# musikisomorphie/implicit-normalizing-flows

Measured on AMD Instinct MI355X. Metric: samples/sec (whole node) + bits/dim Δ vs ref, CIFAR10 density eval at 1/8 GPU, higher is better.
Workload: dtype f32; 1 GPU; cifar10 implicit flow density eval (run_cifar10.sh arch), batch 64 per GPU; global_batch=64, per_gpu_batch=64, parallelism=dp1, probes=device, mode=eval

## Files before the change

implicit-normalizing-flows_amd/csrc/engine.h:

```cpp
#pragma once
#include <math.h>
#include <stdio.h>
#include <stdlib.h>
#include <string.h>

#include <algorithm>
#include <functional>
#include <vector>

#include "glue.h"
#include "kernels.h"

constexpr unsigned INF_EV_SYNC = hipEventDisableTiming | hipEventDisableSystemFence;
constexpr unsigned INF_EV_TIMING = hipEventDisableSystemFence;

namespace inf {

constexpr int TAPS_MAX_CH = 64;
constexpr int SERIES_MAX = 128;

struct Operand {
  int load = BL_DIRECT;
  int taps = 0;
  int M = 0, Mpad = 0, K = 0, Kpad = 0;
  int pack = PK_ROWMAJOR;
  float* A = nullptr;
};

struct WLayer {
  int kind = 0, cin = 0, cout = 0, ks = 1;
  const float *W = nullptr, *b = nullptr, *u = nullptr, *v = nullptr;
  float coeff = 1.f;
  int act = ACT_NONE;
  const float* act_beta = nullptr;
  Operand f, g;
  float* factor = nullptr;
  float* zb = nullptr;
};

}

struct InfNet {
  int C = 0, H = 1, W = 1, P = 1, d = 0;
  bool fc = false;
  int pre_act = inf::ACT_NONE;
  const float* pre_beta = nullptr;
  std::vector<inf::WLayer> L;
  int hidden_max = 0;
  int rows_max = 0;
  float* dev = nullptr;
  double* scratch = nullptr;
  size_t scratch_doubles = 0;
  int device = 0;
  bool fused = false;
  int fhid = 0, K1pad = 0, M3 = 0, M3pad = 0;
  int ftiles = 0, fpix = 0;
  float *F1f = nullptr, *F1b = nullptr, *F2f = nullptr, *F2b = nullptr, *F3f = nullptr, *F3b = nullptr;
  uint16_t* Fs[6] = {nullptr, nullptr, nullptr, nullptr, nullptr, nullptr};
  uint16_t* Fh[6] = {nullptr, nullptr, nullptr, nullptr, nullptr, nullptr};
  int* Fexp = nullptr;
  uint16_t* Fhp[2] = {nullptr, nullptr};
  int mfma_mode = INF_MFMA_F32;
  float* f0 = nullptr;
  int f0_batch = -1;
  int k128 = 1;
  int eval_overlap = 1;
  int convergence = INF_CONV_GLOBAL;
  int line_search = 0;
  int exact_scale = 0;
  int presplit = 1;
  int fc_block = 1;
  int fc_series = 1;
  int fc_skinny = 1;
  bool fcfused = false;
  uint16_t* fch = nullptr;
  int* fchexp = nullptr;
  std::vector<size_t> fch_off;
  uint16_t* fcht = nullptr;
  int* fchtexp = nullptr;
};

namespace inf {

struct WS {
  char* base;
  size_t cap, off;
  bool ok = true;
  template <typename T>
  T* take(size_t n) {
    off = (off + 255) & ~(size_t)255;
    T* p = base ? reinterpret_cast<T*>(base + off) : nullptr;
    off += n * sizeof(T);
    if (off > cap) ok = false;
    return p;
  }
};

struct Bufs {
  float *h0, *h1, *Y;
  std::vector<float*> D;
  float *xin, *xemb, *fx, *xa, *xb, *ga, *gb, *upd, *dx, *dg, *lowest, *va, *vb, *eps_t, *zero, *tmp;
  float *fcur, *flow;
  float* fspec;
  float *U, *VT;
  float *ext0, *ext1;
  double *part, *bpart, *sumsq;
  double* ps_state;
  int *ps_active, *ps_improved;
  float *ps_lowx, *ps_lowf;
  unsigned int* counter;
  int nchunk;
  float* Y2;
  int snchunk;
  unsigned* bk_sync;
  size_t bk_sync_bytes;
  char* bk_out;
  size_t bk_out_bytes;
  hipEvent_t stop_ev = nullptr;
  bool stop_bound = false;
  float* kslab = nullptr;
  size_t kslab_bytes = 0;
  bool sample_sums = false;
};

struct GradBufs {
  std::vector<float*> H, Hd, Ad;
  std::vector<float*> A;
  float *gA, *gB, *hA, *hB, *gad, *ga, *Y, *slab, *dWe, *dWe2, *dsig, *xin, *tmp_in, *act;
  float *x_t, *w_t, *e_t, *gx_t;
  double *bpart, *dot;
  int max_split;
  float* kslab;
  size_t kslab_bytes;
};

size_t carve(const InfNet* n, int B, int T, void* ws, size_t cap, Bufs& b);
size_t ws_need(const InfNet* n, int B, int T);
inline int carve_ws(const InfNet* n, int B, int T, void* ws, size_t ws_bytes, Bufs& b) {
  return (!ws || carve(n, B, T, ws, ws_bytes, b) > ws_bytes) ? INF_ERR_WORKSPACE : INF_OK;
}

inline bool same_shape(const InfNet* a, const InfNet* b) {
  return a->C == b->C && a->H == b->H && a->W == b->W && a->fc == b->fc && a->d == b->d;
}
inline bool fused_pair(const InfNet* a, const InfNet* b) {
  return a->fused && b->fused && a->fhid == b->fhid && (a->L[0].act == ACT_SWISH) == (b->L[0].act == ACT_SWISH);
}

GemmArgs gemm_base(const InfNet* n, const Operand& op, const float* X, int in_ch, int B);
void set_out(const InfNet* n, GemmArgs& g, float* out, int out_rows);
int layer_gemm(const InfNet* n, const GemmArgs& g, int load, int epi, float* kslab, size_t kslab_bytes, hipStream_t s);
Net313Args net313_args(const InfNet* n, const float* in, int B, Bufs& bf, bool vjp);
FcArgs fc_args(const InfNet* n, const float* x, int B);
int out_stage(const InfNet* n, const Operand& op, int mode, OutArgs a, float* Y, int B, hipStream_t s);
inline Operand fused_taps(const InfNet* n) {
  Operand op;
  op.taps = 1;
  op.M = n->M3;
  return op;
}
int run_forward(InfNet* n, const float* x, int B, Bufs& bf, int mode, const OutArgs* oa, hipStream_t s);
int run_vjp(InfNet* n, const float* v, float* vout, const float* xin, const float* eps, double* partial, int B,
            Bufs& bf, hipStream_t s);
int to_internal(InfNet* n, const float* x, float* buf, int B, hipStream_t s, const float** xi);
int to_boundary(InfNet* n, const float* xi, float* out, int B, hipStream_t s);
template <typename Produce>
int write_boundary(InfNet* n, Bufs& bf, float* out, int B, hipStream_t s, Produce&& produce) {
  INF_TRY(produce(n->fc ? bf.tmp : out));
  return n->fc ? to_boundary(n, bf.tmp, out, B, s) : INF_OK;
}

int host_wait(hipEvent_t ev);
InfBroydenStats stats_for(const InfBroydenStats* caller);
struct SpecTail {
  std::function<int(const float* x, const float* f)> fn;
  const float* x = nullptr;
  const float* f = nullptr;
};
int broyden_solve(InfNet* f, const float* y, int B, int T, double eps_in, InfBroydenStats* st, float* diff_detail,
                  Bufs& bf, hipStream_t s, SpecTail* tail = nullptr);
int fc_block_eval(InfNet* nx, InfNet* nz, const float* x, float* z, float* logdet_x, float* logdet_z, int B, int T,
                  double eps_in, InfBroydenStats* stats, Bufs& bf, hipStream_t s);
void solve_release_thread();

int fc_jacobian(InfNet* n, const float* x, int B, Bufs& bf, const float** tang, hipStream_t s);
void logdet_release_thread();

}
```

implicit-normalizing-flows_amd/csrc/engine_chain.hip:

```cpp
#include "engine.h"

using namespace inf;

GemmArgs inf::gemm_base(const InfNet* n, const Operand& op, const float* X, int in_ch, int B) {
  GemmArgs g;
  memset(&g, 0, sizeof(g));
  g.x6 = n->mfma_mode != INF_MFMA_F32;
  g.A = op.A;
  g.M = op.M;
  g.Kpad = op.Kpad;
  g.Ktot = op.K;
  g.X = X;
  if (n->fc) {
    g.P = B;
    g.N = B;
    g.x_sample = 0;
    g.H = 1;
    g.W = B;
  } else {
    g.P = n->P;
    g.N = B * n->P;
    g.x_sample = (long)in_ch * n->P;
    g.H = n->H;
    g.W = n->W;
// ... 108 lines not shown
  }
  const float* cur = x;
  int cur_ch = n->C;
  for (int l = 0; l < L - 1; ++l) {
    const WLayer& w = n->L[l];
    float* out = (l % 2 == 0) ? bf.h0 : bf.h1;
    GemmArgs g = gemm_base(n, w.f, cur, cur_ch, B);
    g.pre_beta = (l == 0) ? n->pre_beta : nullptr;
    g.pre_act = (l == 0) ? n->pre_act : ACT_NONE;
    set_out(n, g, out, w.cout);
    g.bias = w.b;
    g.act = w.act;
    g.act_beta = w.act_beta;
    g.deriv_out = (mode < 0) ? bf.D[l] : nullptr;
    g.write_out = (mode < 0 && l == L - 2) ? 0 : 1;
    INF_TRY(layer_gemm(n, g, w.f.load, EP_BIAS_ACT, bf.kslab, bf.kslab_bytes, s));
    cur = out;
    cur_ch = w.cout;
  }
  if (mode < 0) return INF_OK;
  const WLayer& w = n->L[L - 1];
  GemmArgs g = gemm_base(n, w.f, cur, cur_ch, B);
  g.pre_beta = (L == 1) ? n->pre_beta : nullptr;
  g.pre_act = (L == 1) ? n->pre_act : ACT_NONE;
  set_out(n, g, bf.Y, w.f.M);
  INF_TRY(layer_gemm(n, g, w.f.load, EP_STORE, bf.kslab, bf.kslab_bytes, s));
  OutArgs a = *oa;
  a.bias = w.b;
  a.pre_beta = nullptr;
  return out_stage(n, w.f, mode, a, bf.Y, B, s);
}

int inf::run_vjp(InfNet* n, const float* v, float* vout, const float* xin, const float* eps, double* partial, int B,
                 Bufs& bf, hipStream_t s) {
  const int L = (int)n->L.size();
  OutArgs a;
  memset(&a, 0, sizeof(a));
  a.in0 = eps;
  a.in1 = xin;
  a.out0 = vout;
  a.pre_beta = n->pre_beta;
  a.pre_act = n->pre_act;
  a.partial = partial;
  a.nchunk = n->fc ? fc_nchunk(n->d) : out_nchunk(n->d);
  if (n->fused) {
    Net313Args f = net313_args(n, v, B, bf, true);
    INF_TRY(launch_net313(f, n->fhid, MODE_VJP, s));
    return out_stage(n, fused_taps(n), OM_VJP, a, bf.Y, B, s);
  }
  const float* cur = v;
  int cur_ch = n->C;
  for (int l = L - 1; l >= 1; --l) {
    const WLayer& w = n->L[l];
    float* out = ((L - 1 - l) % 2 == 0) ? bf.h0 : bf.h1;
    GemmArgs g = gemm_base(n, w.g, cur, cur_ch, B);
    set_out(n, g, out, w.cin);
    g.deriv_in = bf.D[l - 1];
    INF_TRY(layer_gemm(n, g, w.g.load, EP_MUL_DERIV, bf.kslab, bf.kslab_bytes, s));
    cur = out;
    cur_ch = w.cin;
  }
  const WLayer& w = n->L[0];
  GemmArgs g = gemm_base(n, w.g, cur, cur_ch, B);
  set_out(n, g, bf.Y, w.g.M);
  INF_TRY(layer_gemm(n, g, w.g.load, EP_STORE, bf.kslab, bf.kslab_bytes, s));
  return out_stage(n, w.g, OM_VJP, a, bf.Y, B, s);
}

int inf::to_internal(InfNet* n, const float* x, float* buf, int B, hipStream_t s, const float** xi) {
  *xi = n->fc ? buf : x;
  return n->fc ? launch_transpose(x, buf, B, n->d, s) : INF_OK;
}
int inf::to_boundary(InfNet* n, const float* xi, float* out, int B, hipStream_t s) {
  if (!n->fc) {
    if (xi != out) INF_HIP(hipMemcpyAsync(out, xi, sizeof(float) * (size_t)B * n->d, hipMemcpyDeviceToDevice, s));
    return INF_OK;
  }
  return launch_transpose(xi, out, n->d, B, s);
}

extern "C" {

int inf_net_forward(InfNet* n, const float* x, float* y, int B, void* ws, size_t ws_bytes, void* stream) {
  if (!n || !x || !y || B <= 0) return INF_ERR_INVALID;
  hipStream_t s = (hipStream_t)stream;
  Bufs bf;
  INF_TRY(carve_ws(n, B, 1, ws, ws_bytes, bf));
  const float* xi;
  INF_TRY(to_internal(n, x, bf.xin, B, s, &xi));
  OutArgs a;
  memset(&a, 0, sizeof(a));
  return write_boundary(n, bf, y, B, s, [&](float* o) {
    a.out0 = o;
    return run_forward(n, xi, B, bf, OM_PLAIN, &a, s);
  });
}

int inf_net_vjp(InfNet* n, const float* x, const float* v, float* out, int B, void* ws, size_t ws_bytes,
                void* stream) {
  if (!n || !x || !v || !out || B <= 0) return INF_ERR_INVALID;
  hipStream_t s = (hipStream_t)stream;
  Bufs bf;
  INF_TRY(carve_ws(n, B, 1, ws, ws_bytes, bf));
  const float *xi, *vi;
  INF_TRY(to_internal(n, x, bf.xin, B, s, &xi));
  INF_TRY(to_internal(n, v, bf.eps_t, B, s, &vi));
  INF_TRY(run_forward(n, xi, B, bf, -1, nullptr, s));
  return write_boundary(n, bf, out, B, s,
                        [&](float* o) { return run_vjp(n, vi, o, xi, nullptr, nullptr, B, bf, s); });
}

}
```

implicit-normalizing-flows_amd/csrc/engine_grad.hip:

```cpp
#include "engine.h"

using namespace inf;

namespace {

constexpr int GRAD_SPLIT = 32;
constexpr int GRAD_BLOCKS = 512;

size_t carve_grad(const InfNet* n, int B, void* ws, size_t cap, GradBufs& g) {
  WS w{reinterpret_cast<char*>(ws), cap, 0};
  const size_t hid = (size_t)B * n->hidden_max * n->P, in = (size_t)B * n->d;
  const int L = (int)n->L.size();
  size_t mn = 1;
  for (const auto& l : n->L) mn = std::max(mn, (size_t)l.cout * l.cin * l.ks * l.ks);
  g.H.resize(L > 0 ? L - 1 : 0);
  g.Hd.resize(L > 0 ? L - 1 : 0);
  g.Ad.resize(L > 0 ? L : 0);
  for (auto& p : g.H) p = w.take<float>(hid);
  for (auto& p : g.Hd) p = w.take<float>(hid);
  for (int l = 0; l < L; ++l) g.Ad[l] = w.take<float>(l == 0 ? in : hid);
  g.A.resize(L > 0 ? L : 0);
  for (int l = 0; l < L; ++l) g.A[l] = w.take<float>(l == 0 ? in : hid);
  for (float** p : {&g.gA, &g.gB, &g.hA, &g.hB, &g.gad, &g.ga}) *p = w.take<float>(std::max(hid, in));
  g.Y = w.take<float>((size_t)B * n->rows_max * n->P);
// ... 233 lines not shown
                                nin, GRAD_BLOCKS, s));
        if (n->pre_beta && gr->dpre_beta) INF_TRY(launch_beta_reduce(gb.bpart, GRAD_BLOCKS, gr->dpre_beta, 0, s));
      } else if (gx) {
        if (G_pri) INF_HIP(hipMemcpyAsync(gx, gb.ga, sizeof(float) * nin, hipMemcpyDeviceToDevice, s));
        else INF_HIP(hipMemsetAsync(gx, 0, sizeof(float) * nin, s));
      }
    }
  }
  return INF_OK;
}

constexpr int FC_JAC_MAX = 16;

size_t logdet_grad_layout(InfNet* n, int B, int mode, int n_terms, char* ws, size_t cap, Bufs* bf, GradBufs* gb,
                          float** A, float** bv, float** xr, float** gxs, float** eps_t, float** a_scr, float** b_scr) {
  const int T = mode == LOGDET_SERIES ? n_terms : n->d;
  const long N = (long)T * B;
  Bufs bf0;
  GradBufs gb0;
  const size_t s1 = (carve(n, B, 1, ws, ws ? cap : 0, bf ? *bf : bf0) + 255) & ~(size_t)255;
  char* w2 = ws ? ws + s1 : nullptr;
  const size_t s2 = (carve_grad(n, (int)N, w2, ws ? (cap > s1 ? cap - s1 : 0) : 0, gb ? *gb : gb0) + 255) & ~(size_t)255;
  WS w{ws ? ws + s1 + s2 : nullptr, ws ? (cap > s1 + s2 ? cap - s1 - s2 : 0) : 0, 0};
  float* p[6];
  const size_t cnt[6] = {(size_t)n->d * N, (size_t)n->d * N, (size_t)n->d * N, (size_t)n->d * N,
                         n->d > FC_JAC_MAX ? 0 : (size_t)n->d * B, mode == LOGDET_SERIES ? (size_t)n_terms * n->d * B : 1};
  for (int i = 0; i < 6; ++i) p[i] = w.take<float>(cnt[i]);
  float* pb = n->d > FC_JAC_MAX ? w.take<float>(((size_t)n_terms + 1) * n->d * B) : nullptr;
  if (A) {
    *A = p[0];
    *bv = p[1];
    *xr = p[2];
    *gxs = p[3];
    *eps_t = p[4];
    *a_scr = p[5];
    *b_scr = pb;
  }
  return s1 + s2 + w.off + 256;
}

int run_jvp(InfNet* n, const float* v, float* out, int B, Bufs& bf, hipStream_t s) {
  const int L = (int)n->L.size();
  const float* cur = v;
  for (int l = 0; l < L; ++l) {
    const WLayer& w = n->L[l];
    const bool last = l == L - 1;
    float* o = last ? out : ((l % 2 == 0) ? bf.h0 : bf.h1);
    GemmArgs g = gemm_base(n, w.f, cur, w.cin, B);
    set_out(n, g, o, w.cout);
    g.deriv_in = last ? nullptr : bf.D[l];
    INF_TRY(layer_gemm(n, g, w.f.load, last ? EP_STORE : EP_MUL_DERIV, bf.kslab, bf.kslab_bytes, s));
    cur = o;
  }
  return INF_OK;
}

int series_pairs_chains(InfNet* n, const float* x, const float* eps, const float* coeff, int n_terms, const float* gout,
                        float* value, int B, Bufs& bf, float* A, float* bv, float* xr, float* a_scr, float* b_scr,
                        hipStream_t s) {
  const size_t dB = (size_t)n->d * B;
  const float* xi;
  INF_TRY(to_internal(n, x, bf.xin, B, s, &xi));
  INF_TRY(launch_transpose(eps, a_scr, B, n->d, s));
  INF_HIP(hipMemcpyAsync(b_scr, a_scr, sizeof(float) * dB, hipMemcpyDeviceToDevice, s));
  INF_TRY(run_forward(n, xi, B, bf, -1, nullptr, s));
  for (int j = 0; j + 1 < n_terms; ++j)
    INF_TRY(run_vjp(n, a_scr + j * dB, a_scr + (j + 1) * dB, xi, nullptr, nullptr, B, bf, s));
  for (int m = 0; m < n_terms; ++m) INF_TRY(run_jvp(n, b_scr + m * dB, b_scr + (m + 1) * dB, B, bf, s));
  return launch_series_pairs_wide(a_scr, b_scr, xi, gout, coeff, n_terms, n->d, B, A, bv, xr, value, s);
}

}

extern "C" {

size_t inf_grad_workspace_bytes(InfNet* n, int B) {
  if (!n || B <= 0) return 0;
  GradBufs gb;
  return carve_grad(n, B, nullptr, 0, gb);
}

int inf_net_param_grad(InfNet* n, const float* x, const float* gout, float* gx, const InfNetGrads* gr, int B,
                       void* ws, size_t ws_bytes, void* stream) {
  if (!n || !x || !gout || !gr || B <= 0) return INF_ERR_INVALID;
  if (!grad_supported(n)) return INF_ERR_UNSUPPORTED;
  hipStream_t s = (hipStream_t)stream;
  GradBufs gb;
  if (!ws || carve_grad(n, B, ws, ws_bytes, gb) > ws_bytes) return INF_ERR_WORKSPACE;
  if (!n->fc) return param_grad_core(n, x, gout, gx, gr, B, gb, s);
  INF_TRY(launch_transpose(x, gb.x_t, B, n->d, s));
  INF_TRY(launch_transpose(gout, gb.w_t, B, n->d, s));
  INF_TRY(param_grad_core(n, gb.x_t, gb.w_t, gx ? gb.gx_t : nullptr, gr, B, gb, s));
  if (gx) INF_TRY(launch_transpose(gb.gx_t, gx, n->d, B, s));
  return INF_OK;
}

int inf_net_surrogate_grad(InfNet* n, const float* x, const float* w, const float* eps, float* value, float* gx,
                           const InfNetGrads* gr, int B, void* ws, size_t ws_bytes, void* stream) {
  if (!n || !x || !w || !eps || !gr || B <= 0) return INF_ERR_INVALID;
  if (!grad_supported(n) || (n->fc && value)) return INF_ERR_UNSUPPORTED;
  hipStream_t s = (hipStream_t)stream;
  GradBufs gb;
  if (!ws || carve_grad(n, B, ws, ws_bytes, gb) > ws_bytes) return INF_ERR_WORKSPACE;
  if (!n->fc) return surrogate_core(n, x, w, eps, value, gx, gr, B, gb, s);
  INF_TRY(launch_transpose(x, gb.x_t, B, n->d, s));
  INF_TRY(launch_transpose(w, gb.w_t, B, n->d, s));
  INF_TRY(launch_transpose(eps, gb.e_t, B, n->d, s));
  INF_TRY(surrogate_core(n, gb.x_t, gb.w_t, gb.e_t, nullptr, gx ? gb.gx_t : nullptr, gr, B, gb, s));
  if (gx) INF_TRY(launch_transpose(gb.gx_t, gx, n->d, B, s));
  return INF_OK;
}

size_t inf_logdet_grad_workspace_bytes(InfNet* n, int B, int mode, int n_terms) {
  if (!n || B <= 0 || mode < LOGDET_SERIES || mode > LOGDET_TRACE || (mode != LOGDET_EXACT && n_terms < 1)) return 0;
  return logdet_grad_layout(n, B, mode, n_terms, nullptr, 0, nullptr, nullptr, nullptr, nullptr, nullptr, nullptr,
                            nullptr, nullptr, nullptr);
}

int inf_logdet_grad(InfNet* n, const float* x, int mode, const float* eps, const float* coeff, int n_terms,
                    const float* gout, float* value, float* gx, const InfNetGrads* gr, int B, void* ws, size_t ws_bytes,
                    void* stream) {
  if (!n || !x || !gr || B <= 0 || mode < LOGDET_SERIES || mode > LOGDET_TRACE) return INF_ERR_INVALID;
  if (mode == LOGDET_SERIES && (!eps || !coeff || n_terms < 1 || n_terms > 128)) return INF_ERR_INVALID;
  if (mode == LOGDET_TRACE && (!coeff || n_terms < 1 || n_terms > 128)) return INF_ERR_INVALID;
  const bool wide = n->fc && n->d > FC_JAC_MAX;
  if (!n->fc || (wide && mode != LOGDET_SERIES) || !grad_supported(n)) return INF_ERR_UNSUPPORTED;
  if (wide && (long)n_terms * B > 0x7fffffffL) return INF_ERR_INVALID;
  hipStream_t s = (hipStream_t)stream;
  Bufs bf;
  GradBufs gb;
  float *A, *bv, *xr, *gxs, *eps_t, *a_scr, *b_scr;
  const int nt = mode == LOGDET_EXACT ? 1 : n_terms;
  if (!ws || logdet_grad_layout(n, B, mode, nt, reinterpret_cast<char*>(ws), ws_bytes, &bf, &gb, &A, &bv, &xr, &gxs,
                                &eps_t, &a_scr, &b_scr) > ws_bytes)
    return INF_ERR_WORKSPACE;
  const int T = mode == LOGDET_SERIES ? n_terms : n->d;
  if (wide) {
    INF_TRY(series_pairs_chains(n, x, eps, coeff, n_terms, gout, value, B, bf, A, bv, xr, a_scr, b_scr, s));
  } else {
    const float* tang = nullptr;
    INF_TRY(fc_jacobian(n, x, B, bf, &tang, s));
    if (mode == LOGDET_SERIES) INF_TRY(launch_transpose(eps, eps_t, B, n->d, s));
    const float one = 1.f;
    INF_TRY(launch_logdet_pairs(mode, tang, eps_t, bf.xin, gout, mode == LOGDET_EXACT ? &one : coeff, nt, n->d, B, A,
                                bv, xr, value, a_scr, s));
  }
  INF_TRY(surrogate_core(n, xr, A, bv, nullptr, gx ? gxs : nullptr, gr, T * B, gb, s));
  if (gx) INF_TRY(launch_sum_pairs(gxs, T, n->d, B, gx, s));
  return INF_OK;
}

}
```

implicit-normalizing-flows_amd/csrc/engine_logdet.hip:

```cpp
#include "engine.h"

using namespace inf;

namespace {

int series_fused(InfNet* const* nets, const float* const* xs, const float* const* es, int nn, const float* coeff,
                 int n_terms, float* const* outs, int B, Bufs* bfs, hipStream_t s, unsigned save_mask = 3u,
                 float* const* wouts = nullptr, const float* ncoeff = nullptr) {
  Net313Args args[2];
  for (int i = 0; i < nn; ++i) {
    args[i] = net313_args(nets[i], xs[i], B, bfs[i], false);
    if (!wouts) INF_HIP(hipMemsetAsync(bfs[i].part, 0, sizeof(double) * n_terms * B * bfs[i].snchunk, s));
    else INF_HIP(hipMemcpyAsync(wouts[i], es[i], sizeof(float) * (size_t)B * nets[i]->d, hipMemcpyDeviceToDevice, s));
  }
  const unsigned all = (1u << nn) - 1u;
  if ((save_mask & all) == all) {
    INF_TRY(launch_net313_multi(args, nn, nets[0]->fhid, MODE_SAVE, s));
  } else {
    for (int i = 0; i < nn; ++i)
      if (save_mask & (1u << i)) INF_TRY(launch_net313_multi(&args[i], 1, nets[0]->fhid, MODE_SAVE, s, nn));
  }
  for (int k = 0; k < n_terms; ++k) {
    for (int i = 0; i < nn; ++i) {
      InfNet* n = nets[i];
      Bufs& bf = bfs[i];
      Net313Args& v = args[i];
      v = net313_args(n, es[i], B, bf, true);
      v.Y = (k % 2 == 0) ? bf.Y : bf.Y2;
      v.tile_order = k & 1;
      if (k > 0) {
        v.in = nullptr;
        v.in_taps = (k % 2 == 1) ? bf.Y : bf.Y2;
        v.vmul_x = n->pre_act != ACT_NONE ? xs[i] : nullptr;
        v.vmul_beta = n->pre_beta;
        v.vmul_act = n->pre_act == ACT_SWISH ? 0 : n->pre_act;
        if (wouts) {
          v.acc_w = wouts[i];
          v.acc_coef = ncoeff[k];
        } else {
          v.dot_eps = es[i];
          v.dot_part = bf.part + (size_t)(k - 1) * B * bf.snchunk;
          v.dot_nchunk = bf.snchunk;
        }
      }
    }
    INF_TRY(launch_net313_multi(args, nn, nets[0]->fhid, MODE_VJP, s));
  }
  for (int i = 0; i < nn; ++i) {
    InfNet* n = nets[i];
    Bufs& bf = bfs[i];
    OutArgs a;
    memset(&a, 0, sizeof(a));
    a.in0 = wouts ? nullptr : es[i];
    a.in1 = xs[i];
    a.out0 = bf.va;
    a.pre_beta = n->pre_beta;
    a.pre_act = n->pre_act;
    a.partial = wouts ? nullptr : bf.part + (size_t)(n_terms - 1) * B * bf.snchunk;
    a.nchunk = bf.snchunk;
    INF_TRY(out_stage(n, fused_taps(n), OM_VJP, a, ((n_terms - 1) % 2 == 0) ? bf.Y : bf.Y2, B, s));
    if (wouts) INF_TRY(glue_axpy_scaled(wouts[i], bf.va, ncoeff[n_terms], (long)B * n->d, s));
  }
  if (wouts) return INF_OK;
  for (int i = 0; i < nn; ++i)
    INF_TRY(launch_series_combine(bfs[i].part, coeff, n_terms, B, bfs[i].snchunk, outs[i], s));
  return INF_OK;
}

struct SideStream {
  hipStream_t s = nullptr;
  hipEvent_t fork = nullptr, join = nullptr;
};
thread_local SideStream g_side[16];
SideStream* side_stream() {
  int dev = 0;
  if (hipGetDevice(&dev) != hipSuccess || dev < 0 || dev >= 16) return nullptr;
  SideStream& ss = g_side[dev];
  if (!ss.s) {
    if (hipStreamCreateWithFlags(&ss.s, hipStreamNonBlocking) != hipSuccess) return nullptr;
    if (hipEventCreateWithFlags(&ss.fork, INF_EV_SYNC) != hipSuccess ||
        hipEventCreateWithFlags(&ss.join, INF_EV_SYNC) != hipSuccess)
      return nullptr;
  }
  return &ss;
}

struct SideJoin {
  SideStream* side = nullptr;
  hipStream_t s = nullptr;
  ~SideJoin() {
    if (!side) return;
    (void)hipEventRecord(side->join, side->s);
    (void)hipStreamWaitEvent(s, side->join, 0);
  }
};

struct FcNextX {
  InfNet* nx = nullptr;
  Bufs* bf = nullptr;
  float* logdet = nullptr;
  bool done = false;
};
struct FcLogpStep {
  const float* lin = nullptr;
  float* lout = nullptr;
  bool done = false;
};
bool fc_block_first(const InfNet* nz) {
  return nz->fc_block == 2 || (nz->fc_block == 1 && nz->convergence == INF_CONV_PER_SAMPLE);
}
bool fc_pair_ok(const InfNet* a, const InfNet* b) {
  return a->fcfused && b->fcfused && a->mfma_mode == INF_MFMA_F16X3 && b->mfma_mode == INF_MFMA_F16X3 &&
         same_shape(a, b) && !a->L.empty() && !b->L.empty() && a->L[0].act == b->L[0].act;
}

int eval_exact_fc(InfNet* nx, InfNet* nz, const float* x, float* z, float* logdet_x, float* logdet_z, int B, int T,
                  double eps, InfBroydenStats* stats, Bufs& bf, hipStream_t s, bool x_done, FcNextX* next,
                  FcLogpStep* lp = nullptr) {
  if (next) next->done = false;
  if (lp) lp->done = false;
  const float* xi = bf.xin;
  if (fc_block_first(nz)) {
    const int st = fc_block_eval(nx, nz, x, z, logdet_x, logdet_z, B, T, eps, stats, bf, s);
    if (st != INF_ERR_UNSUPPORTED) return st;
  }
  if (!x_done) {
    FcArgs fjx = fc_args(nx, nullptr, B);
    fjx.x_bnd = x;
    fjx.x_int = bf.xin;
    fjx.logdet = logdet_x;
    fjx.o.in0 = xi;
    fjx.o.out0 = bf.fx;
    fjx.o.out1 = bf.xemb;
    INF_TRY(launch_fcnet(fjx, true, s));
  }
  auto jac_z = [&](const float* flow) {
    FcArgs fjz = fc_args(nz, nullptr, B);
    fjz.logdet = logdet_z;
    fjz.rc_fx = bf.fx;
    fjz.rc_fz = flow;
    fjz.rc_x = xi;
    fjz.rc_out = z;
    if (lp) {
      fjz.lp_in = lp->lin;
      fjz.lp_ldx = logdet_x;
      fjz.lp_out = lp->lout;
      lp->done = true;
    }
    if (next) {
      FcArgs fjn = fc_args(next->nx, nullptr, B);
      fjn.rc_fx = bf.fx;
      fjn.rc_fz = flow;
      fjn.rc_x = xi;
      fjn.x_int = next->bf->xin;
      fjn.logdet = next->logdet;
      fjn.o.out0 = next->bf->fx;
      fjn.o.out1 = next->bf->xemb;
      const int st = launch_fcnet_jac_pair(fjz, fjn, s);
      next->done = st == INF_OK;
      if (st != INF_ERR_UNSUPPORTED) return st;
    }
    return launch_fcnet(fjz, true, s);
  };
  SpecTail tail;
  tail.fn = [&](const float*, const float* f) { return jac_z(f); };
  InfBroydenStats sst = stats_for(stats);
  INF_TRY(broyden_solve(nz, xi, B, T, eps, &sst, nullptr, bf, s, nz->convergence == INF_CONV_GLOBAL ? &tail : nullptr));
  if (stats) *stats = sst;
  if (!sst.prot_break) {
    if (tail.x && tail.x == bf.lowest && tail.f == bf.flow) return INF_OK;
    return jac_z(bf.flow);
  }
  if (next) next->done = false;
  if (lp) lp->done = false;
  OutArgs a;
  memset(&a, 0, sizeof(a));
// ... 67 lines not shown
  }
  const float *xi, *ei;
  INF_TRY(to_internal(n, x, bf.xin, B, s, &xi));
  INF_TRY(to_internal(n, vareps, bf.eps_t, B, s, &ei));
  if (n->fused) return series_fused(&n, &xi, &ei, 1, coeff, n_terms, &out, B, &bf, s);
  INF_TRY(run_forward(n, xi, B, bf, -1, nullptr, s));
  const float* v = ei;
  for (int k = 0; k < n_terms; ++k) {
    float* vo = (k % 2 == 0) ? bf.va : bf.vb;
    INF_TRY(run_vjp(n, v, vo, xi, ei, bf.part + (size_t)k * B * bf.nchunk, B, bf, s));
    v = vo;
  }
  return launch_series_combine(bf.part, coeff, n_terms, B, bf.nchunk, out, s);
}

int neumann_w(InfNet* n, const float* xi, const float* ei, const float* ncoeff, int n_terms, int B, Bufs& bf,
              hipStream_t s) {
  const size_t E = (size_t)B * n->d;
  INF_TRY(run_forward(n, xi, B, bf, -1, nullptr, s));
  INF_HIP(hipMemcpyAsync(bf.tmp, ei, sizeof(float) * E, hipMemcpyDeviceToDevice, s));
  const float* v = ei;
  for (int k = 1; k <= n_terms; ++k) {
    float* vo = (k % 2 == 1) ? bf.va : bf.vb;
    INF_TRY(run_vjp(n, v, vo, xi, nullptr, nullptr, B, bf, s));
    INF_TRY(glue_axpy_scaled(bf.tmp, vo, ncoeff[k], (long)E, s));
    v = vo;
  }
  return INF_OK;
}

}

int inf::fc_jacobian(InfNet* n, const float* x, int B, Bufs& bf, const float** tang, hipStream_t s) {
  const int d = n->d;
  const float* xi;
  INF_TRY(to_internal(n, x, bf.xin, B, s, &xi));
  if (n->fcfused) {
    FcArgs f = fc_args(n, xi, B);
    f.tang = bf.ext1;
    if (fcnet_supported(f, true)) {
      INF_TRY(launch_fcnet(f, true, s));
      *tang = bf.ext1;
      return INF_OK;
    }
  }
  INF_TRY(glue_init_tangents(xi, bf.ext0, d, B, s));
  const int cols = (d + 1) * B;
  const float* cur = bf.ext0;
  for (size_t l = 0; l < n->L.size(); ++l) {
    const WLayer& w = n->L[l];
    float* o = (l % 2 == 0) ? bf.ext1 : bf.ext0;
    GemmArgs g;
    memset(&g, 0, sizeof(g));
    g.A = w.f.A;
    g.M = w.f.M;
    g.Kpad = w.f.Kpad;
    g.Ktot = w.f.K;
    g.X = cur;
    g.x_sample = 0;
    g.P = cols;
    g.N = cols;
    g.H = 1;
    g.W = cols;
    g.out = o;
    g.o_sample = 0;
    g.bias = w.b;
    g.n_primal = B;
    INF_TRY(launch_gemm(g, BL_DIRECT, EP_BIAS_PRIMAL, s));
    if (w.act != ACT_NONE) INF_TRY(launch_fwdmode_act(o, nullptr, w.cout, B, d, w.act, w.act_beta, s));
    cur = o;
  }
  *tang = cur;
  return INF_OK;
}

void inf::logdet_release_thread() {
  int cur = 0;
  (void)hipGetDevice(&cur);
  for (int dev = 0; dev < 16; ++dev) {
    SideStream& ss = g_side[dev];
    if (!ss.s) continue;
    (void)hipSetDevice(dev);
    (void)hipStreamSynchronize(ss.s);
    if (ss.fork) (void)hipEventDestroy(ss.fork);
    if (ss.join) (void)hipEventDestroy(ss.join);
    (void)hipStreamDestroy(ss.s);
    ss = SideStream{};
  }
  (void)hipSetDevice(cur);
}

extern "C" {

int inf_imblock_eval(InfNet* nx, InfNet* nz, const float* x, float* z, const float* eps_x, const float* eps_z,
                     const float* coeff, int n_terms, float* logdet_x, float* logdet_z, int B, int T, double eps,
                     InfBroydenStats* stats, void* ws, size_t ws_bytes, void* stream) {
  if (!nx || !nz || !x || !z || !eps_x || !eps_z || !coeff || !logdet_x || !logdet_z || B <= 0 || T <= 0 || T > 64 ||
      n_terms < 1 || n_terms > SERIES_MAX || !same_shape(nx, nz))
    return INF_ERR_INVALID;
  if (!fused_pair(nx, nz)) return INF_ERR_UNSUPPORTED;
  hipStream_t s = (hipStream_t)stream;
  const size_t half = ws_need(nx, B, T), zneed = ws_need(nz, B, 1), xneed = ws_need(nx, B, 1);
  if (!ws || ws_bytes < half + zneed) return INF_ERR_WORKSPACE;
  char* w0 = reinterpret_cast<char*>(ws);
  Bufs bfa, bfb, bfc;
  carve(nx, B, T, w0, half, bfa);
  carve(nz, B, 1, w0 + half, zneed, bfb);
  const bool overlap = nx->eval_overlap && ws_bytes >= half + zneed + xneed;
  if (overlap) {
    carve(nx, B, 1, w0 + half + zneed, xneed, bfc);
    bfc.D = bfa.D;
  }
  const int layout = overlap ? 1 : 2;
  {
    Net313Args f = net313_args(nx, x, B, bfa, false);
    INF_TRY(launch_net313_multi(&f, 1, nx->fhid, MODE_EVALSAVE, s, layout));
    OutArgs a;
    memset(&a, 0, sizeof(a));
    a.bias = nx->L[2].b;
    a.in0 = x;
    a.out0 = bfa.fx;
    a.out1 = bfa.xemb;
    INF_TRY(out_stage(nx, fused_taps(nx), OM_EMBED, a, bfa.Y, B, s));
  }
  SideJoin join;
  if (overlap) {
    SideStream* side = side_stream();
    if (!side) return INF_ERR_HIP;
    INF_HIP(hipEventRecord(side->fork, s));
    INF_HIP(hipStreamWaitEvent(side->s, side->fork, 0));
    join.side = side;
    join.s = s;
    INF_TRY(series_fused(&nx, &x, &eps_x, 1, coeff, n_terms, &logdet_x, B, &bfc, side->s, 0u));
  }
  InfBroydenStats st = stats_for(stats);
  INF_TRY(broyden_solve(nz, x, B, T, eps, &st, nullptr, bfa, s));
  if (stats) *stats = st;
  if (!st.prot_break) {
    INF_TRY(glue_recomp(bfa.fx, bfa.flow, x, z, (long)B * nx->d, s));
  } else {
    OutArgs a;
    memset(&a, 0, sizeof(a));
    a.in0 = bfa.fx;
    a.in1 = x;
    a.out0 = z;
    INF_TRY(run_forward(nz, bfa.lowest, B, bfa, OM_RECOMP, &a, s));
  }
  if (overlap) {
    const float* zin = z;
    return series_fused(&nz, &zin, &eps_z, 1, coeff, n_terms, &logdet_z, B, &bfb, s, 1u);
  }
  InfNet* nets[2] = {nx, nz};
  const float* xs[2] = {x, z};
  const float* es[2] = {eps_x, eps_z};
  float* outs[2] = {logdet_x, logdet_z};
  Bufs bfs[2] = {bfa, bfb};
  return series_fused(nets, xs, es, 2, coeff, n_terms, outs, B, bfs, s, 2u);
}

int inf_imblock_eval_exact(InfNet* nx, InfNet* nz, const float* x, float* z, float* logdet_x, float* logdet_z, int B,
                           int T, double eps, InfBroydenStats* stats, void* ws, size_t ws_bytes, void* stream) {
  if (!nx || !nz || !x || !z || !logdet_x || !logdet_z || B <= 0 || T <= 0 || T > 64 || !same_shape(nx, nz))
    return INF_ERR_INVALID;
  INF_TRY(eval_exact_check(nx, nz, x, B));
  Bufs bf;
  INF_TRY(carve_ws(nz, B, T, ws, ws_bytes, bf));
  return eval_exact_fc(nx, nz, x, z, logdet_x, logdet_z, B, T, eps, stats, bf, (hipStream_t)stream, false, nullptr);
}

size_t inf_flow_chain_workspace_bytes(InfNet* const* net_z, int n_blocks, int batch, const int* thresholds) {
  if (!net_z || n_blocks <= 0 || batch <= 0 || !thresholds) return 0;
  size_t blk = 0;
  for (int i = 0; i < n_blocks; ++i)
    if (net_z[i]) blk = std::max(blk, inf_workspace_bytes(net_z[i], batch, thresholds[i]));
  const size_t d = net_z[0] ? (size_t)net_z[0]->d : 0;
  return 2 * ((blk + 255) & ~(size_t)255) + 256 * 8 + sizeof(float) * ((size_t)2 * batch * d + (size_t)6 * batch);
}

int inf_flow_eval_exact_chain(InfNet* const* net_x, InfNet* const* net_z, int n_blocks, const float* x, float* z,
                              const float* logp_in, float* logp_out, int B, const int* thresholds, const double* eps,
                              InfBroydenStats* stats, void* ws, size_t ws_bytes, void* stream) {
  if (!net_x || !net_z || n_blocks <= 0 || !x || !z || !logp_out || B <= 0 || !thresholds || !eps || x == z ||
      logp_in == logp_out)
    return INF_ERR_INVALID;
  for (int i = 0; i < n_blocks; ++i) {
    InfNet *nx = net_x[i], *nz = net_z[i];
    if (!nx || !nz || !same_shape(nx, nz) || !same_shape(nz, net_z[0]) || thresholds[i] <= 0 || thresholds[i] > 64)
      return INF_ERR_INVALID;
    INF_TRY(eval_exact_check(nx, nz, x, B));
  }
  if (!ws || ws_bytes < inf_flow_chain_workspace_bytes(net_z, n_blocks, B, thresholds)) return INF_ERR_WORKSPACE;
  hipStream_t s = (hipStream_t)stream;
  const size_t E = (size_t)B * net_z[0]->d;
  size_t blk = 0;
  for (int i = 0; i < n_blocks; ++i) blk = std::max(blk, inf_workspace_bytes(net_z[i], B, thresholds[i]));
  blk = (blk + 255) & ~(size_t)255;
  char* base = reinterpret_cast<char*>(ws);
  size_t off = 2 * blk;
  auto take = [&](size_t bytes) {
    off = (off + 255) & ~(size_t)255;
    char* p = base + off;
    off += bytes;
    return reinterpret_cast<float*>(p);
  };
  float* zb[2] = {take(sizeof(float) * E), take(sizeof(float) * E)};
  float* ldx[2] = {take(sizeof(float) * B), take(sizeof(float) * B)};
  float* ldz[2] = {take(sizeof(float) * B), take(sizeof(float) * B)};
  float* lp[2] = {take(sizeof(float) * B), take(sizeof(float) * B)};
  Bufs bfs[2];
  auto carve_block = [&](int i) {
    return carve_ws(net_z[i], B, thresholds[i], base + (size_t)(i & 1) * blk, blk, bfs[i & 1]);
  };
  INF_TRY(carve_block(0));
  const float* in = x;
  const float* lin = logp_in;
  bool x_done = false;
  for (int i = 0; i < n_blocks; ++i) {
    const bool last = i == n_blocks - 1;
    float* out = last ? z : zb[i & 1];
    float* lout = last ? logp_out : lp[i & 1];
    FcNextX nxt;
    FcNextX* np = nullptr;
    if (!last) {
      INF_TRY(carve_block(i + 1));
      if (!fc_block_first(net_z[i]) && !fc_block_first(net_z[i + 1]) && fc_pair_ok(net_z[i], net_x[i + 1])) {
        nxt.nx = net_x[i + 1];
        nxt.bf = &bfs[(i + 1) & 1];
        nxt.logdet = ldx[(i + 1) & 1];
        np = &nxt;
      }
    }
    FcLogpStep lps;
    lps.lin = lin;
    lps.lout = lout;
    INF_TRY(eval_exact_fc(net_x[i], net_z[i], in, out, ldx[i & 1], ldz[i & 1], B, thresholds[i], eps[i],
                          stats ? &stats[i] : nullptr, bfs[i & 1], s, x_done, np, &lps));
    if (!lps.done) INF_TRY(glue_logp_step(lin, ldx[i & 1], ldz[i & 1], lout, B, s));
    x_done = np && nxt.done;
    in = out;
    lin = lout;
  }
  return INF_OK;
}

int inf_logdet_series(InfNet* n, const float* x, const float* vareps, const float* coeff, int n_terms, float* out,
                      int B, void* ws, size_t ws_bytes, void* stream) {
  if (!n || !x || !vareps || !coeff || !out || B <= 0 || n_terms < 0 || n_terms > SERIES_MAX) return INF_ERR_INVALID;
  return series_single(n, x, vareps, coeff, n_terms, out, B, ws, ws_bytes, (hipStream_t)stream, true);
}

int inf_logdet_series_pair(InfNet* na, const float* xa, const float* ea, InfNet* nb, const float* xb, const float* eb,
                           const float* coeff, int n_terms, float* out_a, float* out_b, int B, void* ws,
                           size_t ws_bytes, void* stream) {
  if (!na || !nb || !xa || !xb || !ea || !eb || !coeff || !out_a || !out_b || B <= 0 || n_terms < 0 ||
      n_terms > SERIES_MAX || !same_shape(na, nb))
    return INF_ERR_INVALID;
  const size_t half = ws_need(na, B, 1);
  if (!ws || ws_bytes < 2 * half) return INF_ERR_WORKSPACE;
  char* w0 = reinterpret_cast<char*>(ws);
  hipStream_t s = (hipStream_t)stream;
  InfNet* nets[2] = {na, nb};
  const float* xs[2] = {xa, xb};
  const float* es[2] = {ea, eb};
  float* outs[2] = {out_a, out_b};
  if (n_terms > 0) {
    const int st = fc_series(nets, xs, es, coeff, n_terms, outs, 2, B, s);
    if (st != INF_ERR_UNSUPPORTED) return st;
  }
  if (!fused_pair(na, nb)) {
    INF_TRY(series_single(na, xa, ea, coeff, n_terms, out_a, B, w0, half, s, false));
    return series_single(nb, xb, eb, coeff, n_terms, out_b, B, w0 + half, half, s, false);
  }
  Bufs bfs[2];
  carve(na, B, 1, w0, half, bfs[0]);
  carve(nb, B, 1, w0 + half, half, bfs[1]);
  if (n_terms == 0) {
    INF_HIP(hipMemsetAsync(out_a, 0, sizeof(float) * B, s));
    INF_HIP(hipMemsetAsync(out_b, 0, sizeof(float) * B, s));
    return INF_OK;
  }
  return series_fused(nets, xs, es, 2, coeff, n_terms, outs, B, bfs, s);
}

int inf_neumann_vector(InfNet* n, const float* x, const float* vareps, const float* ncoeff, int n_terms, float* w,
                       int B, void* ws, size_t ws_bytes, void* stream) {
  if (!n || !x || !vareps || !ncoeff || !w || B <= 0 || n_terms < 0) return INF_ERR_INVALID;
  hipStream_t s = (hipStream_t)stream;
  Bufs bf;
  INF_TRY(carve_ws(n, B, 1, ws, ws_bytes, bf));
  const float *xi, *ei;
  INF_TRY(to_internal(n, x, bf.xin, B, s, &xi));
  INF_TRY(to_internal(n, vareps, bf.eps_t, B, s, &ei));
  INF_TRY(neumann_w(n, xi, ei, ncoeff, n_terms, B, bf, s));
  return to_boundary(n, bf.tmp, w, B, s);
}

int inf_neumann_vector_pair(InfNet* na, const float* xa, const float* ea, InfNet* nb, const float* xb,
                            const float* eb, const float* ncoeff, int n_terms, float* wa, float* wb, int B, void* ws,
                            size_t ws_bytes, void* stream) {
  if (!na || !nb || !xa || !xb || !ea || !eb || !ncoeff || !wa || !wb || B <= 0 || n_terms < 0 || !same_shape(na, nb))
    return INF_ERR_INVALID;
  const size_t half = ws_bytes / 2;
  char* w1 = reinterpret_cast<char*>(ws) + half;
  if (!fused_pair(na, nb) || n_terms == 0) {
    INF_TRY(inf_neumann_vector(na, xa, ea, ncoeff, n_terms, wa, B, ws, half, stream));
    return inf_neumann_vector(nb, xb, eb, ncoeff, n_terms, wb, B, w1, half, stream);
  }
  hipStream_t s = (hipStream_t)stream;
  Bufs bfs[2];
  INF_TRY(carve_ws(na, B, 1, ws, half, bfs[0]));
  INF_TRY(carve_ws(nb, B, 1, w1, half, bfs[1]));
  InfNet* nets[2] = {na, nb};
  const float* xs[2] = {xa, xb};
  const float* es[2] = {ea, eb};
  float* wouts[2] = {wa, wb};
  float* outs[2] = {nullptr, nullptr};
  return series_fused(nets, xs, es, 2, nullptr, n_terms, outs, B, bfs, s, 3u, wouts, ncoeff);
}

int inf_logdet_neumann(InfNet* n, const float* x, const float* vareps, const float* ncoeff, int n_terms, float* out,
                       int B, void* ws, size_t ws_bytes, void* stream) {
  if (!n || !x || !vareps || !ncoeff || !out || B <= 0 || n_terms < 0) return INF_ERR_INVALID;
  hipStream_t s = (hipStream_t)stream;
  Bufs bf;
  INF_TRY(carve_ws(n, B, 1, ws, ws_bytes, bf));
  const float *xi, *ei;
  INF_TRY(to_internal(n, x, bf.xin, B, s, &xi));
  INF_TRY(to_internal(n, vareps, bf.eps_t, B, s, &ei));
  INF_TRY(neumann_w(n, xi, ei, ncoeff, n_terms, B, bf, s));
  INF_TRY(run_vjp(n, bf.tmp, bf.va, xi, ei, bf.part, B, bf, s));
  const float one = 1.f;
  return launch_series_combine(bf.part, &one, 1, B, bf.nchunk, out, s);
}

int inf_logdet_exact(InfNet* n, const float* x, float* out, int B, void* ws, size_t ws_bytes, void* stream) {
  if (!n || !x || !out || B <= 0) return INF_ERR_INVALID;
  if (!n->fc || n->d > 16 || n->pre_act != ACT_NONE) return INF_ERR_UNSUPPORTED;
  hipStream_t s = (hipStream_t)stream;
  Bufs bf;
  INF_TRY(carve_ws(n, B, 1, ws, ws_bytes, bf));
  if (n->fcfused) {
    const float* xi;
    INF_TRY(to_internal(n, x, bf.xin, B, s, &xi));
    FcArgs f = fc_args(n, xi, B);
    f.logdet = out;
    if (fcnet_supported(f, true)) return launch_fcnet(f, true, s);
  }
  const float* tang = nullptr;
  INF_TRY(fc_jacobian(n, x, B, bf, &tang, s));
  return launch_logdet_small(tang, out, n->d, B, B, s);
}

int inf_logdet_exact_trace(InfNet* n, const float* x, const float* coeff, int n_terms, float* out, int B, void* ws,
                           size_t ws_bytes, void* stream) {
  if (!n || !x || !coeff || !out || B <= 0 || n_terms < 1 || n_terms > SERIES_MAX) return INF_ERR_INVALID;
  if (!n->fc || n->d > 16 || n->pre_act != ACT_NONE) return INF_ERR_UNSUPPORTED;
  hipStream_t s = (hipStream_t)stream;
  Bufs bf;
  INF_TRY(carve_ws(n, B, 1, ws, ws_bytes, bf));
  const float* tang = nullptr;
  INF_TRY(fc_jacobian(n, x, B, bf, &tang, s));
  return launch_trace_series(tang, coeff, n_terms, out, n->d, B, B, s);
}

}
```

implicit-normalizing-flows_amd/csrc/engine_plan.hip:

```cpp
#include <memory>
#include <new>

#include "engine.h"

using namespace inf;

namespace {

int round_up(int x, int m) { return (x + m - 1) / m * m; }

bool fused_act_kind(int act) {
  return act == ACT_SWISH || act == ACT_SIN || act == ACT_ELU || act == ACT_SOFTPLUS || act == ACT_RELU;
}

int act_of_kind(int kind) {
  switch (kind) {
    case INF_ACT_SWISH: return ACT_SWISH;
    case INF_ACT_SIN: return ACT_SIN;
    case INF_ACT_ELU: return ACT_ELU;
    case INF_ACT_SOFTPLUS: return ACT_SOFTPLUS;
    case INF_ACT_RELU: return ACT_RELU;
    case INF_ACT_LCUBE: return ACT_LCUBE;
    case INF_ACT_IDENTITY: return ACT_IDENTITY;
    case INF_ACT_ZERO: return ACT_ZERO;
    default: return -1;
  }
}

struct FusedSizes {
  size_t n[6];
  explicit FusedSizes(const InfNet* net) {
    n[0] = n[1] = (size_t)net->fhid * net->K1pad;
    n[2] = n[3] = (size_t)net->fhid * net->fhid;
    n[4] = n[5] = (size_t)net->M3pad * net->fhid;
  }
  size_t sum() const { return n[0] + n[1] + n[2] + n[3] + n[4] + n[5]; }
};

int parse_mfma(const char* mm, bool has_bf16x6, int* mode) {
  if (!mm || !*mm) return INF_OK;
  if (!strcmp(mm, "f32") || !strcmp(mm, "fp32")) *mode = INF_MFMA_F32;
  else if (!strcmp(mm, "bf16x6")) *mode = has_bf16x6 ? INF_MFMA_BF16X6 : INF_MFMA_F32;
  else if (strcmp(mm, "f16x3") != 0) {
    fprintf(stderr, "libinflow: INFLOW_MFMA=%s is not one of f32, fp32, bf16x6, f16x3\n", mm);
    return INF_ERR_INVALID;
  }
  return INF_OK;
}

struct NetOption {
  int id;
  int InfNet::*slot;
  int hi;
  const char* env;
  const char* names[4];
  bool resets_f0;
};
const NetOption OPTIONS[] = {
    {INF_OPT_FUSED_K128, &InfNet::k128, 3, "INFLOW_FUSED_K128", {"0", "1", "2", "3"}, true},
    {INF_OPT_EVAL_OVERLAP, &InfNet::eval_overlap, 1, "INFLOW_EVAL_OVERLAP", {"0", "1"}, false},
    {INF_OPT_CONVERGENCE, &InfNet::convergence, 1, "INFLOW_CONVERGENCE", {"global", "per_sample"}, false},
    {INF_OPT_LINE_SEARCH, &InfNet::line_search, 1, nullptr, {}, false},
    {INF_OPT_K128_EXACT_SCALE, &InfNet::exact_scale, 1, nullptr, {}, true},
    {INF_OPT_FC_BLOCK, &InfNet::fc_block, 2, "INFLOW_FC_BLOCK", {"0", "1", "2"}, false},
    {INF_OPT_FC_SERIES, &InfNet::fc_series, 1, "INFLOW_FC_SERIES", {"0", "1"}, false},
    {INF_OPT_FC_SKINNY, &InfNet::fc_skinny, 1, nullptr, {}, false},
    {INF_OPT_FUSED_PRESPLIT, &InfNet::presplit, 1, "INFLOW_FUSED_PRESPLIT", {"0", "1"}, false},
};
const NetOption* find_option(int id) {
  for (const NetOption& o : OPTIONS)
    if (o.id == id) return &o;
  return nullptr;
}

void free_net(InfNet* n) {
  if (!n) return;
  if (n->dev) (void)hipFree(n->dev);
  if (n->scratch) (void)hipFree(n->scratch);
  if (n->f0) (void)hipFree(n->f0);
  if (n->fch) (void)hipFree(n->fch);
  if (n->fchexp) (void)hipFree(n->fchexp);
  delete n;
}
struct NetDeleter {
  void operator()(InfNet* n) const { free_net(n); }
};

size_t per_sample_hidden(const InfNet* n) {
  return (size_t)n->hidden_max * (n->fc ? 1 : (n->fused ? std::max(n->P, n->fpix) : n->P));
}

}

size_t inf::carve(const InfNet* n, int B, int T, void* ws, size_t cap, Bufs& b) {
  WS w{reinterpret_cast<char*>(ws), cap, 0};
  const size_t E = (size_t)B * n->d;
  const size_t Hs = (size_t)B * per_sample_hidden(n);
  const size_t Ys = (size_t)B * n->rows_max * (n->fc ? 1 : n->P);
  const int nchunk = n->fc ? fc_nchunk(n->d) : out_nchunk(n->d);
  b.nchunk = nchunk;
  b.snchunk = n->fused ? std::max(nchunk, std::max(n->P / 32, n->ftiles)) : nchunk;
  b.h0 = w.take<float>(Hs);
  b.h1 = w.take<float>(Hs);
  b.Y = w.take<float>(Ys);
  b.Y2 = n->fused ? w.take<float>(Ys) : nullptr;
  b.D.resize(n->L.size() > 0 ? n->L.size() - 1 : 0);
  for (auto& p : b.D) p = w.take<float>(Hs);
  float** vecs[] = {&b.xin, &b.xemb, &b.fx, &b.xa, &b.xb, &b.ga, &b.gb, &b.upd,
                    &b.dx, &b.dg, &b.lowest, &b.va, &b.vb, &b.eps_t, &b.zero, &b.tmp, &b.fcur, &b.flow,
                    &b.fspec, &b.ps_lowx, &b.ps_lowf};
  for (float** v : vecs) *v = w.take<float>(E);
  b.U = w.take<float>((size_t)T * E);
  b.VT = w.take<float>((size_t)T * E);
  if (n->fc && n->d <= 16) {
    const size_t ext = (size_t)(n->d + 1) * B * std::max(n->hidden_max, n->d);
    b.ext0 = w.take<float>(ext);
    b.ext1 = w.take<float>(ext);
  } else {
    b.ext0 = b.ext1 = nullptr;
  }
  b.part = w.take<double>((size_t)B * std::max(nchunk, b.snchunk) * SERIES_MAX);
  const int bch = (n->d + 1023) / 1024;
  b.bpart = w.take<double>((size_t)B * bch * (3 * (size_t)T + 2) + 64);
  b.sumsq = w.take<double>((size_t)B + 1);
  b.counter = w.take<unsigned int>(64);
  b.ps_state = w.take<double>((size_t)B * (PS_HEAD + T));
  b.ps_active = w.take<int>((size_t)B);
  b.ps_improved = w.take<int>((size_t)B);
  if (n->fc) {
    b.bk_sync_bytes = 16 + sizeof(unsigned long long) * 8 * (size_t)fcblock_grid(B);
    b.bk_sync = reinterpret_cast<unsigned*>(w.take<char>(b.bk_sync_bytes));
    b.bk_out_bytes = sizeof(FcBlockStats) + (sizeof(int) * 3 + sizeof(double)) * (size_t)B + 64;
    b.bk_out = w.take<char>(b.bk_out_bytes);
  } else {
    b.bk_sync = nullptr;
    b.bk_out = nullptr;
    b.bk_sync_bytes = b.bk_out_bytes = 0;
  }
  b.kslab_bytes = (n->fc && n->d > FC_NARROW_MAX) ? SKINNY_SLAB_BYTES : 0;
  b.kslab = b.kslab_bytes ? w.take<float>(b.kslab_bytes / sizeof(float)) : nullptr;
  return w.off + 256;
}

// ... 203 lines not shown
    if (v < 0) {
      fprintf(stderr, "libinflow: %s=%s is not one of", o.env, e);
      for (int k = 0; k <= o.hi; ++k) fprintf(stderr, " %s", o.names[k]);
      fprintf(stderr, "\n");
      return INF_ERR_INVALID;
    }
    n->*o.slot = v;
  }
  size_t sc = SIGMA_MAX_PARTS + 64;
  for (auto& w : n->L) sc = std::max(sc, (size_t)w.cout * (n->fc ? 1 : n->P) / 256 + 64);
  n->scratch_doubles = sc;
  if (hipGetDevice(&n->device) != hipSuccess) n->device = 0;
  if (hipMalloc(&n->dev, floats * sizeof(float)) != hipSuccess ||
      hipMalloc(&n->scratch, sc * sizeof(double)) != hipSuccess)
    return INF_ERR_HIP;
  float* p = n->dev;
  for (auto& w : n->L) {
    for (Operand* op : {&w.f, &w.g}) {
      op->A = p;
      p += (size_t)op->Mpad * op->Kpad + 64;
    }
    w.factor = p;
    p += 64;
    if (!w.b) {
      w.zb = p;
      w.b = p;
      p += round_up(w.cout, 64);
    }
  }
  if (n->fused) {
    float** bufs[] = {&n->F1f, &n->F1b, &n->F2f, &n->F2b, &n->F3f, &n->F3b};
    const FusedSizes sz(n);
    for (int k = 0; k < 6; ++k) {
      *bufs[k] = p;
      p += sz.n[k] + 64;
    }
    for (int k = 0; k < 6; ++k) {
      n->Fs[k] = reinterpret_cast<uint16_t*>(p);
      p += (3 * sz.n[k] + 1) / 2 + 64;
    }
    for (int k = 0; k < 6; ++k) {
      n->Fh[k] = reinterpret_cast<uint16_t*>(p);
      p += sz.n[k] + 64;
    }
    n->Fexp = reinterpret_cast<int*>(p);
    p += 64;
    for (int k = 0; k < 2; ++k) {
      n->Fhp[k] = reinterpret_cast<uint16_t*>(p);
      p += sz.n[4 + k] + 64;
    }
  }
  *out = net.release();
  return INF_OK;
}

int inf_net_destroy(InfNet* n) {
  free_net(n);
  return INF_OK;
}

int inf_net_set_mfma(InfNet* n, int mode) {
  if (!n || (mode != INF_MFMA_F32 && mode != INF_MFMA_BF16X6 && mode != INF_MFMA_F16X3)) return INF_ERR_INVALID;
  if (n->mfma_mode != mode) n->f0_batch = -1;
  n->mfma_mode = mode;
  return INF_OK;
}
int inf_net_get_mfma(const InfNet* n) { return n ? n->mfma_mode : -1; }

int inf_net_set_option(InfNet* n, int option, int value) {
  const NetOption* o = n ? find_option(option) : nullptr;
  if (!o || value < 0 || value > o->hi) return -INF_ERR_INVALID;
  const int prev = n->*o->slot;
  n->*o->slot = value;
  if (prev != value && o->resets_f0) n->f0_batch = -1;
  return prev;
}

int inf_net_get_option(const InfNet* n, int option) {
  const NetOption* o = n ? find_option(option) : nullptr;
  return o ? n->*o->slot : -INF_ERR_INVALID;
}

int inf_net_refresh(InfNet* n, void* stream) {
  if (!n) return INF_ERR_INVALID;
  hipStream_t s = (hipStream_t)stream;
  n->f0_batch = -1;
  for (auto& w : n->L) {
    if (w.zb) INF_HIP(hipMemsetAsync(w.zb, 0, sizeof(float) * w.cout, s));
    const int H = n->fc ? 1 : (w.ks == 1 ? 1 : n->H), Wd = n->fc ? 1 : (w.ks == 1 ? 1 : n->W);
    INF_TRY(launch_sigma(w.W, w.u, w.v, w.cout, w.cin, w.ks, H, Wd, w.coeff, w.factor,
                         reinterpret_cast<float*>(n->scratch), s));
    INF_TRY(launch_pack(w.W, w.factor, w.f.A, w.cout, w.cin, w.ks, w.f.Mpad, w.f.Kpad, w.f.pack, s));
    INF_TRY(launch_pack(w.W, w.factor, w.g.A, w.cout, w.cin, w.ks, w.g.Mpad, w.g.Kpad, w.g.pack, s));
  }
  if (n->fch) {
    const int L = (int)n->L.size();
    for (int l = 0; l < L; ++l) {
      const WLayer& w = n->L[l];
      const int nrt = l == L - 1 ? 1 : 8, nks = l == 0 ? 1 : 4;
      INF_TRY(launch_fc_split_h3(w.f.A, w.cout, w.f.Kpad, nrt, nks, n->fch + n->fch_off[l], n->fchexp + l, s));
      const int j = L - 1 - l, trt = j == L - 1 ? 1 : 8, tks = j == 0 ? 1 : 4;
      INF_TRY(launch_fc_split_h3(w.g.A, w.cin, w.g.Kpad, trt, tks, n->fcht + n->fch_off[j], n->fchtexp + j, s));
    }
  }
  if (n->fused) {
    const WLayer &l0 = n->L[0], &l1 = n->L[1], &l2 = n->L[2];
    const int H = n->fhid;
    INF_TRY(launch_pack(l0.W, l0.factor, n->F1f, l0.cout, l0.cin, 3, H, n->K1pad, PK_IM2COL_FWD, s, 1));
    INF_TRY(launch_pack(l2.W, l2.factor, n->F1b, l2.cout, l2.cin, 3, H, n->K1pad, PK_IM2COL_BWD, s, 1));
    INF_TRY(launch_pack(l1.W, l1.factor, n->F2f, H, H, 1, H, H, PK_ROWMAJOR, s, 1));
    INF_TRY(launch_pack(l1.W, l1.factor, n->F2b, H, H, 1, H, H, PK_TRANSPOSE, s, 1));
    INF_TRY(launch_pack(l2.W, l2.factor, n->F3f, l2.cout, l2.cin, 3, n->M3pad, H, PK_TAPS_FWD, s, 1));
    INF_TRY(launch_pack(l0.W, l0.factor, n->F3b, l0.cout, l0.cin, 3, n->M3pad, H, PK_TAPS_BWD, s, 1));
    const float* src[6] = {n->F1f, n->F1b, n->F2f, n->F2b, n->F3f, n->F3b};
    const FusedSizes cnt(n);
    for (int i = 0; i < 6; ++i) INF_TRY(launch_split3(src[i], n->Fs[i], (long)cnt.n[i], s));
    for (int i = 0; i < 6; ++i)
      INF_TRY(launch_split2h(src[i], n->Fh[i], (long)cnt.n[i], n->Fexp + 3 * (i & 1) + i / 2, s));
    for (int i = 0; i < 2; ++i) INF_TRY(launch_permute_k23(n->Fh[4 + i], n->Fhp[i], (long)cnt.n[4 + i] / 512, s));
  }
  return INF_OK;
}

}
```

implicit-normalizing-flows_amd/csrc/engine_solve.hip:

```cpp
#include <chrono>
#include <thread>

#include "engine.h"

using namespace inf;

namespace {

struct SumsSlot {
  double* host = nullptr;
  hipEvent_t ev = nullptr;
  int cap = 0;
};
thread_local SumsSlot g_sums_slots[2];
int sums_slot(int i, int B, SumsSlot** out) {
  SumsSlot& sl = g_sums_slots[i & 1];
  if (sl.cap < B + 1) {
    if (sl.host) (void)hipHostFree(sl.host);
    sl.host = nullptr;
    const int cap = std::max(B + 1, 1024);
    if (hipHostMalloc(reinterpret_cast<void**>(&sl.host), sizeof(double) * cap, hipHostMallocCoherent) != hipSuccess)
      return INF_ERR_HIP;
    sl.cap = cap;
  }
// ... 744 lines not shown
  INF_HIP(hipMemcpyAsync(g_bk_host, bf.bk_sync, 16, hipMemcpyDeviceToHost, s));
  INF_HIP(hipMemcpyAsync(g_bk_host + 16, bf.bk_out, nbytes, hipMemcpyDeviceToHost, s));
  if (!g_bk_ev && hipEventCreateWithFlags(&g_bk_ev, INF_EV_SYNC) != hipSuccess) return INF_ERR_HIP;
  hipEvent_t ev = g_bk_ev;
  INF_HIP(hipEventRecord(ev, s));
  INF_TRY(host_wait(ev));
  if (*reinterpret_cast<unsigned*>(g_bk_host) != 0) {
    set_hip_error(hipErrorLaunchTimeOut);
    return INF_ERR_HIP;
  }
  const FcBlockStats* hs = reinterpret_cast<const FcBlockStats*>(g_bk_host + 16);
  InfBroydenStats st = stats_for(stats);
  st.convergence = nz->convergence;
  if (!a.per_sample) {
    st.nstep = hs->nstep;
    st.lowest_step = hs->lowest_step;
    st.prot_break = hs->prot_break;
    st.n_trace = std::min(hs->n_trace, 64);
    for (int k = 0; k < st.n_trace; ++k) st.trace[k] = hs->trace[k];
    st.diff = hs->lowest;
    st.eps = a.eps;
  } else {
    const char* base = g_bk_host + 16;
    const int* sn = reinterpret_cast<const int*>(base + sizeof(FcBlockStats));
    const int* sl = sn + B;
    const int* sp = sl + B;
    const double* slo = reinterpret_cast<const double*>(
        base + ((sizeof(FcBlockStats) + sizeof(int) * 3 * (size_t)B + 7) & ~(size_t)7));
    double d2 = 0.0;
    for (int b = 0; b < B; ++b) {
      st.nstep = std::max(st.nstep, sn[b]);
      st.lowest_step = std::max(st.lowest_step, sl[b]);
      st.prot_break |= sp[b];
      d2 += slo[b] * slo[b];
      if (st.sample_nstep) st.sample_nstep[b] = sn[b];
      if (st.sample_lowest_step) st.sample_lowest_step[b] = sl[b];
      if (st.sample_prot_break) st.sample_prot_break[b] = sp[b];
    }
    st.diff = sqrt(d2);
    st.eps = a.eps_ps;
  }
  st.tnstep = st.nstep;
  if (st.prot_break) {
    std::vector<int> todo;
    if (a.per_sample) {
      const int* sp = reinterpret_cast<const int*>(g_bk_host + 16 + sizeof(FcBlockStats)) + 2 * B;
      todo.assign(sp, sp + B);
    }
    int it = 0;
    INF_TRY(banach_solve(nz, bf.xin, B, eps_in, 1000, todo.empty() ? nullptr : todo.data(), bf, s, &it));
    st.fixed_point_iters = it;
    OutArgs o;
    memset(&o, 0, sizeof(o));
    o.in0 = bf.fx;
    o.in1 = bf.xin;
    o.out0 = bf.tmp;
    INF_TRY(run_forward(nz, bf.lowest, B, bf, OM_RECOMP, &o, s));
    FcArgs fjz = fc_args(nz, bf.tmp, B);
    fjz.logdet = logdet_z;
    INF_TRY(launch_fcnet(fjz, true, s));
    INF_TRY(to_boundary(nx, bf.tmp, z, B, s));
  }
  if (stats) *stats = st;
  return INF_OK;
}

void inf::solve_release_thread() {
  for (SumsSlot& sl : g_sums_slots) {
    if (sl.host) (void)hipHostFree(sl.host);
    if (sl.ev) (void)hipEventDestroy(sl.ev);
    sl = SumsSlot{};
  }
  if (g_bk_host) (void)hipHostFree(g_bk_host);
  g_bk_host = nullptr;
  g_bk_host_cap = 0;
  if (g_bk_ev) (void)hipEventDestroy(g_bk_ev);
  g_bk_ev = nullptr;
}

extern "C" {

int inf_root_find(InfNet* f, InfNet* e, const float* y, float* out, int B, int T, double eps, InfBroydenStats* stats,
                  float* diff_detail, void* ws, size_t ws_bytes, void* stream) {
  if (!f || !e || !y || !out || B <= 0 || T <= 0 || T > 64 || !same_shape(f, e)) return INF_ERR_INVALID;
  hipStream_t s = (hipStream_t)stream;
  Bufs bf;
  INF_TRY(carve_ws(f, B, T, ws, ws_bytes, bf));
  const float* yi;
  INF_TRY(embed(f, e, y, B, bf, &yi, s));
  INF_TRY(broyden_solve(f, yi, B, T, eps, stats, diff_detail, bf, s));
  return to_boundary(f, bf.lowest, out, B, s);
}

int inf_imblock_forward(InfNet* nx, InfNet* nz, const float* x, float* z, int B, int T, double eps,
                        InfBroydenStats* stats, void* ws, size_t ws_bytes, void* stream) {
  if (!nx || !nz || !x || !z || B <= 0 || T <= 0 || T > 64 || !same_shape(nx, nz)) return INF_ERR_INVALID;
  hipStream_t s = (hipStream_t)stream;
  Bufs bf;
  INF_TRY(carve_ws(nx, B, T, ws, ws_bytes, bf));
  const float* xi;
  InfBroydenStats st = stats_for(stats);
  INF_TRY(embed(nz, nx, x, B, bf, &xi, s));
  INF_TRY(broyden_solve(nz, xi, B, T, eps, &st, nullptr, bf, s));
  if (stats) *stats = st;
  return write_boundary(nx, bf, z, B, s, [&](float* o) {
    if (!st.prot_break) return glue_recomp(bf.fx, bf.flow, xi, o, (long)B * nx->d, s);
    OutArgs a;
    memset(&a, 0, sizeof(a));
    a.in0 = bf.fx;
    a.in1 = xi;
    a.out0 = o;
    return run_forward(nz, bf.lowest, B, bf, OM_RECOMP, &a, s);
  });
}

int inf_imblock_backward(InfNet* nx, InfNet* nz, const float* z, const float* x, const float* grad, float* dl_dh,
                         float* dl_dx, int B, int T, double eps, InfBroydenStats* stats, void* ws, size_t ws_bytes,
                         void* stream) {
  if (!nx || !nz || !z || !x || !grad || !dl_dh || !dl_dx || B <= 0 || T <= 0 || T > 64 || !same_shape(nx, nz))
    return INF_ERR_INVALID;
  hipStream_t s = (hipStream_t)stream;
  {
    Bufs bf;
    INF_TRY(carve_ws(nz, B, T, ws, ws_bytes, bf));
    const float *zi, *gi;
    INF_TRY(to_internal(nz, z, bf.xin, B, s, &zi));
    INF_TRY(to_internal(nz, grad, bf.xemb, B, s, &gi));
    INF_TRY(run_forward(nz, zi, B, bf, -1, nullptr, s));
    InfBroydenStats bs = stats_for(stats);
    std::vector<double> lowest_ss;
    const ResidFn resid = [&](const float* y, float* gout, float* dg, const float* gprev) {
      return vjp_resid_part(nz, y, zi, gi, gout, dg, gprev, B, bf, s);
    };
    INF_TRY(broyden_core(nz, resid, B, T, eps, bs, lowest_ss, bf, s));
    if (stats) *stats = bs;
    INF_TRY(to_boundary(nz, bf.lowest, dl_dh, B, s));
  }
  Bufs bf;
  INF_TRY(carve_ws(nx, B, 1, ws, ws_bytes, bf));
  const float *xi, *hi;
  INF_TRY(to_internal(nx, x, bf.xin, B, s, &xi));
  INF_TRY(to_internal(nx, dl_dh, bf.eps_t, B, s, &hi));
  INF_TRY(run_forward(nx, xi, B, bf, -1, nullptr, s));
  INF_TRY(run_vjp(nx, hi, bf.va, xi, nullptr, nullptr, B, bf, s));
  return write_boundary(nx, bf, dl_dx, B, s,
                        [&](float* o) { return glue_add(bf.va, hi, o, (long)B * nx->d, s); });
}

int inf_banach_find_root(InfNet* f, InfNet* e, const float* y, float* out, int B, int threshold, double eps,
                         int* iters, void* ws, size_t ws_bytes, void* stream) {
  if (!f || !e || !y || !out || B <= 0 || threshold < 0 || !same_shape(f, e)) return INF_ERR_INVALID;
  hipStream_t s = (hipStream_t)stream;
  Bufs bf;
  INF_TRY(carve_ws(f, B, 1, ws, ws_bytes, bf));
  const float* yi;
  INF_TRY(embed(f, e, y, B, bf, &yi, s));
  std::vector<int> todo;
  if (f->convergence == INF_CONV_PER_SAMPLE) todo.assign(B, 1);
  int it = 0;
  INF_TRY(banach_solve(f, yi, B, eps, threshold, todo.empty() ? nullptr : todo.data(), bf, s, &it));
  if (iters) *iters = it;
  return to_boundary(f, bf.lowest, out, B, s);
}

size_t inf_broyden_workspace_bytes(int batch, int d, int threshold) {
  const size_t nchunk = (size_t)(d + 1023) / 1024;
  return sizeof(double) * ((size_t)batch * nchunk * (3 * (size_t)threshold + 2) + 64);
}

int inf_broyden_update(float* U, float* VT, const float* dx, const float* dg, const float* gx, const float* x,
                       float* update, float* x_next, float* dx_next, int B, int d, int T, int nstep, void* ws,
                       size_t ws_bytes, void* stream) {
  if (!U || !VT || !dx || !dg || !gx || !x || !update || !x_next || !dx_next || B <= 0 || d <= 0 || T <= 0 ||
      T > 64 || nstep < 1 || nstep > T)
    return INF_ERR_INVALID;
  if (!ws || ws_bytes < inf_broyden_workspace_bytes(B, d, T)) return INF_ERR_WORKSPACE;
  BroydenArgs ba;
  memset(&ba, 0, sizeof(ba));
  ba.batch = B;
  ba.d = d;
  ba.T = T;
  ba.sb = d;
  ba.si = 1;
  ba.cs = (long)B * d;
  ba.U = U;
  ba.VT = VT;
  ba.dx = dx;
  ba.dg = dg;
  ba.gx = gx;
  ba.x = x;
  ba.xnew = x_next;
  ba.dxnew = dx_next;
  ba.upd = update;
  ba.part = reinterpret_cast<double*>(ws);
  ba.m = (nstep - 1) % T;
  ba.ncols = std::min(nstep, T);
  return launch_broyden_update(ba, (hipStream_t)stream);
}

int inf_broyden_line_step(const float* x0, const float* update, float step, float* x_est, float* dx, size_t n,
                          void* stream) {
  if (!x0 || !update || !x_est || !dx || n == 0) return INF_ERR_INVALID;
  return launch_line_step(x0, update, step, x_est, dx, (long)n, (hipStream_t)stream);
}

}
```

implicit-normalizing-flows_amd/csrc/glue.h:

```cpp
#pragma once
#include "common.h"

namespace inf {
int glue_logit(const float* x, float* y, const float* lin, float* lout, int B, int per, float alpha, hipStream_t s);
int glue_actnorm(const float* x, float* y, const float* w, const float* b, const float* lin, float* lout, int B, int C,
                 int hw, hipStream_t s);
int glue_squeeze2(const float* x, float* y, int B, int C, int H, int W, hipStream_t s);
int glue_normal_logprob(const float* z, float* out, int B, int per, hipStream_t s);
int glue_rademacher(float* out, size_t n, uint64_t seed, uint64_t offset, hipStream_t s);
int glue_poison_lds(hipStream_t s);
int glue_add(const float* a, const float* b, float* out, long n, hipStream_t s);
size_t glue_batched_dot_scratch(int B, long per);
int glue_batched_dot(const float* a, const float* c, float* out, int B, long per, double* scratch, hipStream_t s);
int glue_logp_step(const float* lin, const float* ldx, const float* ldz, float* lout, int B, hipStream_t s);
int glue_recomp(const float* fx, const float* fz, const float* x, float* out, long n, hipStream_t s);
int glue_fixed_point_check(const float* x, const float* xp, const float* y, long n, float eps, unsigned int* count,
                           hipStream_t s);
int glue_axpy_scaled(float* y, const float* x, float c, long n, hipStream_t s);
int glue_init_tangents(const float* xT, float* ext, int d, int B, hipStream_t s);
}
```

implicit-normalizing-flows_amd/csrc/glue.hip:

```cpp
#include "kernels.h"
#include "glue.h"

namespace inf {

__global__ __launch_bounds__(256) void logit_kernel(const float* x, float* y, const float* lin, float* lout, int per,
                                                    float alpha) {
  __shared__ double red[16];
  const int b = blockIdx.x;
  const float* xb = x + (long)b * per;
  float* yb = y + (long)b * per;
  const float c1 = 1.f - 2.f * alpha;
  const float lc = logf(c1);
  double acc = 0.0;
  for (int i = threadIdx.x; i < per; i += blockDim.x) {
    const float s = alpha + c1 * xb[i];
    yb[i] = logf(s) - logf(1.f - s);
    acc += (double)(-logf(s - s * s) + lc);
  }
  acc = block_sum(acc, red);
  if (threadIdx.x == 0) lout[b] = (lin ? lin[b] : 0.f) - (float)acc;
}

__global__ __launch_bounds__(256) void actnorm_kernel(const float* x, float* y, const float* w, const float* bias,
                                                      const float* lin, float* lout, int C, int hw, int vec) {
  __shared__ double red[16];
  const int b = blockIdx.y;
  const long per = (long)C * hw;
  const float* xb = x + b * per;
  float* yb = y + b * per;
  const long i0 = ((long)blockIdx.x * blockDim.x + threadIdx.x) * 4;
  if (vec) {
    if (i0 < per) {
      const int c = (int)(i0 / hw);
      const float bc = bias[c], ec = expf(w[c]);
      const float4 v = *reinterpret_cast<const float4*>(xb + i0);
      *reinterpret_cast<float4*>(yb + i0) = make_float4((v.x + bc) * ec, (v.y + bc) * ec, (v.z + bc) * ec, (v.w + bc) * ec);
    }
  } else {
    for (long i = i0; i < i0 + 4 && i < per; ++i) {
      const int c = (int)(i / hw);
      yb[i] = (xb[i] + bias[c]) * expf(w[c]);
    }
  }
  if (blockIdx.x != 0) return;
  double acc = 0.0;
  for (int c = threadIdx.x; c < C; c += blockDim.x) acc += (double)w[c] * hw;
  acc = block_sum(acc, red);
  if (threadIdx.x == 0 && lout) lout[b] = (lin ? lin[b] : 0.f) - (float)acc;
}

__global__ void squeeze2_kernel(const float* x, float* y, int C, int H, int W, long n) {
  const long i = (long)blockIdx.x * blockDim.x + threadIdx.x;
  if (i >= n) return;
  const int Ho = H / 2, Wo = W / 2;
  long t = i;
  const int xo = t % Wo; t /= Wo;
  const int yo = t % Ho; t /= Ho;
  const int co = t % (4 * C); t /= (4 * C);
  const long b = t;
  const int c = co >> 2, ry = (co >> 1) & 1, rx = co & 1;
  y[i] = x[((b * C + c) * H + 2 * yo + ry) * W + 2 * xo + rx];
}

__global__ __launch_bounds__(256) void normal_logprob_kernel(const float* z, float* out, int per) {
  __shared__ double red[16];
  const int b = blockIdx.x;
  const float* zb = z + (long)b * per;
  const float logZ = -0.5f * logf(2.f * 3.14159265358979323846f);
  double acc = 0.0;
  for (int i = threadIdx.x; i < per; i += blockDim.x) {
    const float v = zb[i];
    acc += (double)(logZ - v * v / 2.f);
  }
  acc = block_sum(acc, red);
  if (threadIdx.x == 0) out[b] = (float)acc;
}

__device__ __forceinline__ uint64_t splitmix64(uint64_t z) {
  z += 0x9e3779b97f4a7c15ULL;
  z = (z ^ (z >> 30)) * 0xbf58476d1ce4e5b9ULL;
  z = (z ^ (z >> 27)) * 0x94d049bb133111ebULL;
  return z ^ (z >> 31);
}
__global__ void rademacher_kernel(float* out, size_t n, uint64_t seed, uint64_t offset) {
  const size_t i = (size_t)blockIdx.x * blockDim.x + threadIdx.x;
  if (i >= n) return;
  const uint64_t h = splitmix64(seed * 0x2545F4914F6CDD1DULL + offset + i);
  out[i] = (h >> 63) ? 1.f : -1.f;
}

__global__ void fixed_point_check_kernel(const float* x, const float* xp, const float* y, long n, float eps,
                                         unsigned int* count) {
  const long i = (long)blockIdx.x * blockDim.x + threadIdx.x;
  bool bad = false;
  if (i < n) {
    const float d = x[i] - xp[i];
    const float tol = eps + eps * fabsf(y[i]);
    bad = !((d * d) / tol < 1.f);
  }
  const unsigned long long m = __ballot(bad);
  if ((threadIdx.x & 63) == 0 && m) atomicAdd(count, (unsigned int)__popcll(m));
}

__global__ void axpy_scaled_kernel(float* y, const float* x, float c, long n) {
  const long i = (long)blockIdx.x * blockDim.x + threadIdx.x;
  if (i < n) y[i] = y[i] + c * x[i];
}

__global__ void init_tangents_kernel(const float* xT, float* ext, int d, int B) {
  const long i = (long)blockIdx.x * blockDim.x + threadIdx.x;
  const long ld = (long)(d + 1) * B;
  if (i >= (long)d * ld) return;
  const int f = i / ld;
  const long col = i - (long)f * ld;
  const int j = col / B, b = col - (long)j * B;
  ext[i] = j == 0 ? xT[(long)f * B + b] : (f == j - 1 ? 1.f : 0.f);
}

#define GRID1(n) dim3((unsigned)(((n) + 255) / 256)), dim3(256)

int glue_logit(const float* x, float* y, const float* lin, float* lout, int B, int per, float alpha, hipStream_t s) {
  hipLaunchKernelGGL(logit_kernel, dim3(B), dim3(256), 0, s, x, y, lin, lout, per, alpha);
  INF_CHECK_LAUNCH();
  return INF_OK;
}
int glue_actnorm(const float* x, float* y, const float* w, const float* b, const float* lin, float* lout, int B, int C,
                 int hw, hipStream_t s) {
  const long per = (long)C * hw;
  const int vec = (hw % 4 == 0) && (((uintptr_t)x | (uintptr_t)y) & 15) == 0;
  hipLaunchKernelGGL(actnorm_kernel, dim3((unsigned)((per + 1023) / 1024), B), dim3(256), 0, s, x, y, w, b, lin, lout, C, hw,
                     vec);
  INF_CHECK_LAUNCH();
  return INF_OK;
}
int glue_squeeze2(const float* x, float* y, int B, int C, int H, int W, hipStream_t s) {
  const long n = (long)B * C * H * W;
  hipLaunchKernelGGL(squeeze2_kernel, GRID1(n), 0, s, x, y, C, H, W, n);
  INF_CHECK_LAUNCH();
  return INF_OK;
}
int glue_normal_logprob(const float* z, float* out, int B, int per, hipStream_t s) {
  hipLaunchKernelGGL(normal_logprob_kernel, dim3(B), dim3(256), 0, s, z, out, per);
  INF_CHECK_LAUNCH();
  return INF_OK;
}
int glue_rademacher(float* out, size_t n, uint64_t seed, uint64_t offset, hipStream_t s) {
  if (n == 0) return INF_OK;
  INF_PROF_LAUNCH(s, 721, 4.0 * n, rademacher_kernel, GRID1(n), 0, s, out, n, seed, offset);
  return INF_OK;
}
int glue_fixed_point_check(const float* x, const float* xp, const float* y, long n, float eps, unsigned int* count,
                           hipStream_t s) {
  hipLaunchKernelGGL(fixed_point_check_kernel, GRID1(n), 0, s, x, xp, y, n, eps, count);
  INF_CHECK_LAUNCH();
  return INF_OK;
}
int glue_axpy_scaled(float* y, const float* x, float c, long n, hipStream_t s) {
  hipLaunchKernelGGL(axpy_scaled_kernel, GRID1(n), 0, s, y, x, c, n);
  INF_CHECK_LAUNCH();
  return INF_OK;
}
int glue_init_tangents(const float* xT, float* ext, int d, int B, hipStream_t s) {
  const long n = (long)d * (d + 1) * B;
  hipLaunchKernelGGL(init_tangents_kernel, GRID1(n), 0, s, xT, ext, d, B);
  INF_CHECK_LAUNCH();
  return INF_OK;
}

__global__ void add_kernel(const float* a, const float* b, float* out, long n) {
  const long i = (long)blockIdx.x * blockDim.x + threadIdx.x;
  if (i < n) out[i] = b[i] + a[i];
}
int glue_add(const float* a, const float* b, float* out, long n, hipStream_t s) {
  hipLaunchKernelGGL(add_kernel, GRID1(n), 0, s, a, b, out, n);
  INF_CHECK_LAUNCH();
  return INF_OK;
}

__global__ void logp_step_kernel(const float* lin, const float* ldx, const float* ldz, float* lout, int B) {
  const int b = blockIdx.x * blockDim.x + threadIdx.x;
  if (b < B) lout[b] = (lin ? lin[b] : 0.f) - (ldx[b] - ldz[b]);
}
int glue_logp_step(const float* lin, const float* ldx, const float* ldz, float* lout, int B, hipStream_t s) {
  hipLaunchKernelGGL(logp_step_kernel, dim3((B + 255) / 256), dim3(256), 0, s, lin, ldx, ldz, lout, B);
  INF_CHECK_LAUNCH();
  return INF_OK;
}

__global__ void recomp_kernel(const float* fx, const float* fz, const float* x, float* out, long n) {
  const long i = (long)blockIdx.x * blockDim.x + threadIdx.x;
  if (i < n) out[i] = (fx[i] - fz[i]) + x[i];
}
int glue_recomp(const float* fx, const float* fz, const float* x, float* out, long n, hipStream_t s) {
  INF_PROF_LAUNCH(s, 706, 16.0 * n, recomp_kernel, GRID1(n), 0, s, fx, fz, x, out, n);
  return INF_OK;
}

constexpr int DOT_CHUNK = 16384;
__global__ __launch_bounds__(256) void batched_dot_partial_kernel(const float* a, const float* c, double* part,
                                                                  long per, int nchunk) {
  __shared__ double red[16];
  const int ch = blockIdx.x, b = blockIdx.y;
  const long base = (long)b * per, lo = (long)ch * DOT_CHUNK, hi = min(per, lo + DOT_CHUNK);
  double acc = 0.0;
  for (long i = lo + threadIdx.x; i < hi; i += blockDim.x) acc += (double)a[base + i] * (double)c[base + i];
  const double t = block_sum(acc, red);
  if (threadIdx.x == 0) part[(long)b * nchunk + ch] = t;
}
__global__ void batched_dot_final_kernel(const double* part, int nchunk, int B, float* out) {
  const int b = blockIdx.x * blockDim.x + threadIdx.x;
  if (b >= B) return;
  double s = 0.0;
  for (int k = 0; k < nchunk; ++k) s += part[(long)b * nchunk + k];
  out[b] = (float)s;
}
size_t glue_batched_dot_scratch(int B, long per) { return (size_t)B * ((per + DOT_CHUNK - 1) / DOT_CHUNK); }
int glue_batched_dot(const float* a, const float* c, float* out, int B, long per, double* scratch, hipStream_t s) {
// ... 22 lines not shown
```

implicit-normalizing-flows_amd/csrc/power.hip:

```cpp
#include <algorithm>
#include <cstring>
#include <vector>

#include "kernels.h"

namespace inf {

struct PIState {
  int done, iters, use_tol, pad;
  float atol, rtol;
  double err_u, max_u;
  double sigma;
};

struct PIOp {
  const float* W;
  int cin, cout, ks, H, Wd;
};

__global__ void pi_apply_w(PIOp op, const float* __restrict__ x, float* __restrict__ y, const PIState* st) {
  if (st && st->done) return;
  const int P = op.H * op.Wd;
  const long n = (long)op.cout * P;
  const long i = (long)blockIdx.x * blockDim.x + threadIdx.x;
// ... 441 lines not shown
  op.H = spatial ? d->height : 1;
  op.Wd = spatial ? d->width : 1;
  return op;
}

static long pi_nu(const PIOp& op) { return (long)op.cout * op.H * op.Wd; }
static long pi_nv(const PIOp& op) { return (long)op.cin * op.H * op.Wd; }

static int pi_valid(const InfPowerIterDesc* d) {
  if (!d || !d->weight || !d->u || !d->v || d->cin <= 0 || d->cout <= 0) return 0;
  if (d->kind == INF_LAYER_CONV) {
    if (d->ksize < 1 || !(d->ksize & 1)) return 0;
    if (d->ksize > 1 && (d->height <= 0 || d->width <= 0)) return 0;
  } else if (d->kind != INF_LAYER_LINEAR) {
    return 0;
  }
  for (const float p : {d->domain, d->codomain})
    if (!(p == 0.f || p >= 1.f)) return 0;
  return 1;
}

static bool pi_stale_u(const InfPowerIterDesc* d) {
  return d->kind == INF_LAYER_CONV && d->ksize == 1 && std::isinf(d->codomain);
}
static bool pi_stale_v(const InfPowerIterDesc* d) {
  return d->kind == INF_LAYER_CONV && d->ksize == 1 && d->domain == 1.f;
}
static size_t pi_align(size_t b) { return (b + 255) / 256 * 256; }
static size_t pi_layer_bytes(const InfPowerIterDesc* d) {
  const PIOp op = pi_op(d);
  const size_t nu = (size_t)pi_nu(op), nv = (size_t)pi_nv(op);
  return pi_align((nu + nv) * sizeof(float)) + pi_align(PI_SCR * sizeof(double)) +
         (pi_stale_u(d) ? pi_align(nu * sizeof(float)) : 0) + (pi_stale_v(d) ? pi_align(nv * sizeof(float)) : 0);
}

struct PILayer {
  PIOp op;
  long nu, nv;
  PINorm nmu, nmv;
  float *us, *vs;
  float *u, *v;
  double* scr;
};
static int pi_layer_setup(const InfPowerIterDesc* d, char* cur, PILayer* l, hipStream_t s) {
  l->op = pi_op(d);
  l->nu = pi_nu(l->op);
  l->nv = pi_nv(l->op);
  l->nmu = pi_norm_of(d->codomain, true);
  l->nmv = pi_norm_of(d->domain, false);
  l->us = reinterpret_cast<float*>(cur);
  l->vs = l->us + l->nu;
  cur += pi_align((size_t)(l->nu + l->nv) * sizeof(float));
  l->scr = reinterpret_cast<double*>(cur);
  cur += pi_align(PI_SCR * sizeof(double));
  l->u = d->u;
  l->v = d->v;
  if (pi_stale_u(d)) {
    l->u = reinterpret_cast<float*>(cur);
    cur += pi_align((size_t)l->nu * sizeof(float));
    INF_HIP(hipMemcpyAsync(l->u, d->u, (size_t)l->nu * sizeof(float), hipMemcpyDeviceToDevice, s));
  }
  if (pi_stale_v(d)) {
    l->v = reinterpret_cast<float*>(cur);
    INF_HIP(hipMemcpyAsync(l->v, d->v, (size_t)l->nv * sizeof(float), hipMemcpyDeviceToDevice, s));
  }
  return INF_OK;
}
static void pi_launch_iteration(const PILayer& l, PIState* st, hipStream_t s) {
  pi_launch_w(l.op, l.v, l.us, st, s);
  pi_launch_normalize(l.us, l.u, l.nu, st, 0, l.nmu, l.scr, s);
  pi_launch_wt(l.op, l.u, l.vs, st, s);
  pi_launch_normalize(l.vs, l.v, l.nv, st, 1, l.nmv, l.scr, s);
}
static void pi_launch_sigma(const PILayer& l, PIState* st, float* scale, hipStream_t s) {
  pi_launch_w(l.op, l.v, l.us, nullptr, s);
  if (l.nu < PI_MULTI_MIN) {
    hipLaunchKernelGGL(pi_sigma, dim3(1), dim3(1024), 0, s, l.u, l.us, l.nu, st, scale);
  } else {
    hipLaunchKernelGGL(pi_dot_part, dim3(PI_NB), dim3(256), 0, s, l.u, l.us, l.nu, nullptr, l.scr);
    hipLaunchKernelGGL(pi_sigma_final, dim3(1), dim3(256), 0, s, l.scr, PI_NB, st, scale);
  }
}

}

using namespace inf;

extern "C" {

size_t inf_power_iteration_workspace_bytes(const InfPowerIterDesc* d) {
  if (!pi_valid(d)) return 0;
  return 256 + pi_layer_bytes(d);
}

int inf_power_iteration(const InfPowerIterDesc* d, int max_iters, int use_tol, float atol, float rtol,
                        int* iters_used, void* ws, size_t ws_bytes, void* stream) {
  if (!pi_valid(d) || max_iters < 0) return INF_ERR_INVALID;
  if (!ws || ws_bytes < inf_power_iteration_workspace_bytes(d)) return INF_ERR_WORKSPACE;
  hipStream_t s = (hipStream_t)stream;
  char* base = reinterpret_cast<char*>(ws);
  PIState* st = reinterpret_cast<PIState*>(base);
  PILayer l;
  INF_TRY(pi_layer_setup(d, base + 256, &l, s));
  PIState h;
  memset(&h, 0, sizeof(h));
  hipLaunchKernelGGL(pi_init, dim3(1), dim3(1), 0, s, st, use_tol ? 1 : 0, atol, rtol);
  int done_iters = 0, chunk = use_tol ? 2 : max_iters;
  while (done_iters < max_iters) {
    const int n = std::min(chunk, max_iters - done_iters);
    for (int k = 0; k < n; ++k) pi_launch_iteration(l, st, s);
    INF_CHECK_LAUNCH();
    done_iters += n;
    chunk = std::min(2 * chunk, 8);
    if (!use_tol) continue;
    INF_HIP(hipMemcpyAsync(&h, st, sizeof(h), hipMemcpyDeviceToHost, s));
    INF_HIP(hipStreamSynchronize(s));
    if (h.done) break;
  }
  pi_launch_sigma(l, st, d->scale, s);
  INF_CHECK_LAUNCH();
  if (iters_used) *iters_used = use_tol ? h.iters : max_iters;
  return INF_OK;
}

size_t inf_power_iteration_batch_workspace_bytes(const InfPowerIterDesc* descs, int n) {
  if (!descs || n <= 0) return 0;
  size_t b = ((sizeof(PIState) * (size_t)n + 255) / 256) * 256;
  for (int i = 0; i < n; ++i) {
    if (!pi_valid(&descs[i])) return 0;
    b += pi_layer_bytes(&descs[i]);
  }
  return b;
}

int inf_power_iteration_batch(const InfPowerIterDesc* descs, int n, int max_iters, int use_tol, float atol,
                              float rtol, int* iters_used, void* ws, size_t ws_bytes, void* stream) {
  if (!descs || n <= 0 || max_iters < 0) return INF_ERR_INVALID;
  for (int i = 0; i < n; ++i)
    if (!pi_valid(&descs[i])) return INF_ERR_INVALID;
  if (!ws || ws_bytes < inf_power_iteration_batch_workspace_bytes(descs, n)) return INF_ERR_WORKSPACE;
  hipStream_t s = (hipStream_t)stream;
  char* base = reinterpret_cast<char*>(ws);
  PIState* states = reinterpret_cast<PIState*>(base);
  char* cur = base + ((sizeof(PIState) * (size_t)n + 255) / 256) * 256;
  std::vector<PILayer> L(n);
  for (int i = 0; i < n; ++i) {
    INF_TRY(pi_layer_setup(&descs[i], cur, &L[i], s));
    cur += pi_layer_bytes(&descs[i]);
    hipLaunchKernelGGL(pi_init, dim3(1), dim3(1), 0, s, states + i, use_tol ? 1 : 0, atol, rtol);
  }
  std::vector<PIState> h(n);
  memset(h.data(), 0, sizeof(PIState) * n);
  std::vector<char> live(n, 1);
  int done_iters = 0, chunk = use_tol ? 2 : max_iters;
  while (done_iters < max_iters) {
    const int c = std::min(chunk, max_iters - done_iters);
    for (int i = 0; i < n; ++i) {
      if (!live[i]) continue;
      for (int k = 0; k < c; ++k) pi_launch_iteration(L[i], states + i, s);
    }
    INF_CHECK_LAUNCH();
    done_iters += c;
    chunk = std::min(2 * chunk, 8);
    if (!use_tol) continue;
    INF_HIP(hipMemcpyAsync(h.data(), states, sizeof(PIState) * n, hipMemcpyDeviceToHost, s));
    INF_HIP(hipStreamSynchronize(s));
    bool any = false;
    for (int i = 0; i < n; ++i) {
      if (h[i].done) live[i] = 0;
      any = any || live[i];
    }
    if (!any) break;
  }
  for (int i = 0; i < n; ++i) pi_launch_sigma(L[i], states + i, descs[i].scale, s);
  INF_CHECK_LAUNCH();
  if (iters_used)
    for (int i = 0; i < n; ++i) iters_used[i] = use_tol ? h[i].iters : max_iters;
  return INF_OK;
}

}
```

implicit-normalizing-flows_amd/lib/_hip/__init__.py:

```python
import atexit
import ctypes
import os
import threading
import weakref

import torch

_HERE = os.path.dirname(os.path.abspath(__file__))
LIB_PATH = os.path.join(_HERE, 'libinflow.so')
LIB_PATH = os.environ.get('INFLOW_LIB') or LIB_PATH

INF_LAYER_CONV, INF_LAYER_LINEAR, INF_ACT_SWISH, INF_ACT_SIN = 1, 2, 3, 4
INF_ACT_ELU, INF_ACT_SOFTPLUS, INF_ACT_RELU, INF_ACT_LCUBE, INF_ACT_IDENTITY, INF_ACT_ZERO = 5, 6, 7, 8, 9, 10
INF_ERR_UNSUPPORTED = 4
INF_OPT_FUSED_K128, INF_OPT_EVAL_OVERLAP, INF_OPT_CONVERGENCE, INF_OPT_K128_EXACT_SCALE = 1, 2, 3, 4
INF_OPT_FC_BLOCK, INF_OPT_FC_SERIES, INF_OPT_LINE_SEARCH, INF_OPT_FUSED_PRESPLIT = 5, 6, 7, 8
INF_OPT_FC_SKINNY = 9
INF_CONV_GLOBAL, INF_CONV_PER_SAMPLE = 0, 1
CONVERGENCE = {'global': INF_CONV_GLOBAL, 'per_sample': INF_CONV_PER_SAMPLE}


class PowerIterDesc(ctypes.Structure):
    _fields_ = [('kind', ctypes.c_int), ('cin', ctypes.c_int), ('cout', ctypes.c_int), ('ksize', ctypes.c_int),
                ('height', ctypes.c_int), ('width', ctypes.c_int), ('weight', ctypes.c_void_p),
                ('u', ctypes.c_void_p), ('v', ctypes.c_void_p), ('scale', ctypes.c_void_p),
                ('domain', ctypes.c_float), ('codomain', ctypes.c_float)]


class NetGrads(ctypes.Structure):
    _fields_ = [('dW', ctypes.POINTER(ctypes.c_void_p)), ('db', ctypes.POINTER(ctypes.c_void_p)),
                ('dbeta', ctypes.POINTER(ctypes.c_void_p)), ('dpre_beta', ctypes.c_void_p)]


class LayerDesc(ctypes.Structure):
    _fields_ = [('kind', ctypes.c_int), ('cin', ctypes.c_int), ('cout', ctypes.c_int), ('ksize', ctypes.c_int),
                ('weight', ctypes.c_void_p), ('bias', ctypes.c_void_p), ('u', ctypes.c_void_p),
                ('v', ctypes.c_void_p), ('coeff', ctypes.c_float), ('beta', ctypes.c_void_p)]


class NetDesc(ctypes.Structure):
    _fields_ = [('n_layers', ctypes.c_int), ('layers', ctypes.POINTER(LayerDesc)), ('channels', ctypes.c_int),
                ('height', ctypes.c_int), ('width', ctypes.c_int)]


class BroydenStats(ctypes.Structure):
    _fields_ = [('nstep', ctypes.c_int), ('lowest_step', ctypes.c_int), ('prot_break', ctypes.c_int),
                ('n_trace', ctypes.c_int), ('trace', ctypes.c_double * 64), ('diff', ctypes.c_double),
                ('eps', ctypes.c_double), ('fixed_point_iters', ctypes.c_int), ('convergence', ctypes.c_int),
                ('sample_nstep', ctypes.POINTER(ctypes.c_int)), ('sample_lowest_step', ctypes.POINTER(ctypes.c_int)),
                ('sample_prot_break', ctypes.POINTER(ctypes.c_int)), ('tnstep', ctypes.c_int)]

    def want_samples(self, batch):
        self._samples = [(ctypes.c_int * batch)() for _ in range(3)]
        self.sample_nstep, self.sample_lowest_step, self.sample_prot_break = [
            ctypes.cast(a, ctypes.POINTER(ctypes.c_int)) for a in self._samples]
        return self

    def as_dict(self, threshold):
        d = {'nstep': self.nstep, 'tnstep': self.tnstep, 'lowest_step': self.lowest_step,
             'diff': self.diff, 'prot_break': bool(self.prot_break),
             'trace': [self.trace[i] for i in range(self.n_trace)], 'eps': self.eps,
             'threshold': threshold, 'fixed_point_iters': self.fixed_point_iters,
             'convergence': 'per_sample' if self.convergence == INF_CONV_PER_SAMPLE else 'global'}
        if self.convergence == INF_CONV_PER_SAMPLE and getattr(self, '_samples', None):
            d['sample_nstep'], d['sample_lowest_step'], d['sample_prot_break'] = [list(a) for a in self._samples]
        return d


class KernelStat(ctypes.Structure):
    _fields_ = [('tag', ctypes.c_int), ('launches', ctypes.c_int), ('total_ms', ctypes.c_double),
                ('flops', ctypes.c_double), ('bytes', ctypes.c_double), ('peak_ms', ctypes.c_double)]


class HipError(RuntimeError):
    pass


_lib = None
_lock = threading.Lock()

_P = ctypes.c_void_p
_SIGS = {
    'inf_version': (ctypes.c_int, []),
    'inf_shutdown': (ctypes.c_int, []),
    'inf_status_string': (ctypes.c_char_p, [ctypes.c_int]),
    'inf_last_hip_error': (ctypes.c_int, []),
    'inf_net_create': (ctypes.c_int, [ctypes.POINTER(NetDesc), ctypes.POINTER(_P)]),
    'inf_net_destroy': (ctypes.c_int, [_P]),
    'inf_net_refresh': (ctypes.c_int, [_P, _P]),
    'inf_net_set_tensors': (ctypes.c_int, [_P, ctypes.POINTER(NetDesc)]),
    'inf_net_set_mfma': (ctypes.c_int, [_P, ctypes.c_int]),
    'inf_net_get_mfma': (ctypes.c_int, [_P]),
    'inf_workspace_bytes': (ctypes.c_size_t, [_P, ctypes.c_int, ctypes.c_int]),
    'inf_net_forward': (ctypes.c_int, [_P, _P, _P, ctypes.c_int, _P, ctypes.c_size_t, _P]),
    'inf_net_vjp': (ctypes.c_int, [_P, _P, _P, _P, ctypes.c_int, _P, ctypes.c_size_t, _P]),
    'inf_root_find': (ctypes.c_int, [_P, _P, _P, _P, ctypes.c_int, ctypes.c_int, ctypes.c_double,
                                     ctypes.POINTER(BroydenStats), _P, _P, ctypes.c_size_t, _P]),
    'inf_imblock_eval': (ctypes.c_int, [_P, _P, _P, _P, _P, _P, ctypes.POINTER(ctypes.c_float), ctypes.c_int, _P, _P,
                                        ctypes.c_int, ctypes.c_int, ctypes.c_double, ctypes.POINTER(BroydenStats), _P,
                                        ctypes.c_size_t, _P]),
    'inf_imblock_eval_exact': (ctypes.c_int, [_P, _P, _P, _P, _P, _P, ctypes.c_int, ctypes.c_int, ctypes.c_double,
                                              ctypes.POINTER(BroydenStats), _P, ctypes.c_size_t, _P]),
    'inf_flow_chain_workspace_bytes': (ctypes.c_size_t, [ctypes.POINTER(_P), ctypes.c_int, ctypes.c_int,
                                                         ctypes.POINTER(ctypes.c_int)]),
    'inf_flow_eval_exact_chain': (ctypes.c_int, [ctypes.POINTER(_P), ctypes.POINTER(_P), ctypes.c_int, _P, _P, _P, _P,
                                                 ctypes.c_int, ctypes.POINTER(ctypes.c_int),
                                                 ctypes.POINTER(ctypes.c_double), ctypes.POINTER(BroydenStats), _P,
                                                 ctypes.c_size_t, _P]),
    'inf_imblock_backward': (ctypes.c_int, [_P, _P, _P, _P, _P, _P, _P, ctypes.c_int, ctypes.c_int, ctypes.c_double,
                                            ctypes.POINTER(BroydenStats), _P, ctypes.c_size_t, _P]),
    'inf_imblock_forward': (ctypes.c_int, [_P, _P, _P, _P, ctypes.c_int, ctypes.c_int, ctypes.c_double,
                                           ctypes.POINTER(BroydenStats), _P, ctypes.c_size_t, _P]),
    'inf_broyden_workspace_bytes': (ctypes.c_size_t, [ctypes.c_int, ctypes.c_int, ctypes.c_int]),
    'inf_broyden_update': (ctypes.c_int, [_P, _P, _P, _P, _P, _P, _P, _P, _P, ctypes.c_int, ctypes.c_int,
                                          ctypes.c_int, ctypes.c_int, _P, ctypes.c_size_t, _P]),
    'inf_broyden_line_step': (ctypes.c_int, [_P, _P, ctypes.c_float, _P, _P, ctypes.c_size_t, _P]),
    'inf_logdet_series': (ctypes.c_int, [_P, _P, _P, ctypes.POINTER(ctypes.c_float), ctypes.c_int, _P,
                                         ctypes.c_int, _P, ctypes.c_size_t, _P]),
    'inf_logdet_series_pair': (ctypes.c_int, [_P, _P, _P, _P, _P, _P, ctypes.POINTER(ctypes.c_float), ctypes.c_int,
                                              _P, _P, ctypes.c_int, _P, ctypes.c_size_t, _P]),
    'inf_logdet_neumann': (ctypes.c_int, [_P, _P, _P, ctypes.POINTER(ctypes.c_float), ctypes.c_int, _P,
                                          ctypes.c_int, _P, ctypes.c_size_t, _P]),
    'inf_neumann_vector': (ctypes.c_int, [_P, _P, _P, ctypes.POINTER(ctypes.c_float), ctypes.c_int, _P,
                                          ctypes.c_int, _P, ctypes.c_size_t, _P]),
    'inf_neumann_vector_pair': (ctypes.c_int, [_P, _P, _P, _P, _P, _P, ctypes.POINTER(ctypes.c_float), ctypes.c_int,
                                               _P, _P, ctypes.c_int, _P, ctypes.c_size_t, _P]),
    'inf_logdet_exact': (ctypes.c_int, [_P, _P, _P, ctypes.c_int, _P, ctypes.c_size_t, _P]),
    'inf_logdet_exact_trace': (ctypes.c_int, [_P, _P, ctypes.POINTER(ctypes.c_float), ctypes.c_int, _P, ctypes.c_int,
                                              _P, ctypes.c_size_t, _P]),
    'inf_logit_forward': (ctypes.c_int, [_P, _P, _P, _P, ctypes.c_int, ctypes.c_int, ctypes.c_float, _P]),
    'inf_actnorm_forward': (ctypes.c_int, [_P, _P, _P, _P, _P, _P, ctypes.c_int, ctypes.c_int, ctypes.c_int, _P]),
    'inf_squeeze2': (ctypes.c_int, [_P, _P, ctypes.c_int, ctypes.c_int, ctypes.c_int, ctypes.c_int, _P]),
    'inf_normal_logprob': (ctypes.c_int, [_P, _P, ctypes.c_int, ctypes.c_int, _P]),
    'inf_profile_begin': (ctypes.c_int, [ctypes.c_int]),
    'inf_profile_end': (ctypes.c_int, [ctypes.POINTER(KernelStat), ctypes.c_int, ctypes.POINTER(ctypes.c_int)]),
    'inf_rademacher': (ctypes.c_int, [_P, ctypes.c_size_t, ctypes.c_uint64, ctypes.c_uint64, _P]),
    'inf_debug_poison_lds': (ctypes.c_int, [_P]),
    'inf_debug_readback_check': (ctypes.c_int, [ctypes.c_int, ctypes.c_int, _P]),
    'inf_net_set_option': (ctypes.c_int, [_P, ctypes.c_int, ctypes.c_int]),
    'inf_net_get_option': (ctypes.c_int, [_P, ctypes.c_int]),
    'inf_banach_find_root': (ctypes.c_int, [_P, _P, _P, _P, ctypes.c_int, ctypes.c_int, ctypes.c_double,
                                            ctypes.POINTER(ctypes.c_int), _P, ctypes.c_size_t, _P]),
    'inf_grad_workspace_bytes': (ctypes.c_size_t, [_P, ctypes.c_int]),
    'inf_logdet_grad_workspace_bytes': (ctypes.c_size_t, [_P, ctypes.c_int, ctypes.c_int, ctypes.c_int]),
    'inf_logdet_grad': (ctypes.c_int, [_P, _P, ctypes.c_int, _P, ctypes.POINTER(ctypes.c_float), ctypes.c_int, _P, _P,
                                       _P, ctypes.POINTER(NetGrads), ctypes.c_int, _P, ctypes.c_size_t, _P]),
    'inf_net_param_grad': (ctypes.c_int, [_P, _P, _P, _P, ctypes.POINTER(NetGrads), ctypes.c_int, _P, ctypes.c_size_t,
                                          _P]),
    'inf_net_surrogate_grad': (ctypes.c_int, [_P, _P, _P, _P, _P, _P, ctypes.POINTER(NetGrads), ctypes.c_int, _P,
                                              ctypes.c_size_t, _P]),
    'inf_power_iteration_workspace_bytes': (ctypes.c_size_t, [ctypes.POINTER(PowerIterDesc)]),
    'inf_power_iteration': (ctypes.c_int, [ctypes.POINTER(PowerIterDesc), ctypes.c_int, ctypes.c_int, ctypes.c_float,
                                           ctypes.c_float, ctypes.POINTER(ctypes.c_int), _P, ctypes.c_size_t, _P]),
    'inf_power_iteration_batch_workspace_bytes': (ctypes.c_size_t, [ctypes.POINTER(PowerIterDesc), ctypes.c_int]),
    'inf_power_iteration_batch': (ctypes.c_int, [ctypes.POINTER(PowerIterDesc), ctypes.c_int, ctypes.c_int,
                                                 ctypes.c_int, ctypes.c_float, ctypes.c_float,
                                                 ctypes.POINTER(ctypes.c_int), _P, ctypes.c_size_t, _P]),
}
EXPORTS = tuple(_SIGS)


def load(path=LIB_PATH):
    global _lib
    with _lock:
        if _lib is None:
            if not os.path.exists(path):
                raise HipError('libinflow.so is not built (%s); run __graft_entry__.build()' % path)
            lib = ctypes.CDLL(path)
            for name, (res, args) in _SIGS.items():
                fn = getattr(lib, name)
                fn.restype = res
                fn.argtypes = args
            _lib = lib
            atexit.register(_shutdown)
        return _lib


def _shutdown():
    if _lib is not None and torch.cuda.is_initialized():
        _lib.inf_shutdown()


def check(status, what):
    if status != 0:
        lib = load()
        msg = lib.inf_status_string(status).decode()
        raise HipError('%s failed: %s (status %d, hip error %d)' % (what, msg, status, lib.inf_last_hip_error()))


def ptr(t):
    return ctypes.c_void_p(t.data_ptr()) if t is not None else ctypes.c_void_p(0)


def stream_of(t):
    idx = t.device.index
    return ctypes.c_void_p(_raw_stream(idx if idx is not None else torch.cuda.current_device()))


def _raw_stream_slow(idx):
    return torch.cuda.current_stream(idx).cuda_stream


_raw_stream = getattr(torch._C, '_cuda_getCurrentRawStream', _raw_stream_slow)


def require_device(t, who):
    if not (isinstance(t, torch.Tensor) and t.is_cuda):
        raise HipError('%s runs on the MI355X engine (libinflow.so) and needs a HIP device tensor; got %s'
                       % (who, 'a CPU tensor' if isinstance(t, torch.Tensor) else type(t).__name__))
    if t.dtype != torch.float32:
        raise HipError('%s: fp32 tensors only (got %s)' % (who, t.dtype))


_ws = {}


def workspace(device, nbytes):
    idx = torch.device(device).index if torch.device(device).index is not None else torch.cuda.current_device()
    key = (idx, torch.cuda.current_stream(idx).cuda_stream)
    buf = _ws.get(key)
    if buf is None or buf.numel() < nbytes:
        buf = torch.empty(int(nbytes * 1.1) + 4096, dtype=torch.uint8, device=device)
        _ws[key] = buf
    return buf


class NativeNet:

    created = 0
    refreshed = 0

    def __init__(self, entries, shape, device):
        self.lib = load()
        self.device = device
        self.shape = tuple(shape)
        nd, self._tensors, keep = self._desc(entries)
        h = ctypes.c_void_p()
        with torch.cuda.device(device):
            check(self.lib.inf_net_create(ctypes.byref(nd), ctypes.byref(h)), 'inf_net_create')
        NativeNet.created += 1
        self.handle = h
        self._stamp = None
        self._lock = threading.Lock()
        self.value_source = None
        self.holder = None
        self.ptrs = self.current_ptrs()

    def _desc(self, entries):
        tensors, descs = [], []
        for kind, m in entries:
            d = LayerDesc()
            d.kind = kind
            if kind in (INF_LAYER_CONV, INF_LAYER_LINEAR):
                w = m.weight
                d.cin, d.cout = int(w.shape[1]), int(w.shape[0])
                d.ksize = int(w.shape[2]) if kind == INF_LAYER_CONV else 1
                d.weight, d.bias, d.u, d.v = ptr(w), ptr(m.bias), ptr(m.u), ptr(m.v)
                d.coeff = float(m.coeff)
                tensors += [t for t in (w, m.bias, m.u, m.v) if t is not None]
            elif kind == INF_ACT_SWISH:
                d.beta = ptr(m.beta)
                tensors.append(m.beta)
            descs.append(d)
        arr = (LayerDesc * len(descs))(*descs)
        nd = NetDesc()
        nd.n_layers = len(descs)
        nd.layers = arr
        if len(self.shape) == 3:
            nd.channels, nd.height, nd.width = self.shape
        else:
            nd.channels, nd.height, nd.width = self.shape[0], 1, 1
        return nd, tensors, arr

    def retarget(self, entries):
        nd, tensors, keep = self._desc(entries)
        check(self.lib.inf_net_set_tensors(self.handle, ctypes.byref(nd)), 'inf_net_set_tensors')
        self._tensors = tensors
        self.ptrs = self.current_ptrs()

    def current_ptrs(self):
        return tuple(t.data_ptr() for t in self._tensors)

    @staticmethod
    def _tensors_of(entries):
        out = []
        for kind, m in entries:
            if kind in (INF_LAYER_CONV, INF_LAYER_LINEAR):
                out += [t for t in (m.weight, m.bias, m.u, m.v) if t is not None]
            elif kind == INF_ACT_SWISH:
                out.append(m.beta)
        return out

    def stamp(self):
        return tuple((t.data_ptr(), t._version) for t in self._tensors)

    def refresh_if_needed(self, stream):
        with self._lock:
            st = self.value_source() if self.value_source is not None else self.stamp()
            if st != self._stamp:
                check(self.lib.inf_net_refresh(self.handle, stream), 'inf_net_refresh')
                NativeNet.refreshed += 1
                self._stamp = st

    def set_option(self, option, value):
        prev = self.lib.inf_net_set_option(self.handle, int(option), int(value))
        if prev < 0:
            raise HipError('inf_net_set_option(%d, %d): invalid option or value' % (option, value))
# ... 189 lines not shown
```

implicit-normalizing-flows_amd/lib/implicit_flow.py:

```python
import numpy as np
import torch
import torch.nn as nn

from . import layers
from .layers import base as base_layers

ACT_FNS = {
    'softplus': lambda b: nn.Softplus(),
    'elu': lambda b: nn.ELU(inplace=b),
    'swish': lambda b: base_layers.Swish(),
    'lcube': lambda b: base_layers.LipschitzCube(),
    'identity': lambda b: base_layers.Identity(),
    'relu': lambda b: nn.ReLU(inplace=b),
    'sin': lambda b: base_layers.Sin(),
    'zero': lambda b: base_layers.Zero(),
}


def _parse_vnorms(vnorms):
    ps = [float('inf') if p == 'f' else float(p) for p in vnorms]
    return ps[:-1], ps[1:]


class FCNet(nn.Module):

    def __init__(self, input_shape, idim, lipschitz_layer, nhidden, coeff, domains, codomains, n_iterations,
                 activation_fn, preact, dropout, sn_atol, sn_rtol, learn_p, div_in=1):
        super().__init__()
        if dropout or learn_p:
            raise NotImplementedError('dropout / learn_p are not provided')
        self.input_shape = input_shape
        dim = int(np.prod(input_shape))
        mods = [ACT_FNS[activation_fn](False)] if preact else []
        last = dim // div_in
        for i in range(nhidden):
            mods.append(lipschitz_layer(last, idim, coeff=coeff, n_iterations=n_iterations, domain=domains[i],
                                        codomain=codomains[i], atol=sn_atol, rtol=sn_rtol))
            mods.append(ACT_FNS[activation_fn](True))
            last = idim
        mods.append(lipschitz_layer(last, dim, coeff=coeff, n_iterations=n_iterations, domain=domains[-1],
                                    codomain=codomains[-1], atol=sn_atol, rtol=sn_rtol))
        self.nnet = nn.Sequential(*mods)

    def forward(self, x, restore=False):
        y = self.nnet(x.view(x.shape[0], -1))
        return y.view(y.shape[0], *self.input_shape)


class FCWrapper(nn.Module):

    def __init__(self, fc_module):
        super().__init__()
        self.fc_module = fc_module

    def forward(self, x, logpx=None, restore=False):
        shape = x.shape
        out = self.fc_module(x.reshape(shape[0], -1), logpx) if logpx is not None else self.fc_module(
            x.reshape(shape[0], -1))
        if logpx is None:
            return out.view(*shape)
        return out[0].view(*shape), out[1]

    def inverse(self, y, logpy=None):
        shape = y.shape
        if logpy is None:
            return self.fc_module.inverse(y.reshape(shape[0], -1)).view(*shape)
        x, logpx = self.fc_module.inverse(y.reshape(shape[0], -1), logpy)
        return x.view(*shape), logpx


class StackedImplicitBlocks(layers.SequentialFlow):

    def __init__(self, initial_size, idim, squeeze=True, init_layer=None, n_blocks=1, quadratic=False, actnorm=False,
                 fc_actnorm=False, batchnorm=False, dropout=0, fc=False, coeff=0.9, vnorms='122f',
                 n_lipschitz_iters=None, sn_atol=None, sn_rtol=None, n_power_series=5, n_dist='geometric',
                 n_samples=1, kernels='3-1-3', activation_fn='elu', fc_end=True, fc_nblocks=2, fc_idim=128,
                 n_exact_terms=0, preact=False, neumann_grad=True, grad_in_forward=False, first_resblock=True,
                 learn_p=False):
        if quadratic or batchnorm or dropout or learn_p:
            raise NotImplementedError('quadratic / batchnorm / dropout / learn_p are not provided')
        domains, codomains = _parse_vnorms(vnorms)
        ks = list(map(int, kernels.split('-')))
        assert len(domains) == len(ks)
        block_kw = dict(n_power_series=n_power_series, n_dist=n_dist, n_samples=n_samples,
                        n_exact_terms=n_exact_terms, neumann_grad=neumann_grad, grad_in_forward=grad_in_forward)

        def actnorm_layer(as_fc):
# ... 18 lines not shown

        def block(as_fc, first, width=idim):
            if as_fc:
                return layers.imBlock(fc_net(width), fc_net(width), **block_kw)
            return layers.imBlock(conv_net(first), conv_net(first), **block_kw)

        chain = []
        if init_layer is not None:
            chain.append(init_layer)
        if first_resblock and actnorm:
            chain.append(actnorm_layer(fc))
        if first_resblock and fc_actnorm:
            chain.append(actnorm_layer(True))
        for i in range(n_blocks):
            chain.append(block(fc, first_resblock and i == 0))
            if actnorm:
                chain.append(actnorm_layer(fc))
            if fc_actnorm:
                chain.append(actnorm_layer(True))
        if squeeze:
            chain.append(layers.SqueezeLayer(2))
        elif fc_end:
            for _ in range(fc_nblocks):
                chain.append(block(True, False, fc_idim))
                if actnorm or fc_actnorm:
                    chain.append(actnorm_layer(True))
        super().__init__(chain)


class ImplicitFlow(nn.Module):

    def __init__(self, input_size, n_blocks=[16, 16], intermediate_dim=64, factor_out=True, quadratic=False,
                 init_layer=None, actnorm=False, fc_actnorm=False, batchnorm=False, dropout=0, fc=False, coeff=0.9,
                 vnorms='122f', n_lipschitz_iters=None, sn_atol=None, sn_rtol=None, n_power_series=5,
                 n_dist='geometric', n_samples=1, kernels='3-1-3', activation_fn='elu', fc_end=True, fc_idim=128,
                 n_exact_terms=0, preact=False, neumann_grad=True, grad_in_forward=False, first_resblock=True,
                 learn_p=False, classification=False, classification_hdim=64, n_classes=10):
        super().__init__()
        if classification:
            raise NotImplementedError('classification heads are outside the density-evaluation path')
        _, c, h, w = input_size
        n_scale, hh, ww = 0, h, w
        while hh >= 4 and ww >= 4:
            n_scale, hh, ww = n_scale + 1, hh // 2, ww // 2
        self.n_scale = min(len(n_blocks), n_scale)
        if not self.n_scale > 0:
            raise ValueError('Could not compute number of scales for input of size (%d,%d,%d,%d)' % input_size)
        self.n_blocks = n_blocks
        self.factor_out = factor_out
        self.init_layer = init_layer
        common = dict(idim=intermediate_dim, quadratic=quadratic, actnorm=actnorm, fc_actnorm=fc_actnorm,
                      batchnorm=batchnorm, dropout=dropout, fc=fc, coeff=coeff, vnorms=vnorms,
                      n_lipschitz_iters=n_lipschitz_iters, sn_atol=sn_atol, sn_rtol=sn_rtol,
                      n_power_series=n_power_series, n_dist=n_dist, n_samples=n_samples, kernels=kernels,
                      activation_fn=activation_fn, fc_end=fc_end, fc_idim=fc_idim, n_exact_terms=n_exact_terms,
                      preact=preact, neumann_grad=neumann_grad, grad_in_forward=grad_in_forward, learn_p=learn_p)
        scales = []
        for i in range(self.n_scale):
            scales.append(StackedImplicitBlocks(initial_size=(c, h, w), squeeze=(i < self.n_scale - 1),
                                                init_layer=init_layer if i == 0 else None, n_blocks=n_blocks[i],
                                                first_resblock=first_resblock and i == 0, **common))
            c, h, w = (c * 2 if factor_out else c * 4), h // 2, w // 2
        self.transforms = nn.ModuleList(scales)
        self.dims = [o[1:] for o in self.calc_output_size(input_size)]

    def calc_output_size(self, input_size):
        n, c, h, w = input_size
        if not self.factor_out:
            k = self.n_scale - 1
            return [[n, c * 4 ** k, h // 2 ** k, w // 2 ** k]]
        sizes = []
        for i in range(self.n_scale):
            if i < self.n_scale - 1:
                c, h, w = c * 2, h // 2, w // 2
            sizes.append((n, c, h, w))
        return tuple(sizes)

    def forward(self, x, logpx=None, inverse=False, classify=False, restore=False):
        if inverse:
            return self.inverse(x, logpx)
        if classify:
            raise NotImplementedError('classification heads are outside the density-evaluation path')
        factored = []
        for idx, stage in enumerate(self.transforms):
            if logpx is not None:
                x, logpx = stage(x, logpx, restore=restore)
            else:
                x = stage(x, restore=restore)
            if self.factor_out and idx < len(self.transforms) - 1:
                half = x.size(1) // 2
                x, f = x[:, :half], x[:, half:]
                factored.append(f)
        factored.append(x)
        out = torch.cat([o.reshape(o.size(0), -1) for o in factored], 1)
        return out if logpx is None else (out, logpx)

    def inverse(self, z, logpz=None):
        if self.factor_out:
            z = z.view(z.shape[0], -1)
            parts, i = [], 0
            for dims in self.dims:
                s = int(np.prod(dims))
                parts.append(z[:, i:i + s].view(z.shape[0], *dims))
                i += s
            z_prev = parts[-1]
            for idx in range(len(self.transforms) - 1, -1, -1):
                if idx < len(self.transforms) - 1:
                    z_prev = torch.cat((z_prev, parts[idx]), dim=1)
                if logpz is None:
                    z_prev = self.transforms[idx].inverse(z_prev)
                else:
                    z_prev, logpz = self.transforms[idx].inverse(z_prev, logpz)
            return z_prev if logpz is None else (z_prev, logpz)
        z = z.view(z.shape[0], *self.dims[-1])
        for idx in range(len(self.transforms) - 1, -1, -1):
            if logpz is None:
                z = self.transforms[idx].inverse(z)
            else:
                z, logpz = self.transforms[idx].inverse(z, logpz)
        return z if logpz is None else (z, logpz)
```

implicit-normalizing-flows_amd/lib/layers/flows.py:

```python
import math

import torch
import torch.nn as nn

from .. import _hip

__all__ = ['SequentialFlow', 'Inverse', 'SqueezeLayer', 'ActNorm1d', 'ActNorm2d', 'LogitTransform',
           'ZeroMeanTransform', 'Normalize']


def _logp_tensor(logpx, B, device):
    if logpx is None:
        return None
    if torch.is_tensor(logpx):
        return logpx.reshape(B).contiguous().to(device=device, dtype=torch.float32)
    return torch.full((B,), float(logpx), device=device)


class SequentialFlow(nn.Module):

    def __init__(self, layersList):
        super().__init__()
        self.chain = nn.ModuleList(layersList)

    def forward(self, x, logpx=None, restore=False):
        if logpx is not None and not restore and not self.training and x.is_cuda:
            from .imblock import eval_exact_chain
            out = eval_exact_chain(list(self.chain), x, logpx, owner=self)
            if out is not None:
                return out
        if logpx is None:
            for layer in self.chain:
                x = layer(x, restore=restore)
            return x
        for layer in self.chain:
            x, logpx = layer(x, logpx, restore=restore)
        return x, logpx

    def inverse(self, y, logpy=None):
        for layer in reversed(self.chain):
            if logpy is None:
                y = layer.inverse(y)
            else:
                y, logpy = layer.inverse(y, logpy)
        return y if logpy is None else (y, logpy)


class Inverse(nn.Module):

    def __init__(self, flow):
        super().__init__()
        self.flow = flow

    def forward(self, x, logpx=None):
        return self.flow.inverse(x, logpx)

    def inverse(self, y, logpy=None):
        return self.flow.forward(y, logpy)


def _graph(*ts):
    return torch.is_grad_enabled() and any(t is not None and t.requires_grad for t in ts)


def squeeze(x, downscale_factor=2):
    if downscale_factor == 2 and x.is_cuda and x.dtype == torch.float32 and not _graph(x):
        B, C, H, W = x.shape
        x = x.contiguous()
        y = torch.empty(B, 4 * C, H // 2, W // 2, device=x.device)
        _hip.check(_hip.load().inf_squeeze2(_hip.ptr(x), _hip.ptr(y), B, C, H, W, _hip.stream_of(x)), 'inf_squeeze2')
        return y
    B, C, H, W = x.shape
    r = downscale_factor
    return x.reshape(B, C, H // r, r, W // r, r).permute(0, 1, 3, 5, 2, 4).reshape(B, C * r * r, H // r, W // r)


def unsqueeze(x, upscale_factor=2):
    return torch.pixel_shuffle(x, upscale_factor)


class SqueezeLayer(nn.Module):

    def __init__(self, downscale_factor):
        super().__init__()
        self.downscale_factor = downscale_factor

    def forward(self, x, logpx=None, restore=False):
        y = squeeze(x, self.downscale_factor)
        return y if logpx is None else (y, logpx)

    def inverse(self, y, logpy=None):
        x = unsqueeze(y, self.downscale_factor)
        return x if logpy is None else (x, logpy)


class _ActNorm(nn.Module):
    view_shape = None

    def __init__(self, num_features, eps=1e-12):
        super().__init__()
        self.num_features = num_features
        self.eps = eps
        self.weight = nn.Parameter(torch.Tensor(num_features))
        self.bias = nn.Parameter(torch.Tensor(num_features))
        self.register_buffer('initialized', torch.tensor(0))

    def _load_from_state_dict(self, *args, **kwargs):
        self.__dict__['_init_seen'] = False
        super()._load_from_state_dict(*args, **kwargs)

    def _data_init(self, x):
        with torch.no_grad():
            c = x.size(1)
            xt = x.transpose(0, 1).contiguous().view(c, -1)
            var = torch.max(torch.var(xt, dim=1), torch.tensor(0.2).to(xt))
            self.bias.data.copy_(-torch.mean(xt, dim=1))
            self.weight.data.copy_(-0.5 * torch.log(var))
            self.initialized.fill_(1)

    def forward(self, x, logpx=None, restore=None):
        if not self.__dict__.get('_init_seen', False):
            if not self.initialized:
                self._data_init(x)
            self.__dict__['_init_seen'] = True
        B, C = x.shape[0], x.shape[1]
        hw = x[0, 0].numel()
        lgraph = logpx if torch.is_tensor(logpx) else None
        if x.is_cuda and x.dtype == torch.float32 and not _graph(x, self.weight, self.bias, lgraph):
            x = x.contiguous()
            y = torch.empty_like(x)
            lin = _logp_tensor(logpx, B, x.device)
            lout = torch.empty(B, device=x.device) if logpx is not None else None
            _hip.check(_hip.load().inf_actnorm_forward(
                _hip.ptr(x), _hip.ptr(y), _hip.ptr(self.weight), _hip.ptr(self.bias), _hip.ptr(lin),
                _hip.ptr(lout), B, C, hw, _hip.stream_of(x)), 'inf_actnorm_forward')
            return y if logpx is None else (y, lout.view(B, 1))
        shape = [1, -1] + [1] * (x.dim() - 2)
        y = (x + self.bias.view(*shape)) * torch.exp(self.weight.view(*shape))
        return y if logpx is None else (y, logpx - self._logdetgrad(x))

    def inverse(self, y, logpy=None):
        shape = [1, -1] + [1] * (y.dim() - 2)
        x = y * torch.exp(-self.weight.view(*shape)) - self.bias.view(*shape)
        return x if logpy is None else (x, logpy + self._logdetgrad(x))

    def _logdetgrad(self, x):
        return (self.weight.sum() * x[0, 0].numel()).expand(x.shape[0], 1)

    def __repr__(self):
        return '%s(%d)' % (type(self).__name__, self.num_features)


class ActNorm1d(_ActNorm):
    pass


class ActNorm2d(_ActNorm):
    pass


class LogitTransform(nn.Module):

    def __init__(self, alpha=1e-6):
        super().__init__()
        self.alpha = alpha

    def forward(self, x, logpx=None, restore=False):
        B = x.shape[0]
        lgraph = logpx if torch.is_tensor(logpx) else None
        if x.is_cuda and x.dtype == torch.float32 and not _graph(x, lgraph):
            x = x.contiguous()
            y = torch.empty_like(x)
            lin = _logp_tensor(logpx, B, x.device)
            lout = torch.empty(B, device=x.device)
            _hip.check(_hip.load().inf_logit_forward(_hip.ptr(x), _hip.ptr(y), _hip.ptr(lin), _hip.ptr(lout), B,
                                                     x[0].numel(), float(self.alpha), _hip.stream_of(x)),
                       'inf_logit_forward')
            return y if logpx is None else (y, lout.view(B, 1))
        s = self.alpha + (1 - 2 * self.alpha) * x
        y = torch.log(s) - torch.log(1 - s)
        return y if logpx is None else (y, logpx - self._logdetgrad(x).view(B, -1).sum(1, keepdim=True))

    def inverse(self, y, logpy=None):
        x = (torch.sigmoid(y) - self.alpha) / (1 - 2 * self.alpha)
        if logpy is None:
            return x
        return x, logpy + self._logdetgrad(x).view(x.size(0), -1).sum(1, keepdim=True)

    def _logdetgrad(self, x):
        s = self.alpha + (1 - 2 * self.alpha) * x
        return -torch.log(s - s * s) + math.log(1 - 2 * self.alpha)

    def __repr__(self):
        return 'LogitTransform(%s)' % self.alpha


class ZeroMeanTransform(nn.Module):

    def forward(self, x, logpx=None, restore=False):
        return x - .5 if logpx is None else (x - .5, logpx)

    def inverse(self, y, logpy=None):
        return y + .5 if logpy is None else (y + .5, logpy)


class Normalize(nn.Module):

    def __init__(self, mean, std):
        super().__init__()
        self.register_buffer('mean', torch.as_tensor(mean, dtype=torch.float32))
        self.register_buffer('std', torch.as_tensor(std, dtype=torch.float32))

    def _per_channel(self, t):
        return t.view(1, -1, 1, 1)

    def _logdetgrad(self, x):
        hw = x[0, 0].numel()
        return (-hw * self.std.abs().log().sum()).expand(x.shape[0], 1)

    def forward(self, x, logpx=None, restore=False):
        c = self.mean.numel()
        y = x.clone()
        y[:, :c] = (x[:, :c] - self._per_channel(self.mean)) / self._per_channel(self.std)
        return y if logpx is None else (y, logpx - self._logdetgrad(x))

    def inverse(self, y, logpy=None):
        c = self.mean.numel()
        x = y.clone()
        x[:, :c] = y[:, :c] * self._per_channel(self.std) + self._per_channel(self.mean)
        return x if logpy is None else (x, logpy + self._logdetgrad(x))
```

implicit-normalizing-flows_amd/lib/layers/imblock.py:

```python
import copy
import ctypes
import math

import numpy as np
import torch
import torch.nn as nn

from .. import _hip
from . import netgrad, solvers

__all__ = ['imBlock', 'set_probe_mode', 'set_probe_shard', 'set_convergence', 'RootFind']

_PROBES = {'mode': 'reference', 'seed': 0, 'offset': 0, 'shard': None}
_SOLVE = {'convergence': 'global'}
_MFMA_F16X3 = 2
_JAC_MAX = 16
WIDE_FC_GRADS = True


def set_probe_mode(mode, seed=0):
    if mode not in ('reference', 'device'):
        raise ValueError(mode)
    _PROBES.update(mode=mode, seed=int(seed), offset=0)

# ... 486 lines not shown
        if key not in self.__dict__:
            allowed = (('InducedNormConv2d', 'Swish', 'Sin') if t.dim() == 4
                       else ('InducedNormLinear', 'Swish', 'Sin'))
            ok = True
            for net in (self.nnet_x, self.nnet_z):
                for m in net.modules():
                    if isinstance(m, nn.Sequential):
                        continue
                    if type(m).__name__ not in allowed:
                        ok = False
            self.__dict__[key] = ok
        return self.__dict__[key]

    def _net_forward(self, native, t):
        B = t.shape[0]
        ws = _hip.workspace(t.device, native.ws_bytes(B))
        y = torch.empty_like(t)
        _hip.check(_hip.load().inf_net_forward(native.handle, _hip.ptr(t.contiguous()), _hip.ptr(y), B, _hip.ptr(ws),
                                               ws.numel(), _hip.stream_of(t)), 'inf_net_forward')
        return y

    @staticmethod
    def _neumann_coeffs(n_ps, coeff_fn):
        nco = np.zeros(n_ps + 1, dtype=np.float32)
        nco[0] = 1.
        for k in range(1, n_ps + 1):
            nco[k] = (-1) ** k * coeff_fn(k)
        return nco

    def _neumann_pair(self, na, ta, ea, nb, tb, eb, n_ps, coeff_fn, stream):
        B = ta.shape[0]
        nco = self._neumann_coeffs(n_ps, coeff_fn)
        wa, wb = torch.empty_like(ta), torch.empty_like(tb)
        ws = _hip.workspace(ta.device, 2 * max(na.ws_bytes(B), nb.ws_bytes(B)))
        half = ws.numel() // 2
        _hip.check(_hip.load().inf_neumann_vector_pair(
            na.handle, _hip.ptr(ta.contiguous()), _hip.ptr(ea), nb.handle, _hip.ptr(tb.contiguous()), _hip.ptr(eb),
            nco.ctypes.data_as(ctypes.POINTER(ctypes.c_float)), n_ps, _hip.ptr(wa), _hip.ptr(wb), B, _hip.ptr(ws),
            2 * half, stream), 'inf_neumann_vector_pair')
        return wa, wb

    def _neumann_vector(self, native, t, eps, n_ps, coeff_fn, stream):
        B = t.shape[0]
        nco = np.zeros(n_ps + 1, dtype=np.float32)
        nco[0] = 1.
        for k in range(1, n_ps + 1):
            nco[k] = (-1) ** k * coeff_fn(k)
        w = torch.empty_like(t)
        ws = _hip.workspace(t.device, native.ws_bytes(B))
        _hip.check(_hip.load().inf_neumann_vector(native.handle, _hip.ptr(t.contiguous()), _hip.ptr(eps),
                                                  nco.ctypes.data_as(ctypes.POINTER(ctypes.c_float)), n_ps,
                                                  _hip.ptr(w), B, _hip.ptr(ws), ws.numel(), stream),
                   'inf_neumann_vector')
        return w

    def _root(self, net_f, net_e, y, eps, stream, forward):
        lib = _hip.load()
        y = y.contiguous()
        B = y.shape[0]
        T = int(self.threshold)
        ws = _hip.workspace(y.device, max(net_f.ws_bytes(B, T), net_e.ws_bytes(B, T)))
        out = torch.empty_like(y)
        st = _stats(B, (net_f,))
        if forward:
            rc = lib.inf_imblock_forward(net_e.handle, net_f.handle, _hip.ptr(y), _hip.ptr(out), B, T, float(eps),
                                         ctypes.byref(st), _hip.ptr(ws), ws.numel(), stream)
            _hip.check(rc, 'inf_imblock_forward')
        else:
            rc = lib.inf_root_find(net_f.handle, net_e.handle, _hip.ptr(y), _hip.ptr(out), B, T, float(eps),
                                   ctypes.byref(st), None, _hip.ptr(ws), ws.numel(), stream)
            _hip.check(rc, 'inf_root_find')
        self.last_broyden = st.as_dict(T)
        return out

    def forward(self, x, logpx=None, restore=False):
        if _needs_graph(self, x):
            return self._forward_graph(x, logpx, restore)
        if restore:
            with torch.no_grad():
                self.nnet_x_copy(x)
                self.nnet_z_copy(x)
        nx, nz, stream = self._native(x)
        if logpx is not None and not self.training and not self.exact_trace and x.dim() == 4:
            out = self._eval_fused(nx, nz, x, stream)
            if out is not None:
                return out[0], logpx - out[1]
        if logpx is not None and not self.training and x.dim() == 2 and x.shape[1] <= 10:
            out = self._eval_exact(nx, nz, x, stream)
            if out is not None:
                return out[0], logpx - out[1]
        with torch.no_grad():
            z = self._root(nz, nx, x, self.eps_forward, stream, forward=True)
        if self.training:
            self._refresh_copies()
        if logpx is None:
            return z
        return z, logpx - self._logdetgrad(z, x)

    def _eval_exact(self, nx, nz, x, stream):
        x = x.contiguous()
        B, T = x.shape[0], int(self.threshold)
        ws = _hip.workspace(x.device, nz.ws_bytes(B, T))
        z = torch.empty_like(x)
        out = torch.empty(2, B, device=x.device)
        st = _stats(B, (nz,))
        rc = _hip.load().inf_imblock_eval_exact(nx.handle, nz.handle, _hip.ptr(x), _hip.ptr(z), _hip.ptr(out[0]),
                                                _hip.ptr(out[1]), B, T, float(self.eps_forward), ctypes.byref(st),
                                                _hip.ptr(ws), ws.numel(), stream)
        if rc == _hip.INF_ERR_UNSUPPORTED:
            return None
        _hip.check(rc, 'inf_imblock_eval_exact')
        self.last_broyden = st.as_dict(T)
        return z, (out[0] - out[1]).view(-1, 1)

    def _eval_fused(self, nx, nz, x, stream):
        lib = _hip.load()
        x = x.contiguous()
        B, T = x.shape[0], int(self.threshold)
        plan = self._series_plan()
        n_ps, coeff_fn, ns = plan
        probes = (_probes(x.shape, x.device), _probes(x.shape, x.device))
        co = solvers.logdet_coefficients(n_ps, coeff_fn)
        ws = _hip.workspace(x.device, nx.ws_bytes(B, T) + nz.ws_bytes(B, 1) + nx.ws_bytes(B, 1))
        z = torch.empty_like(x)
        out = torch.empty(2, B, device=x.device)
        st = _stats(B, (nz,))
        rc = lib.inf_imblock_eval(nx.handle, nz.handle, _hip.ptr(x), _hip.ptr(z), _hip.ptr(probes[0]),
                                  _hip.ptr(probes[1]), co.ctypes.data_as(ctypes.POINTER(ctypes.c_float)), n_ps,
                                  _hip.ptr(out[0]), _hip.ptr(out[1]), B, T, float(self.eps_forward), ctypes.byref(st),
                                  _hip.ptr(ws), ws.numel(), stream)
        if rc == _hip.INF_ERR_UNSUPPORTED:
            with torch.no_grad():
                z = self._root(nz, nx, x, self.eps_forward, stream, forward=True)
            return z, self._logdetgrad(z, x, plan=plan, probes=probes)
        _hip.check(rc, 'inf_imblock_eval')
        self.last_broyden = st.as_dict(T)
        return z, self._finish_logdet(out[0] - out[1], n_ps, ns)

    def inverse(self, z, logpy=None):
        nx, nz, stream = self._native(z)
        with torch.no_grad():
            x = self._root(nx, nz, z, self.eps_sample, stream, forward=False)
        if logpy is None:
            return x
        return x, logpy + self._logdetgrad(z, x)

    def _refresh_copies(self):
        groups = {}
        for net, cp in ((self.nnet_x, self.nnet_x_copy), (self.nnet_z, self.nnet_z_copy)):
            src, dst = net.state_dict(keep_vars=True), cp.state_dict(keep_vars=True)
            for k, t in src.items():
                d = dst[k]
                key = (d.device, d.dtype, t.device, t.dtype)
                g = groups.setdefault(key, ([], []))
                g[0].append(d)
                g[1].append(t.detach())
        with torch.no_grad():
            for (dd, ddt, sd, sdt), (dsts, srcs) in groups.items():
                if dd == sd and ddt == sdt and dd.type != 'cpu':
                    torch._foreach_copy_(dsts, srcs)
                else:
                    for a, b in zip(dsts, srcs):
                        a.copy_(b)

    def _host_scalar(self, name, t, fn=None):
        key = (t.data_ptr(), t._version, t.device)
        cache = self.__dict__.setdefault('_host_scalars', {})
        if cache.get(name, (None,))[0] != key:
            with torch.no_grad():
                cache[name] = (key, (fn(t) if fn is not None else t).item())
        return cache[name][1]

    def _series_plan(self):
        if self.n_dist == 'geometric':
            param = self._host_scalar('geom_p', self.geom_p, torch.sigmoid)
        elif self.n_dist == 'poisson':
            param = self._host_scalar('lamb', self.lamb)
        else:
            raise ValueError(self.n_dist)
        if self.training and self.n_power_series is not None:
            return self.n_power_series, (lambda k: 1.), None
        n_exact = self.n_exact_terms if self.training else self.n_exact_terms_test
        return solvers.series_coefficients(self.n_dist, param, n_exact, self.n_samples)

    def _logdetgrad(self, z, x, plan=None, probes=None):
        lib = _hip.load()
        nx, nz, stream = self._native(x)
        B = x.shape[0]
        if (self.brute_force or not self.training) and x.dim() == 2 and x.shape[1] <= 10:
            out = torch.empty(2, B, device=x.device)
            ws = _hip.workspace(x.device, max(nx.ws_bytes(B), nz.ws_bytes(B)))
            for i, (net, t) in enumerate(((nx, x), (nz, z))):
                _hip.check(lib.inf_logdet_exact(net.handle, _hip.ptr(t.contiguous()), _hip.ptr(out[i]), B,
                                                _hip.ptr(ws), ws.numel(), stream), 'inf_logdet_exact')
            return (out[0] - out[1]).view(-1, 1)
        n_ps, coeff_fn, ns = plan if plan is not None else self._series_plan()
        if self.exact_trace:
            if x.dim() != 2:
                raise NotImplementedError('exact_trace=True needs the full Jacobian; supported for fc nets (d <= 16)')
            logdetgrad = (solvers.exact_trace_logdet(nx, x, n_ps, coeff_fn, stream) -
                          solvers.exact_trace_logdet(nz, z, n_ps, coeff_fn, stream))
            return self._finish_logdet(logdetgrad, n_ps, ns)
        if probes is not None:
            vareps_x, vareps_z = probes
        else:
            vareps_x = _probes(x.shape, x.device)
            vareps_z = _probes(z.shape, z.device)
        ws = _hip.workspace(x.device, max(nx.ws_bytes(B), nz.ws_bytes(B)))
        out = torch.empty(2, B, device=x.device)
        if self.training and self.neumann_grad:
            nco = np.zeros(n_ps + 1, dtype=np.float32)
            nco[0] = 1.
            for k in range(1, n_ps + 1):
                nco[k] = (-1) ** k * coeff_fn(k)
            carr = nco.ctypes.data_as(ctypes.POINTER(ctypes.c_float))
            for i, (net, t, e) in enumerate(((nx, x, vareps_x), (nz, z, vareps_z))):
                _hip.check(lib.inf_logdet_neumann(net.handle, _hip.ptr(t.contiguous()), _hip.ptr(e), carr, n_ps,
                                                  _hip.ptr(out[i]), B, _hip.ptr(ws), ws.numel(), stream),
                           'inf_logdet_neumann')
        else:
            co = solvers.logdet_coefficients(n_ps, coeff_fn)
            carr = co.ctypes.data_as(ctypes.POINTER(ctypes.c_float))
# ... 21 lines not shown
```

include/inflow.h:

```cpp
#ifndef INFLOW_H
#define INFLOW_H

#include <stddef.h>
#include <stdint.h>

#ifdef __cplusplus
extern "C" {
#endif

typedef enum InfStatus {
  INF_OK = 0,
  INF_ERR_INVALID = 1,
  INF_ERR_HIP = 2,
  INF_ERR_WORKSPACE = 3,
  INF_ERR_UNSUPPORTED = 4
} InfStatus;

typedef enum InfLayerKind {
  INF_LAYER_CONV = 1,
  INF_LAYER_LINEAR = 2,
  INF_ACT_SWISH = 3,
  INF_ACT_SIN = 4,
  INF_ACT_ELU = 5,
  INF_ACT_SOFTPLUS = 6,
  INF_ACT_RELU = 7,
  INF_ACT_LCUBE = 8,
  INF_ACT_IDENTITY = 9,
  INF_ACT_ZERO = 10
} InfLayerKind;

typedef struct InfLayerDesc {
  int kind;
  int cin, cout, ksize;
  const float* weight;
  const float* bias;
  const float* u;
  const float* v;
  float coeff;
  const float* beta;
} InfLayerDesc;

typedef struct InfNetDesc {
  int n_layers;
  const InfLayerDesc* layers;
  int channels, height, width;
} InfNetDesc;

typedef struct InfNet InfNet;

typedef struct InfBroydenStats {
  int nstep;
  int lowest_step;
  int prot_break;
  int n_trace;
  double trace[64];
  double diff;
  double eps;
  int fixed_point_iters;
  int convergence;
  int* sample_nstep;
  int* sample_lowest_step;
  int* sample_prot_break;
  int tnstep;
} InfBroydenStats;

int inf_version(void);
int inf_shutdown(void);
const char* inf_status_string(int status);
int inf_last_hip_error(void);

int inf_net_create(const InfNetDesc* desc, InfNet** out);
int inf_net_destroy(InfNet* net);
int inf_net_refresh(InfNet* net, void* stream);
int inf_net_set_tensors(InfNet* net, const InfNetDesc* desc);
typedef enum InfMfmaMode { INF_MFMA_F32 = 0, INF_MFMA_BF16X6 = 1, INF_MFMA_F16X3 = 2 } InfMfmaMode;
int inf_net_set_mfma(InfNet* net, int mode);
int inf_net_get_mfma(const InfNet* net);
typedef enum InfNetOption {
  INF_OPT_FUSED_K128 = 1, INF_OPT_EVAL_OVERLAP = 2, INF_OPT_CONVERGENCE = 3, INF_OPT_K128_EXACT_SCALE = 4,
  INF_OPT_FC_BLOCK = 5, INF_OPT_FC_SERIES = 6, INF_OPT_LINE_SEARCH = 7, INF_OPT_FUSED_PRESPLIT = 8,
  INF_OPT_FC_SKINNY = 9
} InfNetOption;
typedef enum InfConvergence { INF_CONV_GLOBAL = 0, INF_CONV_PER_SAMPLE = 1 } InfConvergence;
int inf_net_set_option(InfNet* net, int option, int value);
int inf_net_get_option(const InfNet* net, int option);
size_t inf_workspace_bytes(const InfNet* net, int batch, int threshold);
int inf_net_forward(InfNet* net, const float* x, float* y, int batch, void* ws, size_t ws_bytes, void* stream);
int inf_net_vjp(InfNet* net, const float* x, const float* v, float* out, int batch, void* ws, size_t ws_bytes,
                void* stream);

int inf_root_find(InfNet* net_f, InfNet* net_e, const float* y, float* out, int batch, int threshold, double eps,
                  InfBroydenStats* stats, float* diff_detail, void* ws, size_t ws_bytes, void* stream);
int inf_banach_find_root(InfNet* net_f, InfNet* net_e, const float* y, float* out, int batch, int threshold,
                         double eps, int* iters, void* ws, size_t ws_bytes, void* stream);
size_t inf_broyden_workspace_bytes(int batch, int d, int threshold);
int inf_broyden_update(float* U, float* VT, const float* dx, const float* dg, const float* gx, const float* x,
                       float* update, float* x_next, float* dx_next, int batch, int d, int threshold, int nstep,
                       void* ws, size_t ws_bytes, void* stream);
int inf_broyden_line_step(const float* x0, const float* update, float step, float* x_est, float* dx, size_t n,
                          void* stream);
int inf_imblock_forward(InfNet* net_x, InfNet* net_z, const float* x, float* z, int batch, int threshold,
                        double eps, InfBroydenStats* stats, void* ws, size_t ws_bytes, void* stream);

int inf_logdet_series(InfNet* net, const float* x, const float* vareps, const float* coeff, int n_terms,
                      float* out, int batch, void* ws, size_t ws_bytes, void* stream);
int inf_logdet_series_pair(InfNet* net_a, const float* x_a, const float* vareps_a, InfNet* net_b, const float* x_b,
                           const float* vareps_b, const float* coeff, int n_terms, float* out_a, float* out_b,
                           int batch, void* ws, size_t ws_bytes, void* stream);
int inf_imblock_eval(InfNet* net_x, InfNet* net_z, const float* x, float* z, const float* eps_x, const float* eps_z,
                     const float* coeff, int n_terms, float* logdet_x, float* logdet_z, int batch, int threshold,
                     double eps, InfBroydenStats* stats, void* ws, size_t ws_bytes, void* stream);
int inf_imblock_eval_exact(InfNet* net_x, InfNet* net_z, const float* x, float* z, float* logdet_x, float* logdet_z,
                           int batch, int threshold, double eps, InfBroydenStats* stats, void* ws, size_t ws_bytes,
                           void* stream);
size_t inf_flow_chain_workspace_bytes(InfNet* const* net_z, int n_blocks, int batch, const int* thresholds);
int inf_flow_eval_exact_chain(InfNet* const* net_x, InfNet* const* net_z, int n_blocks, const float* x, float* z,
                              const float* logp_in, float* logp_out, int batch, const int* thresholds,
                              const double* eps, InfBroydenStats* stats, void* ws, size_t ws_bytes, void* stream);
int inf_logdet_neumann(InfNet* net, const float* x, const float* vareps, const float* ncoeff, int n_terms,
                       float* out, int batch, void* ws, size_t ws_bytes, void* stream);
int inf_neumann_vector(InfNet* net, const float* x, const float* vareps, const float* ncoeff, int n_terms, float* w,
                       int batch, void* ws, size_t ws_bytes, void* stream);
int inf_neumann_vector_pair(InfNet* net_a, const float* x_a, const float* vareps_a, InfNet* net_b, const float* x_b,
                            const float* vareps_b, const float* ncoeff, int n_terms, float* w_a, float* w_b,
                            int batch, void* ws, size_t ws_bytes, void* stream);
int inf_logdet_exact(InfNet* net, const float* x, float* out, int batch, void* ws, size_t ws_bytes, void* stream);
int inf_imblock_backward(InfNet* net_x, InfNet* net_z, const float* z, const float* x, const float* grad,
                         float* dl_dh, float* dl_dx, int batch, int threshold, double eps, InfBroydenStats* stats,
                         void* ws, size_t ws_bytes, void* stream);
int inf_logdet_exact_trace(InfNet* net, const float* x, const float* coeff, int n_terms, float* out, int batch,
                           void* ws, size_t ws_bytes, void* stream);

int inf_logit_forward(const float* x, float* y, const float* logp_in, float* logp_out, int batch, int per_sample,
                      float alpha, void* stream);
int inf_actnorm_forward(const float* x, float* y, const float* weight, const float* bias, const float* logp_in,
                        float* logp_out, int batch, int channels, int hw, void* stream);
int inf_squeeze2(const float* x, float* y, int batch, int channels, int height, int width, void* stream);
int inf_normal_logprob(const float* z, float* out, int batch, int per_sample, void* stream);
int inf_rademacher(float* out, size_t n, uint64_t seed, uint64_t offset, void* stream);

typedef struct InfKernelStat {
  int tag;
  int launches;
  double total_ms;
  double flops;
  double bytes;
  double peak_ms;
} InfKernelStat;
int inf_profile_begin(int max_launches);
int inf_profile_end(InfKernelStat* out, int max_out, int* n_out);

typedef struct InfPowerIterDesc {
  int kind;
  int cin, cout, ksize;
  int height, width;
  const float* weight;
  float* u;
  float* v;
  float* scale;
  float domain, codomain;
} InfPowerIterDesc;
size_t inf_power_iteration_workspace_bytes(const InfPowerIterDesc* desc);
int inf_power_iteration(const InfPowerIterDesc* desc, int max_iters, int use_tol, float atol, float rtol,
                        int* iters_used, void* ws, size_t ws_bytes, void* stream);
size_t inf_power_iteration_batch_workspace_bytes(const InfPowerIterDesc* descs, int n);
int inf_power_iteration_batch(const InfPowerIterDesc* descs, int n, int max_iters, int use_tol, float atol,
                              float rtol, int* iters_used, void* ws, size_t ws_bytes, void* stream);

typedef struct InfNetGrads {
  float** dW;
  float** db;
  float** dbeta;
  float* dpre_beta;
} InfNetGrads;
size_t inf_grad_workspace_bytes(InfNet* net, int batch);
int inf_net_param_grad(InfNet* net, const float* x, const float* gout, float* gx, const InfNetGrads* grads,
                       int batch, void* ws, size_t ws_bytes, void* stream);
int inf_net_surrogate_grad(InfNet* net, const float* x, const float* w, const float* eps, float* value, float* gx,
                           const InfNetGrads* grads, int batch, void* ws, size_t ws_bytes, void* stream);

int inf_debug_poison_lds(void* stream);
int inf_debug_readback_check(int iters, int n, void* stream);

typedef enum InfLogdetMode { INF_LOGDET_SERIES = 0, INF_LOGDET_EXACT = 1, INF_LOGDET_TRACE = 2 } InfLogdetMode;
size_t inf_logdet_grad_workspace_bytes(InfNet* net, int batch, int mode, int n_terms);
int inf_logdet_grad(InfNet* net, const float* x, int mode, const float* eps, const float* coeff, int n_terms,
                    const float* gout, float* value, float* gx, const InfNetGrads* grads, int batch, void* ws,
                    size_t ws_bytes, void* stream);

#ifdef __cplusplus
}
#endif
#endif
```

Measured before the change: 3038 samples/s.

## Pipeline z-side logdet series across imblocks on a second side stream

Runs the z-side log-determinant power series of each implicit block on a new side stream, and returns before it finishes, so the next block's Broyden solve can overlap with it. Two rotating workspace slots with events guard against reusing buffers that are still in flight. logp accumulation (logp step, actnorm logp) is moved onto the side stream, and deferred tensors are kept alive until a join. Every other entry point now joins pending work first. This adds event and stream bookkeeping and a risk of races if any consumer forgets to join.

Measured after the change: 3063 samples/s (median of 6 runs). No clear change (+0.8%).

```diff
diff --git a/implicit-normalizing-flows_amd/csrc/engine.h b/implicit-normalizing-flows_amd/csrc/engine.h
--- a/implicit-normalizing-flows_amd/csrc/engine.h
+++ b/implicit-normalizing-flows_amd/csrc/engine.h
@@ -65,6 +65,7 @@
   int f0_batch = -1;
   int k128 = 1;
   int eval_overlap = 1;
+  int eval_pipeline = 1;
   int convergence = INF_CONV_GLOBAL;
   int line_search = 0;
   int exact_scale = 0;
@@ -185,5 +186,6 @@
 
 int fc_jacobian(InfNet* n, const float* x, int B, Bufs& bf, const float** tang, hipStream_t s);
 void logdet_release_thread();
+int eval_join_pending(hipStream_t s);
 
 }
diff --git a/implicit-normalizing-flows_amd/csrc/engine_chain.hip b/implicit-normalizing-flows_amd/csrc/engine_chain.hip
--- a/implicit-normalizing-flows_amd/csrc/engine_chain.hip
+++ b/implicit-normalizing-flows_amd/csrc/engine_chain.hip
@@ -214,6 +214,7 @@
 extern "C" {
 
 int inf_net_forward(InfNet* n, const float* x, float* y, int B, void* ws, size_t ws_bytes, void* stream) {
+  INF_TRY(eval_join_pending((hipStream_t)stream));
   if (!n || !x || !y || B <= 0) return INF_ERR_INVALID;
   hipStream_t s = (hipStream_t)stream;
   Bufs bf;
@@ -230,6 +231,7 @@
 
 int inf_net_vjp(InfNet* n, const float* x, const float* v, float* out, int B, void* ws, size_t ws_bytes,
                 void* stream) {
+  INF_TRY(eval_join_pending((hipStream_t)stream));
   if (!n || !x || !v || !out || B <= 0) return INF_ERR_INVALID;
   hipStream_t s = (hipStream_t)stream;
   Bufs bf;
diff --git a/implicit-normalizing-flows_amd/csrc/engine_grad.hip b/implicit-normalizing-flows_amd/csrc/engine_grad.hip
--- a/implicit-normalizing-flows_amd/csrc/engine_grad.hip
+++ b/implicit-normalizing-flows_amd/csrc/engine_grad.hip
@@ -339,6 +339,7 @@
 
 int inf_net_param_grad(InfNet* n, const float* x, const float* gout, float* gx, const InfNetGrads* gr, int B,
                        void* ws, size_t ws_bytes, void* stream) {
+  INF_TRY(eval_join_pending((hipStream_t)stream));
   if (!n || !x || !gout || !gr || B <= 0) return INF_ERR_INVALID;
   if (!grad_supported(n)) return INF_ERR_UNSUPPORTED;
   hipStream_t s = (hipStream_t)stream;
@@ -354,6 +355,7 @@
 
 int inf_net_surrogate_grad(InfNet* n, const float* x, const float* w, const float* eps, float* value, float* gx,
                            const InfNetGrads* gr, int B, void* ws, size_t ws_bytes, void* stream) {
+  INF_TRY(eval_join_pending((hipStream_t)stream));
   if (!n || !x || !w || !eps || !gr || B <= 0) return INF_ERR_INVALID;
   if (!grad_supported(n) || (n->fc && value)) return INF_ERR_UNSUPPORTED;
   hipStream_t s = (hipStream_t)stream;
@@ -377,6 +379,7 @@
 int inf_logdet_grad(InfNet* n, const float* x, int mode, const float* eps, const float* coeff, int n_terms,
                     const float* gout, float* value, float* gx, const InfNetGrads* gr, int B, void* ws, size_t ws_bytes,
                     void* stream) {
+  INF_TRY(eval_join_pending((hipStream_t)stream));
   if (!n || !x || !gr || B <= 0 || mode < LOGDET_SERIES || mode > LOGDET_TRACE) return INF_ERR_INVALID;
   if (mode == LOGDET_SERIES && (!eps || !coeff || n_terms < 1 || n_terms > 128)) return INF_ERR_INVALID;
   if (mode == LOGDET_TRACE && (!coeff || n_terms < 1 || n_terms > 128)) return INF_ERR_INVALID;
diff --git a/implicit-normalizing-flows_amd/csrc/engine_logdet.hip b/implicit-normalizing-flows_amd/csrc/engine_logdet.hip
--- a/implicit-normalizing-flows_amd/csrc/engine_logdet.hip
+++ b/implicit-normalizing-flows_amd/csrc/engine_logdet.hip
@@ -67,9 +67,19 @@
   return INF_OK;
 }
 
+struct PipeSlot {
+  hipEvent_t done[2] = {nullptr, nullptr};
+  const char *lo = nullptr, *hi = nullptr;
+  bool live = false;
+};
 struct SideStream {
   hipStream_t s = nullptr;
   hipEvent_t fork = nullptr, join = nullptr;
+  hipStream_t sz = nullptr;
+  hipEvent_t zfork = nullptr, tail[2] = {nullptr, nullptr};
+  PipeSlot slot[2];
+  int next = 0;
+  bool active = false;
 };
 thread_local SideStream g_side[16];
 SideStream* side_stream() {
@@ -84,6 +94,52 @@
   }
   return &ss;
 }
+SideStream* pipe_streams() {
+  SideStream* ss = side_stream();
+  if (!ss || ss->sz) return ss;
+  hipEvent_t* evs[] = {&ss->zfork, &ss->tail[0], &ss->tail[1], &ss->slot[0].done[0], &ss->slot[0].done[1],
+                       &ss->slot[1].done[0], &ss->slot[1].done[1]};
+  for (hipEvent_t* e : evs)
+    if (!*e && hipEventCreateWithFlags(e, INF_EV_SYNC) != hipSuccess) return nullptr;
+  if (hipStreamCreateWithFlags(&ss->sz, hipStreamNonBlocking) != hipSuccess) {
+    ss->sz = nullptr;
+    return nullptr;
+  }
+  return ss;
+}
+SideStream* side_existing() {
+  int dev = 0;
+  if (hipGetDevice(&dev) != hipSuccess || dev < 0 || dev >= 16) return nullptr;
+  return g_side[dev].sz ? &g_side[dev] : nullptr;
+}
+int pipe_wait_slot(PipeSlot& sl, hipStream_t s) {
+  if (!sl.live) return INF_OK;
+  sl.live = false;
+  INF_HIP(hipStreamWaitEvent(s, sl.done[0], 0));
+  INF_HIP(hipStreamWaitEvent(s, sl.done[1], 0));
+  return INF_OK;
+}
+int pipe_join_all(SideStream* ss, hipStream_t s) {
+  if (!ss || !ss->active) return INF_OK;
+  ss->active = false;
+  ss->slot[0].live = ss->slot[1].live = false;
+  INF_HIP(hipEventRecord(ss->tail[0], ss->s));
+  INF_HIP(hipEventRecord(ss->tail[1], ss->sz));
+  INF_HIP(hipStreamWaitEvent(s, ss->tail[0], 0));
+  INF_HIP(hipStreamWaitEvent(s, ss->tail[1], 0));
+  return INF_OK;
+}
+int logp_stream(hipStream_t s, bool needs_x, hipStream_t* out) {
+  SideStream* ss = side_existing();
+  *out = s;
+  if (!ss || !ss->active) return INF_OK;
+  if (needs_x) {
+    INF_HIP(hipEventRecord(ss->tail[0], ss->s));
+    INF_HIP(hipStreamWaitEvent(ss->sz, ss->tail[0], 0));
+  }
+  *out = ss->sz;
+  return INF_OK;
+}
 
 struct SideJoin {
   SideStream* side = nullptr;
@@ -92,6 +148,13 @@
     if (!side) return;
     (void)hipEventRecord(side->join, side->s);
     (void)hipStreamWaitEvent(s, side->join, 0);
+  }
+};
+struct PipeJoin {
+  SideStream* side = nullptr;
+  hipStream_t s = nullptr;
+  ~PipeJoin() {
+    if (side) (void)pipe_join_all(side, s);
   }
 };
 
@@ -325,31 +388,55 @@
     if (!ss.s) continue;
     (void)hipSetDevice(dev);
     (void)hipStreamSynchronize(ss.s);
-    if (ss.fork) (void)hipEventDestroy(ss.fork);
-    if (ss.join) (void)hipEventDestroy(ss.join);
+    if (ss.sz) (void)hipStreamSynchronize(ss.sz);
+    hipEvent_t evs[] = {ss.fork, ss.join, ss.zfork, ss.tail[0], ss.tail[1], ss.slot[0].done[0], ss.slot[0].done[1],
+                        ss.slot[1].done[0], ss.slot[1].done[1]};
+    for (hipEvent_t e : evs)
+      if (e) (void)hipEventDestroy(e);
     (void)hipStreamDestroy(ss.s);
+    if (ss.sz) (void)hipStreamDestroy(ss.sz);
     ss = SideStream{};
   }
   (void)hipSetDevice(cur);
 }
+
+int inf::eval_join_pending(hipStream_t s) { return pipe_join_all(side_existing(), s); }
 
 extern "C" {
 
 int inf_imblock_eval(InfNet* nx, InfNet* nz, const float* x, float* z, const float* eps_x, const float* eps_z,
                      const float* coeff, int n_terms, float* logdet_x, float* logdet_z, int B, int T, double eps,
                      InfBroydenStats* stats, void* ws, size_t ws_bytes, void* stream) {
+  hipStream_t s = (hipStream_t)stream;
   if (!nx || !nz || !x || !z || !eps_x || !eps_z || !coeff || !logdet_x || !logdet_z || B <= 0 || T <= 0 || T > 64 ||
-      n_terms < 1 || n_terms > SERIES_MAX || !same_shape(nx, nz))
+      n_terms < 1 || n_terms > SERIES_MAX || !same_shape(nx, nz)) {
+    INF_TRY(eval_join_pending(s));
     return INF_ERR_INVALID;
-  if (!fused_pair(nx, nz)) return INF_ERR_UNSUPPORTED;
-  hipStream_t s = (hipStream_t)stream;
+  }
+  if (!fused_pair(nx, nz)) {
+    INF_TRY(eval_join_pending(s));
+    return INF_ERR_UNSUPPORTED;
+  }
   const size_t half = ws_need(nx, B, T), zneed = ws_need(nz, B, 1), xneed = ws_need(nx, B, 1);
+  const bool overlap = nx->eval_overlap && ws && ws_bytes >= half + zneed + xneed;
+  SideStream* pipe = nullptr;
+  if (overlap && nx->eval_pipeline) {
+    pipe = pipe_streams();
+    if (!pipe) return INF_ERR_HIP;
+  } else {
+    INF_TRY(eval_join_pending(s));
+  }
   if (!ws || ws_bytes < half + zneed) return INF_ERR_WORKSPACE;
   char* w0 = reinterpret_cast<char*>(ws);
+  const char* w1 = w0 + half + zneed + xneed;
+  if (pipe) {
+    for (PipeSlot& sl : pipe->slot)
+      if (sl.live && sl.lo < w1 && w0 < sl.hi) INF_TRY(pipe_wait_slot(sl, s));
+    INF_TRY(pipe_wait_slot(pipe->slot[pipe->next], s));
+  }
   Bufs bfa, bfb, bfc;
   carve(nx, B, T, w0, half, bfa);
   carve(nz, B, 1, w0 + half, zneed, bfb);
-  const bool overlap = nx->eval_overlap && ws_bytes >= half + zneed + xneed;
   if (overlap) {
     carve(nx, B, 1, w0 + half + zneed, xneed, bfc);
     bfc.D = bfa.D;
@@ -367,14 +454,22 @@
     INF_TRY(out_stage(nx, fused_taps(nx), OM_EMBED, a, bfa.Y, B, s));
   }
   SideJoin join;
+  PipeJoin pjoin;
   if (overlap) {
-    SideStream* side = side_stream();
+    SideStream* side = pipe ? pipe : side_stream();
     if (!side) return INF_ERR_HIP;
     INF_HIP(hipEventRecord(side->fork, s));
     INF_HIP(hipStreamWaitEvent(side->s, side->fork, 0));
-    join.side = side;
-    join.s = s;
+    if (pipe) {
+      pipe->active = true;
+      pjoin.side = pipe;
+      pjoin.s = s;
+    } else {
+      join.side = side;
+      join.s = s;
+    }
     INF_TRY(series_fused(&nx, &x, &eps_x, 1, coeff, n_terms, &logdet_x, B, &bfc, side->s, 0u));
+    if (pipe) INF_HIP(hipEventRecord(pipe->slot[pipe->next].done[0], side->s));
   }
   InfBroydenStats st = stats_for(stats);
   INF_TRY(broyden_solve(nz, x, B, T, eps, &st, nullptr, bfa, s));
@@ -389,6 +484,20 @@
     a.out0 = z;
     INF_TRY(run_forward(nz, bfa.lowest, B, bfa, OM_RECOMP, &a, s));
   }
+  if (pipe && !st.prot_break) {
+    PipeSlot& sl = pipe->slot[pipe->next];
+    const float* zin = z;
+    INF_HIP(hipEventRecord(pipe->zfork, s));
+    INF_HIP(hipStreamWaitEvent(pipe->sz, pipe->zfork, 0));
+    INF_TRY(series_fused(&nz, &zin, &eps_z, 1, coeff, n_terms, &logdet_z, B, &bfb, pipe->sz, 1u));
+    INF_HIP(hipEventRecord(sl.done[1], pipe->sz));
+    sl.lo = w0;
+    sl.hi = w1;
+    sl.live = true;
+    pipe->next ^= 1;
+    pjoin.side = nullptr;
+    return INF_OK;
+  }
   if (overlap) {
     const float* zin = z;
     return series_fused(&nz, &zin, &eps_z, 1, coeff, n_terms, &logdet_z, B, &bfb, s, 1u);
@@ -401,8 +510,30 @@
   return series_fused(nets, xs, es, 2, coeff, n_terms, outs, B, bfs, s, 2u);
 }
 
+int inf_eval_join(void* stream) { return eval_join_pending((hipStream_t)stream); }
+
+int inf_eval_pending(void) {
+  SideStream* ss = side_existing();
+  return ss && ss->active ? 1 : 0;
+}
+
+int inf_eval_logp_step(const float* lin, const float* logdet_x, const float* logdet_z, float* lout, int B,
+                       void* stream) {
+  if (!logdet_x || !logdet_z || !lout || B <= 0) return INF_ERR_INVALID;
+  hipStream_t t;
+  INF_TRY(logp_stream((hipStream_t)stream, true, &t));
+  return glue_logp_step(lin, logdet_x, logdet_z, lout, B, t);
+}
+int inf_eval_actnorm_logp(const float* w, const float* lin, float* lout, int B, int C, int hw, void* stream) {
+  if (!w || !lout || B <= 0 || C <= 0) return INF_ERR_INVALID;
+  hipStream_t t;
+  INF_TRY(logp_stream((hipStream_t)stream, false, &t));
+  return glue_actnorm_logp(w, lin, lout, B, C, hw, t);
+}
+
 int inf_imblock_eval_exact(InfNet* nx, InfNet* nz, const float* x, float* z, float* logdet_x, float* logdet_z, int B,
                            int T, double eps, InfBroydenStats* stats, void* ws, size_t ws_bytes, void* stream) {
+  INF_TRY(eval_join_pending((hipStream_t)stream));
   if (!nx || !nz || !x || !z || !logdet_x || !logdet_z || B <= 0 || T <= 0 || T > 64 || !same_shape(nx, nz))
     return INF_ERR_INVALID;
   INF_TRY(eval_exact_check(nx, nz, x, B));
@@ -423,6 +554,7 @@
 int inf_flow_eval_exact_chain(InfNet* const* net_x, InfNet* const* net_z, int n_blocks, const float* x, float* z,
                               const float* logp_in, float* logp_out, int B, const int* thresholds, const double* eps,
                               InfBroydenStats* stats, void* ws, size_t ws_bytes, void* stream) {
+  INF_TRY(eval_join_pending((hipStream_t)stream));
   if (!net_x || !net_z || n_blocks <= 0 || !x || !z || !logp_out || B <= 0 || !thresholds || !eps || x == z ||
       logp_in == logp_out)
     return INF_ERR_INVALID;
@@ -488,6 +620,7 @@
 
 int inf_logdet_series(InfNet* n, const float* x, const float* vareps, const float* coeff, int n_terms, float* out,
                       int B, void* ws, size_t ws_bytes, void* stream) {
+  INF_TRY(eval_join_pending((hipStream_t)stream));
   if (!n || !x || !vareps || !coeff || !out || B <= 0 || n_terms < 0 || n_terms > SERIES_MAX) return INF_ERR_INVALID;
   return series_single(n, x, vareps, coeff, n_terms, out, B, ws, ws_bytes, (hipStream_t)stream, true);
 }
@@ -495,6 +628,7 @@
 int inf_logdet_series_pair(InfNet* na, const float* xa, const float* ea, InfNet* nb, const float* xb, const float* eb,
                            const float* coeff, int n_terms, float* out_a, float* out_b, int B, void* ws,
                            size_t ws_bytes, void* stream) {
+  INF_TRY(eval_join_pending((hipStream_t)stream));
   if (!na || !nb || !xa || !xb || !ea || !eb || !coeff || !out_a || !out_b || B <= 0 || n_terms < 0 ||
       n_terms > SERIES_MAX || !same_shape(na, nb))
     return INF_ERR_INVALID;
@@ -527,6 +661,7 @@
 
 int inf_neumann_vector(InfNet* n, const float* x, const float* vareps, const float* ncoeff, int n_terms, float* w,
                        int B, void* ws, size_t ws_bytes, void* stream) {
+  INF_TRY(eval_join_pending((hipStream_t)stream));
   if (!n || !x || !vareps || !ncoeff || !w || B <= 0 || n_terms < 0) return INF_ERR_INVALID;
   hipStream_t s = (hipStream_t)stream;
   Bufs bf;
@@ -541,6 +676,7 @@
 int inf_neumann_vector_pair(InfNet* na, const float* xa, const float* ea, InfNet* nb, const float* xb,
                             const float* eb, const float* ncoeff, int n_terms, float* wa, float* wb, int B, void* ws,
                             size_t ws_bytes, void* stream) {
+  INF_TRY(eval_join_pending((hipStream_t)stream));
   if (!na || !nb || !xa || !xb || !ea || !eb || !ncoeff || !wa || !wb || B <= 0 || n_terms < 0 || !same_shape(na, nb))
     return INF_ERR_INVALID;
   const size_t half = ws_bytes / 2;
@@ -563,6 +699,7 @@
 
 int inf_logdet_neumann(InfNet* n, const float* x, const float* vareps, const float* ncoeff, int n_terms, float* out,
                        int B, void* ws, size_t ws_bytes, void* stream) {
+  INF_TRY(eval_join_pending((hipStream_t)stream));
   if (!n || !x || !vareps || !ncoeff || !out || B <= 0 || n_terms < 0) return INF_ERR_INVALID;
   hipStream_t s = (hipStream_t)stream;
   Bufs bf;
@@ -577,6 +714,7 @@
 }
 
 int inf_logdet_exact(InfNet* n, const float* x, float* out, int B, void* ws, size_t ws_bytes, void* stream) {
+  INF_TRY(eval_join_pending((hipStream_t)stream));
   if (!n || !x || !out || B <= 0) return INF_ERR_INVALID;
   if (!n->fc || n->d > 16 || n->pre_act != ACT_NONE) return INF_ERR_UNSUPPORTED;
   hipStream_t s = (hipStream_t)stream;
@@ -596,6 +734,7 @@
 
 int inf_logdet_exact_trace(InfNet* n, const float* x, const float* coeff, int n_terms, float* out, int B, void* ws,
                            size_t ws_bytes, void* stream) {
+  INF_TRY(eval_join_pending((hipStream_t)stream));
   if (!n || !x || !coeff || !out || B <= 0 || n_terms < 1 || n_terms > SERIES_MAX) return INF_ERR_INVALID;
   if (!n->fc || n->d > 16 || n->pre_act != ACT_NONE) return INF_ERR_UNSUPPORTED;
   hipStream_t s = (hipStream_t)stream;
diff --git a/implicit-normalizing-flows_amd/csrc/engine_plan.hip b/implicit-normalizing-flows_amd/csrc/engine_plan.hip
--- a/implicit-normalizing-flows_amd/csrc/engine_plan.hip
+++ b/implicit-normalizing-flows_amd/csrc/engine_plan.hip
@@ -59,6 +59,7 @@
 const NetOption OPTIONS[] = {
     {INF_OPT_FUSED_K128, &InfNet::k128, 3, "INFLOW_FUSED_K128", {"0", "1", "2", "3"}, true},
     {INF_OPT_EVAL_OVERLAP, &InfNet::eval_overlap, 1, "INFLOW_EVAL_OVERLAP", {"0", "1"}, false},
+    {INF_OPT_EVAL_PIPELINE, &InfNet::eval_pipeline, 1, nullptr, {}, false},
     {INF_OPT_CONVERGENCE, &InfNet::convergence, 1, "INFLOW_CONVERGENCE", {"global", "per_sample"}, false},
     {INF_OPT_LINE_SEARCH, &InfNet::line_search, 1, nullptr, {}, false},
     {INF_OPT_K128_EXACT_SCALE, &InfNet::exact_scale, 1, nullptr, {}, true},
@@ -428,6 +429,7 @@
 }
 
 int inf_net_refresh(InfNet* n, void* stream) {
+  INF_TRY(eval_join_pending((hipStream_t)stream));
   if (!n) return INF_ERR_INVALID;
   hipStream_t s = (hipStream_t)stream;
   n->f0_batch = -1;
diff --git a/implicit-normalizing-flows_amd/csrc/engine_solve.hip b/implicit-normalizing-flows_amd/csrc/engine_solve.hip
--- a/implicit-normalizing-flows_amd/csrc/engine_solve.hip
+++ b/implicit-normalizing-flows_amd/csrc/engine_solve.hip
@@ -850,6 +850,7 @@
 
 int inf_root_find(InfNet* f, InfNet* e, const float* y, float* out, int B, int T, double eps, InfBroydenStats* stats,
                   float* diff_detail, void* ws, size_t ws_bytes, void* stream) {
+  INF_TRY(eval_join_pending((hipStream_t)stream));
   if (!f || !e || !y || !out || B <= 0 || T <= 0 || T > 64 || !same_shape(f, e)) return INF_ERR_INVALID;
   hipStream_t s = (hipStream_t)stream;
   Bufs bf;
@@ -862,6 +863,7 @@
 
 int inf_imblock_forward(InfNet* nx, InfNet* nz, const float* x, float* z, int B, int T, double eps,
                         InfBroydenStats* stats, void* ws, size_t ws_bytes, void* stream) {
+  INF_TRY(eval_join_pending((hipStream_t)stream));
   if (!nx || !nz || !x || !z || B <= 0 || T <= 0 || T > 64 || !same_shape(nx, nz)) return INF_ERR_INVALID;
   hipStream_t s = (hipStream_t)stream;
   Bufs bf;
@@ -885,6 +887,7 @@
 int inf_imblock_backward(InfNet* nx, InfNet* nz, const float* z, const float* x, const float* grad, float* dl_dh,
                          float* dl_dx, int B, int T, double eps, InfBroydenStats* stats, void* ws, size_t ws_bytes,
                          void* stream) {
+  INF_TRY(eval_join_pending((hipStream_t)stream));
   if (!nx || !nz || !z || !x || !grad || !dl_dh || !dl_dx || B <= 0 || T <= 0 || T > 64 || !same_shape(nx, nz))
     return INF_ERR_INVALID;
   hipStream_t s = (hipStream_t)stream;
@@ -917,6 +920,7 @@
 
 int inf_banach_find_root(InfNet* f, InfNet* e, const float* y, float* out, int B, int threshold, double eps,
                          int* iters, void* ws, size_t ws_bytes, void* stream) {
+  INF_TRY(eval_join_pending((hipStream_t)stream));
   if (!f || !e || !y || !out || B <= 0 || threshold < 0 || !same_shape(f, e)) return INF_ERR_INVALID;
   hipStream_t s = (hipStream_t)stream;
   Bufs bf;
@@ -939,6 +943,7 @@
 int inf_broyden_update(float* U, float* VT, const float* dx, const float* dg, const float* gx, const float* x,
                        float* update, float* x_next, float* dx_next, int B, int d, int T, int nstep, void* ws,
                        size_t ws_bytes, void* stream) {
+  INF_TRY(eval_join_pending((hipStream_t)stream));
   if (!U || !VT || !dx || !dg || !gx || !x || !update || !x_next || !dx_next || B <= 0 || d <= 0 || T <= 0 ||
       T > 64 || nstep < 1 || nstep > T)
     return INF_ERR_INVALID;
diff --git a/implicit-normalizing-flows_amd/csrc/glue.h b/implicit-normalizing-flows_amd/csrc/glue.h
--- a/implicit-normalizing-flows_amd/csrc/glue.h
+++ b/implicit-normalizing-flows_amd/csrc/glue.h
@@ -5,6 +5,7 @@
 int glue_logit(const float* x, float* y, const float* lin, float* lout, int B, int per, float alpha, hipStream_t s);
 int glue_actnorm(const float* x, float* y, const float* w, const float* b, const float* lin, float* lout, int B, int C,
                  int hw, hipStream_t s);
+int glue_actnorm_logp(const float* w, const float* lin, float* lout, int B, int C, int hw, hipStream_t s);
 int glue_squeeze2(const float* x, float* y, int B, int C, int H, int W, hipStream_t s);
 int glue_normal_logprob(const float* z, float* out, int B, int per, hipStream_t s);
 int glue_rademacher(float* out, size_t n, uint64_t seed, uint64_t offset, hipStream_t s);
diff --git a/implicit-normalizing-flows_amd/csrc/glue.hip b/implicit-normalizing-flows_amd/csrc/glue.hip
--- a/implicit-normalizing-flows_amd/csrc/glue.hip
+++ b/implicit-normalizing-flows_amd/csrc/glue.hip
@@ -19,6 +19,14 @@
   }
   acc = block_sum(acc, red);
   if (threadIdx.x == 0) lout[b] = (lin ? lin[b] : 0.f) - (float)acc;
+}
+
+__device__ __forceinline__ void actnorm_logp(const float* w, const float* lin, float* lout, int C, int hw, int b,
+                                             double* red) {
+  double acc = 0.0;
+  for (int c = threadIdx.x; c < C; c += blockDim.x) acc += (double)w[c] * hw;
+  acc = block_sum(acc, red);
+  if (threadIdx.x == 0 && lout) lout[b] = (lin ? lin[b] : 0.f) - (float)acc;
 }
 
 __global__ __launch_bounds__(256) void actnorm_kernel(const float* x, float* y, const float* w, const float* bias,
@@ -43,10 +51,12 @@
     }
   }
   if (blockIdx.x != 0) return;
-  double acc = 0.0;
-  for (int c = threadIdx.x; c < C; c += blockDim.x) acc += (double)w[c] * hw;
-  acc = block_sum(acc, red);
-  if (threadIdx.x == 0 && lout) lout[b] = (lin ? lin[b] : 0.f) - (float)acc;
+  actnorm_logp(w, lin, lout, C, hw, b, red);
+}
+
+__global__ __launch_bounds__(256) void actnorm_logp_kernel(const float* w, const float* lin, float* lout, int C, int hw) {
+  __shared__ double red[16];
+  actnorm_logp(w, lin, lout, C, hw, blockIdx.x, red);
 }
 
 __global__ void squeeze2_kernel(const float* x, float* y, int C, int H, int W, long n) {
@@ -133,6 +143,11 @@
   INF_CHECK_LAUNCH();
   return INF_OK;
 }
+int glue_actnorm_logp(const float* w, const float* lin, float* lout, int B, int C, int hw, hipStream_t s) {
+  hipLaunchKernelGGL(actnorm_logp_kernel, dim3(B), dim3(256), 0, s, w, lin, lout, C, hw);
+  INF_CHECK_LAUNCH();
+  return INF_OK;
+}
 int glue_squeeze2(const float* x, float* y, int B, int C, int H, int W, hipStream_t s) {
   const long n = (long)B * C * H * W;
   hipLaunchKernelGGL(squeeze2_kernel, GRID1(n), 0, s, x, y, C, H, W, n);
diff --git a/implicit-normalizing-flows_amd/csrc/power.hip b/implicit-normalizing-flows_amd/csrc/power.hip
--- a/implicit-normalizing-flows_amd/csrc/power.hip
+++ b/implicit-normalizing-flows_amd/csrc/power.hip
@@ -547,6 +547,8 @@
   }
 }
 
+int eval_join_pending(hipStream_t s);
+
 }
 
 using namespace inf;
@@ -560,6 +562,7 @@
 
 int inf_power_iteration(const InfPowerIterDesc* d, int max_iters, int use_tol, float atol, float rtol,
                         int* iters_used, void* ws, size_t ws_bytes, void* stream) {
+  INF_TRY(eval_join_pending((hipStream_t)stream));
   if (!pi_valid(d) || max_iters < 0) return INF_ERR_INVALID;
   if (!ws || ws_bytes < inf_power_iteration_workspace_bytes(d)) return INF_ERR_WORKSPACE;
   hipStream_t s = (hipStream_t)stream;
@@ -600,6 +603,7 @@
 
 int inf_power_iteration_batch(const InfPowerIterDesc* descs, int n, int max_iters, int use_tol, float atol,
                               float rtol, int* iters_used, void* ws, size_t ws_bytes, void* stream) {
+  INF_TRY(eval_join_pending((hipStream_t)stream));
   if (!descs || n <= 0 || max_iters < 0) return INF_ERR_INVALID;
   for (int i = 0; i < n; ++i)
     if (!pi_valid(&descs[i])) return INF_ERR_INVALID;
diff --git a/implicit-normalizing-flows_amd/lib/_hip/__init__.py b/implicit-normalizing-flows_amd/lib/_hip/__init__.py
--- a/implicit-normalizing-flows_amd/lib/_hip/__init__.py
+++ b/implicit-normalizing-flows_amd/lib/_hip/__init__.py
@@ -16,6 +16,7 @@
 INF_OPT_FUSED_K128, INF_OPT_EVAL_OVERLAP, INF_OPT_CONVERGENCE, INF_OPT_K128_EXACT_SCALE = 1, 2, 3, 4
 INF_OPT_FC_BLOCK, INF_OPT_FC_SERIES, INF_OPT_LINE_SEARCH, INF_OPT_FUSED_PRESPLIT = 5, 6, 7, 8
 INF_OPT_FC_SKINNY = 9
+INF_OPT_EVAL_PIPELINE = 10
 INF_CONV_GLOBAL, INF_CONV_PER_SAMPLE = 0, 1
 CONVERGENCE = {'global': INF_CONV_GLOBAL, 'per_sample': INF_CONV_PER_SAMPLE}
 
@@ -99,6 +100,10 @@
     'inf_imblock_eval': (ctypes.c_int, [_P, _P, _P, _P, _P, _P, ctypes.POINTER(ctypes.c_float), ctypes.c_int, _P, _P,
                                         ctypes.c_int, ctypes.c_int, ctypes.c_double, ctypes.POINTER(BroydenStats), _P,
                                         ctypes.c_size_t, _P]),
+    'inf_eval_join': (ctypes.c_int, [_P]),
+    'inf_eval_pending': (ctypes.c_int, []),
+    'inf_eval_logp_step': (ctypes.c_int, [_P, _P, _P, _P, ctypes.c_int, _P]),
+    'inf_eval_actnorm_logp': (ctypes.c_int, [_P, _P, _P, ctypes.c_int, ctypes.c_int, ctypes.c_int, _P]),
     'inf_imblock_eval_exact': (ctypes.c_int, [_P, _P, _P, _P, _P, _P, ctypes.c_int, ctypes.c_int, ctypes.c_double,
                                               ctypes.POINTER(BroydenStats), _P, ctypes.c_size_t, _P]),
     'inf_flow_chain_workspace_bytes': (ctypes.c_size_t, [ctypes.POINTER(_P), ctypes.c_int, ctypes.c_int,
@@ -215,14 +220,59 @@
 _ws = {}
 
 
-def workspace(device, nbytes):
+def workspace(device, nbytes, slot=0):
     idx = torch.device(device).index if torch.device(device).index is not None else torch.cuda.current_device()
-    key = (idx, torch.cuda.current_stream(idx).cuda_stream)
+    key = (idx, torch.cuda.current_stream(idx).cuda_stream, slot)
     buf = _ws.get(key)
     if buf is None or buf.numel() < nbytes:
         buf = torch.empty(int(nbytes * 1.1) + 4096, dtype=torch.uint8, device=device)
         _ws[key] = buf
     return buf
+
+
+_pipe = threading.local()
+
+
+class eval_scope:
+
+    def __enter__(self):
+        _pipe.depth = getattr(_pipe, 'depth', 0) + 1
+        return self
+
+    def __exit__(self, *exc):
+        _pipe.depth -= 1
+        if _pipe.depth == 0:
+            eval_join()
+        return False
+
+
+def in_eval_scope():
+    return getattr(_pipe, 'depth', 0) > 0
+
+
+def eval_pending():
+    return getattr(_pipe, 'dirty', False) and _lib is not None and _lib.inf_eval_pending() == 1
+
+
+def eval_deferred(*tensors):
+    _pipe.dirty = True
+    if not hasattr(_pipe, 'held'):
+        _pipe.held = []
+    _pipe.held.extend(t for t in tensors if t is not None)
+
+
+def eval_ws_slot():
+    _pipe.slot = 1 - getattr(_pipe, 'slot', 1)
+    return _pipe.slot
+
+
+def eval_join():
+    if not getattr(_pipe, 'dirty', False):
+        return
+    if _lib is not None and _lib.inf_eval_pending() == 1:
+        check(_lib.inf_eval_join(ctypes.c_void_p(_raw_stream(torch.cuda.current_device()))), 'inf_eval_join')
+    _pipe.dirty = False
+    _pipe.held = []
 
 
 class NativeNet:
diff --git a/implicit-normalizing-flows_amd/lib/implicit_flow.py b/implicit-normalizing-flows_amd/lib/implicit_flow.py
--- a/implicit-normalizing-flows_amd/lib/implicit_flow.py
+++ b/implicit-normalizing-flows_amd/lib/implicit_flow.py
@@ -2,7 +2,7 @@
 import torch
 import torch.nn as nn
 
-from . import layers
+from . import _hip, layers
 from .layers import base as base_layers
 
 ACT_FNS = {
@@ -187,15 +187,16 @@
         if classify:
             raise NotImplementedError('classification heads are outside the density-evaluation path')
         factored = []
-        for idx, stage in enumerate(self.transforms):
-            if logpx is not None:
-                x, logpx = stage(x, logpx, restore=restore)
-            else:
-                x = stage(x, restore=restore)
-            if self.factor_out and idx < len(self.transforms) - 1:
-                half = x.size(1) // 2
-                x, f = x[:, :half], x[:, half:]
-                factored.append(f)
+        with _hip.eval_scope():
+            for idx, stage in enumerate(self.transforms):
+                if logpx is not None:
+                    x, logpx = stage(x, logpx, restore=restore)
+                else:
+                    x = stage(x, restore=restore)
+                if self.factor_out and idx < len(self.transforms) - 1:
+                    half = x.size(1) // 2
+                    x, f = x[:, :half], x[:, half:]
+                    factored.append(f)
         factored.append(x)
         out = torch.cat([o.reshape(o.size(0), -1) for o in factored], 1)
         return out if logpx is None else (out, logpx)
diff --git a/implicit-normalizing-flows_amd/lib/layers/flows.py b/implicit-normalizing-flows_amd/lib/layers/flows.py
--- a/implicit-normalizing-flows_amd/lib/layers/flows.py
+++ b/implicit-normalizing-flows_amd/lib/layers/flows.py
@@ -26,6 +26,7 @@
     def forward(self, x, logpx=None, restore=False):
         if logpx is not None and not restore and not self.training and x.is_cuda:
             from .imblock import eval_exact_chain
+            _hip.eval_join()
             out = eval_exact_chain(list(self.chain), x, logpx, owner=self)
             if out is not None:
                 return out
@@ -33,8 +34,9 @@
             for layer in self.chain:
                 x = layer(x, restore=restore)
             return x
-        for layer in self.chain:
-            x, logpx = layer(x, logpx, restore=restore)
+        with _hip.eval_scope():
+            for layer in self.chain:
+                x, logpx = layer(x, logpx, restore=restore)
         return x, logpx
 
     def inverse(self, y, logpy=None):
@@ -131,10 +133,19 @@
             y = torch.empty_like(x)
             lin = _logp_tensor(logpx, B, x.device)
             lout = torch.empty(B, device=x.device) if logpx is not None else None
+            if logpx is not None and _hip.eval_pending():
+                lib, stream = _hip.load(), _hip.stream_of(x)
+                _hip.check(lib.inf_actnorm_forward(_hip.ptr(x), _hip.ptr(y), _hip.ptr(self.weight), _hip.ptr(self.bias),
+                                                   None, None, B, C, hw, stream), 'inf_actnorm_forward')
+                _hip.check(lib.inf_eval_actnorm_logp(_hip.ptr(self.weight), _hip.ptr(lin), _hip.ptr(lout), B, C, hw,
+                                                     stream), 'inf_eval_actnorm_logp')
+                _hip.eval_deferred(lin, lout)
+                return y, lout.view(B, 1)
             _hip.check(_hip.load().inf_actnorm_forward(
                 _hip.ptr(x), _hip.ptr(y), _hip.ptr(self.weight), _hip.ptr(self.bias), _hip.ptr(lin),
                 _hip.ptr(lout), B, C, hw, _hip.stream_of(x)), 'inf_actnorm_forward')
             return y if logpx is None else (y, lout.view(B, 1))
+        _hip.eval_join()
         shape = [1, -1] + [1] * (x.dim() - 2)
         y = (x + self.bias.view(*shape)) * torch.exp(self.weight.view(*shape))
         return y if logpx is None else (y, logpx - self._logdetgrad(x))
@@ -166,6 +177,7 @@
         self.alpha = alpha
 
     def forward(self, x, logpx=None, restore=False):
+        _hip.eval_join()
         B = x.shape[0]
         lgraph = logpx if torch.is_tensor(logpx) else None
         if x.is_cuda and x.dtype == torch.float32 and not _graph(x, lgraph):
@@ -219,6 +231,7 @@
         return (-hw * self.std.abs().log().sum()).expand(x.shape[0], 1)
 
     def forward(self, x, logpx=None, restore=False):
+        _hip.eval_join()
         c = self.mean.numel()
         y = x.clone()
         y[:, :c] = (x[:, :c] - self._per_channel(self.mean)) / self._per_channel(self.std)
diff --git a/implicit-normalizing-flows_amd/lib/layers/imblock.py b/implicit-normalizing-flows_amd/lib/layers/imblock.py
--- a/implicit-normalizing-flows_amd/lib/layers/imblock.py
+++ b/implicit-normalizing-flows_amd/lib/layers/imblock.py
@@ -592,9 +592,8 @@
                 self.nnet_z_copy(x)
         nx, nz, stream = self._native(x)
         if logpx is not None and not self.training and not self.exact_trace and x.dim() == 4:
-            out = self._eval_fused(nx, nz, x, stream)
-            if out is not None:
-                return out[0], logpx - out[1]
+            return self._eval_fused(nx, nz, x, stream, logpx)
+        _hip.eval_join()
         if logpx is not None and not self.training and x.dim() == 2 and x.shape[1] <= 10:
             out = self._eval_exact(nx, nz, x, stream)
             if out is not None:
@@ -623,7 +622,7 @@
         self.last_broyden = st.as_dict(T)
         return z, (out[0] - out[1]).view(-1, 1)
 
-    def _eval_fused(self, nx, nz, x, stream):
+    def _eval_fused(self, nx, nz, x, stream, logpx):
         lib = _hip.load()
         x = x.contiguous()
         B, T = x.shape[0], int(self.threshold)
@@ -631,23 +630,39 @@
         n_ps, coeff_fn, ns = plan
         probes = (_probes(x.shape, x.device), _probes(x.shape, x.device))
         co = solvers.logdet_coefficients(n_ps, coeff_fn)
-        ws = _hip.workspace(x.device, nx.ws_bytes(B, T) + nz.ws_bytes(B, 1) + nx.ws_bytes(B, 1))
+        in_scope = _hip.in_eval_scope()
+        ws = _hip.workspace(x.device, nx.ws_bytes(B, T) + nz.ws_bytes(B, 1) + nx.ws_bytes(B, 1),
+                            _hip.eval_ws_slot() if in_scope else 0)
         z = torch.empty_like(x)
         out = torch.empty(2, B, device=x.device)
         st = _stats(B, (nz,))
+        _hip.eval_deferred(x, z, probes[0], probes[1], out, ws)
         rc = lib.inf_imblock_eval(nx.handle, nz.handle, _hip.ptr(x), _hip.ptr(z), _hip.ptr(probes[0]),
                                   _hip.ptr(probes[1]), co.ctypes.data_as(ctypes.POINTER(ctypes.c_float)), n_ps,
                                   _hip.ptr(out[0]), _hip.ptr(out[1]), B, T, float(self.eps_forward), ctypes.byref(st),
                                   _hip.ptr(ws), ws.numel(), stream)
         if rc == _hip.INF_ERR_UNSUPPORTED:
+            _hip.eval_join()
             with torch.no_grad():
                 z = self._root(nz, nx, x, self.eps_forward, stream, forward=True)
-            return z, self._logdetgrad(z, x, plan=plan, probes=probes)
+            return z, logpx - self._logdetgrad(z, x, plan=plan, probes=probes)
         _hip.check(rc, 'inf_imblock_eval')
         self.last_broyden = st.as_dict(T)
-        return z, self._finish_logdet(out[0] - out[1], n_ps, ns)
+        column = not torch.is_tensor(logpx) or tuple(logpx.shape) == (B, 1)
+        if in_scope and column and _hip.eval_pending():
+            from .flows import _logp_tensor
+            lin = _logp_tensor(logpx, B, x.device)
+            lout = torch.empty(B, device=x.device)
+            _hip.check(lib.inf_eval_logp_step(_hip.ptr(lin), _hip.ptr(out[0]), _hip.ptr(out[1]), _hip.ptr(lout), B,
+                                              stream), 'inf_eval_logp_step')
+            _hip.eval_deferred(lin, lout)
+            self.last_n_power_series = n_ps
+            return z, lout.view(B, 1)
+        _hip.eval_join()
+        return z, logpx - self._finish_logdet(out[0] - out[1], n_ps, ns)
 
     def inverse(self, z, logpy=None):
+        _hip.eval_join()
         nx, nz, stream = self._native(z)
         with torch.no_grad():
             x = self._root(nx, nz, z, self.eps_sample, stream, forward=False)
diff --git a/include/inflow.h b/include/inflow.h
--- a/include/inflow.h
+++ b/include/inflow.h
@@ -79,7 +79,7 @@
 typedef enum InfNetOption {
   INF_OPT_FUSED_K128 = 1, INF_OPT_EVAL_OVERLAP = 2, INF_OPT_CONVERGENCE = 3, INF_OPT_K128_EXACT_SCALE = 4,
   INF_OPT_FC_BLOCK = 5, INF_OPT_FC_SERIES = 6, INF_OPT_LINE_SEARCH = 7, INF_OPT_FUSED_PRESPLIT = 8,
-  INF_OPT_FC_SKINNY = 9
+  INF_OPT_FC_SKINNY = 9, INF_OPT_EVAL_PIPELINE = 10
 } InfNetOption;
 typedef enum InfConvergence { INF_CONV_GLOBAL = 0, INF_CONV_PER_SAMPLE = 1 } InfConvergence;
 int inf_net_set_option(InfNet* net, int option, int value);
@@ -110,6 +110,11 @@
 int inf_imblock_eval(InfNet* net_x, InfNet* net_z, const float* x, float* z, const float* eps_x, const float* eps_z,
                      const float* coeff, int n_terms, float* logdet_x, float* logdet_z, int batch, int threshold,
                      double eps, InfBroydenStats* stats, void* ws, size_t ws_bytes, void* stream);
+int inf_eval_join(void* stream);
+int inf_eval_pending(void);
+int inf_eval_logp_step(const float* lin, const float* logdet_x, const float* logdet_z, float* lout, int batch,
+                       void* stream);
+int inf_eval_actnorm_logp(const float* w, const float* lin, float* lout, int batch, int channels, int hw, void* stream);
 int inf_imblock_eval_exact(InfNet* net_x, InfNet* net_z, const float* x, float* z, float* logdet_x, float* logdet_z,
                            int batch, int threshold, double eps, InfBroydenStats* stats, void* ws, size_t ws_bytes,
                            void* stream);
```
